# edshkim98/LocalDiffusion-Hallucination

Measured on AMD Instinct MI355X. Metric: local patches/sec (256^2, T=1000), higher is better.
Workload: dtype bf16; 1 GPU; cfg3: 8 local patches (vertical band masks) of one 3x256x256 image per GPU, 4-stage dim-32 conditional UNet (12.1M params), DDPM T=1000, pred_x0, sigmoid schedule; patches_per_gpu=8, parallelism=patch-sharded x1, one all-gather per sample, step_graph_replay=True, whole_batch_graph_flag=False, concurrent_sub_batches=2, weight_split_levels=0

## Files before the change

include/localdiff_hip.h:

```cpp
#ifndef LOCALDIFF_HIP_H
#define LOCALDIFF_HIP_H

#include <stddef.h>
#include <stdint.h>

#ifdef __cplusplus
extern "C" {
#endif

#define LD_OK 0
#define LD_EINVAL (-1)
#define LD_EHIP (-2)
#define LD_ETIMEOUT (-3)

#define LD_F32 0
#define LD_BF16 1
#define LD_F16 2

#define LD_STAT_STRIPES 16

#define LD_ACT_NONE 0
#define LD_ACT_SILU 1
#define LD_ACT_RELU 2

// ... 20 lines not shown
int ld_tuning_count(void);
const char* ld_tuning_name(int index);
#define LD_COUNTER_CONV3X3_C32 0
#define LD_COUNTER_CONV3X3_GENERIC 1
#define LD_COUNTER_CONV3X3_S32 2
#define LD_COUNTER_MAX 8
long long ld_counter(int which);
int ld_range_push(const char* name );
int ld_range_pop(void);

typedef struct ld_src {
  const void* data;
  int32_t C;
  int32_t pix_stride;
  int32_t upsample;
  const double* gn_stats;
  const float* gn_gamma;
  const float* gn_beta;
  int32_t gn_groups;
  int32_t act;
  const float* film;
  int32_t film_tstride;
  int32_t film_bstride;
} ld_src;

typedef struct ld_conv3x3_args {
  ld_src src[2];
  int32_t nsrc;
  const void* weight;
  const float* bias;
  void* out;
  double* out_stats;
  int32_t out_groups;
  int32_t B, H, W, Cout;
  const int32_t* t_ptr;
  int32_t dtype;
  const void* addend;
  int32_t weight_terms;
  const void* side_weight;
  const float* side_bias;
  void* side_out;
} ld_conv3x3_args;
int ld_conv3x3(const ld_conv3x3_args* args, void* stream);

#define LD_EPI_PLAIN 0
#define LD_EPI_QKV_LINEAR 1
#define LD_EPI_QKV_FULL 2
#define LD_EPI_RMS_RES 3
#define LD_EPI_RES 4
#define LD_EPI_GN_TAIL 5
typedef struct ld_conv1x1_args {
  ld_src src[2];
  int32_t nsrc;
  int32_t unshuffle;
  int32_t rms_in;
  const void* weight;
  int64_t weight_bstride;
  const float* bias;
  int32_t epilogue;
  int32_t hidden;
  float q_scale;
  const float* g2;
  const void* residual;
  ld_src gn_tail;
  void* out;
  uint32_t* kmax_out;
  int32_t B, H, W, Cout;
  int32_t dtype;
  int32_t weight_terms;
} ld_conv1x1_args;
int ld_conv1x1(const ld_conv1x1_args* args, void* stream);

int ld_pack_conv_weight(const float* w_oihw, const float* scale_in, void* out, int cout, int cin,
                        int ksize, int unshuffle, int dtype, void* stream);
int ld_pack_conv_weight_terms(const float* w_oihw, const float* scale_in, void* out, int cout, int cin,
                              int ksize, int unshuffle, int dtype, int terms, void* stream);

int ld_conv_image(const float* x_nchw, const float* w_oihw, const float* bias, void* out,
                  double* out_stats, int out_groups, int B, int Cin, int H, int W, int ksize,
                  int dtype, void* stream);

size_t ld_stem_packed_bytes(void);
int ld_pack_stem_weight(const float* w_oihw , void* out_packed, int Cin, void* stream);
int ld_conv_stem(const float* x, const void* w_packed, const float* bias, void* out, int B, int Cin, int H, int W,
                 int dtype , void* stream);
typedef struct ld_step_begin_args {
  void* zero_a; size_t bytes_a; void* zero_b; size_t bytes_b;
  int32_t* t_ptr; int delta; int32_t* idx_ptr; const int32_t* t_table;
  const float* film_rows; int row_floats; float* film_cur;
} ld_step_begin_args;
int ld_conv_stem_begin(const float* x, const void* w_packed, const float* bias, void* out, int B, int Cin, int H, int W,
                       int dtype, const ld_step_begin_args* begin, void* stream);


typedef struct ld_gn_apply_args {
  ld_src a;
  ld_src b;
  int32_t final_act;
  int32_t pool;
  void* out;
  int32_t B, H, W;
  const int32_t* t_ptr;
  int32_t dtype;
} ld_gn_apply_args;
int ld_gn_apply(const ld_gn_apply_args* args, void* stream);

int ld_linattn_kmax(const void* qkv, uint32_t* kmax_enc, int B, int n, int heads, int dim_head,
                    int dtype, void* stream);
int ld_linattn_ctx(const void* qkv, const uint32_t* kmax_enc, float* ctx_part,
                   int B, int n, int heads, int dim_head, int nchunks, int dtype, void* stream);
int ld_linattn_ctx_reduce(const float* ctx_part, int nchunks, float* ctxn, int B, int heads,
                          int dim_head, void* stream);
int ld_linattn_fold(const float* ctxn, const float* w_out ,
                    void* w_packed , int B, int C, int heads, int dim_head,
                    int perm, int dtype, void* stream);
int ld_linattn_ctxfold(const float* ctx_part, int nchunks, const float* w_out ,
                       void* w_packed , int B, int C, int heads, int dim_head,
                       int perm, int dtype, void* stream);
int ld_linattn_kvctx(const void* x, const void* wkv_packed, const float* kshift, float* ctx_part, int B,
                     int n, int C, int heads, int dim_head, int nchunks, int dtype, void* stream);
int ld_linattn_out(const void* x, const void* wq_packed, const float* qshift, const void* mfold,
                   const float* bias, const float* g2, void* out, int B, int n, int C, float q_scale,
                   int dtype, void* stream);
int ld_linattn_kvctx_terms(const void* x, const void* wkv_packed, const float* kshift, float* ctx_part, int B, int n, int C,
                           int heads, int dim_head, int nchunks, int dtype, int weight_terms, void* stream);
int ld_linattn_out_terms(const void* x, const void* wq_packed, const float* qshift, const void* mfold, const float* bias,
                         const float* g2, void* out, int B, int n, int C, float q_scale, int dtype, int weight_terms,
                         void* stream);
size_t ld_linattn_ctx_part_floats(int B, int heads, int dim_head, int nchunks);

int ld_attention(const void* qkv, void* out, int B, int n, int heads, int dim_head, int dtype,
                 void* stream);

int ld_time_mlp(const int32_t* times, int n, const float* freqs, int dim, const float* w1,
                const float* b1, const float* w2, const float* b2, int time_dim, float* temb,
                void* stream);
int ld_time_mlp_fourier(const int32_t* times, int n, const float* weights, int learned_dim, const float* w1,
                        const float* b1, const float* w2, const float* b2, int time_dim, float* temb, void* stream);
int ld_film(const float* temb, int n, int time_dim, const float* w, const float* b, int two_c,
            float* film, void* stream);

int ld_final_conv(const void* x, const float* w , const float* b, float* out_nchw,
                  int B, int H, int W, int Cin, int Cout, int dtype, void* stream);

int ld_final_step(const void* x, const float* w, const float* b, float* model_out, float* x_t, float* x0_out,
                  const float* sched, const int32_t* t_ptr, float lo, float hi, int objective, uint64_t seed,
                  int64_t noise_stream, int B, int H, int W, int Cin, int Cout, int dtype, void* stream);


int ld_final_step_at(const void* x, const float* w, const float* b, float* model_out, float* x_t, float* x0_out,
                     const float* sched, const int32_t* t_ptr, float lo, float hi, int objective, uint64_t seed,
                     int64_t noise_base, int64_t noise_tmul, int64_t noise_first, const float* keep_mask,
                     int B, int H, int W, int Cin, int Cout, int dtype, void* stream);

#define LD_OBJ_X0 0
#define LD_OBJ_NOISE 1
#define LD_OBJ_V 2
#define LD_SCHED_COLS 8
#define LD_SCHED_COEF1 0
#define LD_SCHED_COEF2 1
#define LD_SCHED_SIGMA 2
#define LD_SCHED_SQRT_RECIP 3
#define LD_SCHED_SQRT_RECIPM1 4
#define LD_SCHED_SQRT_AB 5
#define LD_SCHED_SQRT_1MAB 6
#define LD_SCHED_ABAR 7

int ld_randn(float* out, int64_t n, uint64_t seed, int64_t stream_base, int64_t stream_tmul,
             const int32_t* t_ptr, void* stream);
int ld_randn_at(float* out, int64_t n, int64_t first, uint64_t seed, int64_t stream_base, int64_t stream_tmul,
                const int32_t* t_ptr, void* stream);
int ld_step_add(int32_t* t_ptr, int delta, void* stream);
int ld_step_begin(void* zero_a, size_t bytes_a, void* zero_b, size_t bytes_b, int32_t* t_ptr, int delta,
                  int32_t* idx_ptr, const int32_t* t_table, void* stream);
int ld_step_begin_film(void* zero_a, size_t bytes_a, void* zero_b, size_t bytes_b, int32_t* t_ptr, int delta,
                       int32_t* idx_ptr, const int32_t* t_table, const float* film_rows, int row_floats,
                       float* film_cur, void* stream);

int ld_ddpm_step(const float* x_t, const float* model_out, const float* noise, float* x_prev,
                 float* x0_out, const float* sched, const int32_t* t_ptr, float lo, float hi,
                 int objective, int64_t n, void* stream);
int ld_ddim_step(const float* x_t, const float* model_out, const float* noise, float* x_next,
                 float sqrt_recip, float sqrt_recipm1, float sqrt_ab, float sqrt_1mab,
                 float sqrt_abar_next, float c, float sigma, float lo, float hi, int objective,
                 int last, int64_t n, void* stream);
int ld_ddim_step_at(const float* x_t, const float* model_out, const float* noise, float* x_next,
                    const float* pair_table, const int32_t* idx_ptr, float lo, float hi, int objective, int64_t n,
                    void* stream);
int ld_branch_conditions(const float* cond, const float* mask, float* cond_out, float* cond_in,
                         float lo_clip, int B, int C, int HW, void* stream);
int ld_mask_out(float* model_out, const float* mask, float min_val, int B, int C, int HW,
                void* stream);
int ld_fuse_ddpm(const float* x_out, const float* x_in, const float* x0_out, const float* x0_in,
                 const float* mask, float* x, float* x0, float lo, float hi, int B, int C, int HW,
                 void* stream);
int ld_branch_conditions_k(const float* cond, const float* masks, float* cond_k, float lo_clip, int B, int C, int K,
                           int HW, void* stream);
int ld_fuse_ddpm_k(const float* x_first, const float* x_rest, const float* x0_first, const float* x0_rest,
                   const float* masks, float* x, float* x0, float lo, float hi, int B, int C, int K, int HW,
                   void* stream);
int ld_posterior_step(const float* x_t, const float* x0, const float* noise, float* x_prev,
                      const float* sched, const int32_t* t_ptr, int64_t n, void* stream);
int ld_fuse_ddim(const float* x_out, const float* x_in, const float* x0_out, const float* x0_in,
                 const float* mask, const float* noise, float* x_next, float sqrt_recip,
                 float sqrt_recipm1, float sqrt_abar_next, float c, float sigma, float lo,
                 float hi, int B, int C, int HW, void* stream);
int ld_fuse_ddim_k(const float* x_first, const float* x_rest, const float* x0_first, const float* x0_rest,
                   const float* masks, const float* noise, float* x_next, float sqrt_recip, float sqrt_recipm1,
                   float sqrt_abar_next, float c, float sigma, float lo, float hi, int B, int C, int K, int HW,
                   void* stream);
int ld_q_sample(const float* x0, const float* noise, float* out, float sqrt_ab, float sqrt_1mab,
                int64_t n, void* stream);
int ld_q_sample_t(const float* x0, const float* noise, float* out, const int* t, const float* sqrt_ab,
                  const float* sqrt_1mab, int B, int64_t elems_per_sample, void* stream);
int ld_p_losses(const float* model_out, const float* x_start, const float* noise, const int* t, const float* sqrt_ab,
                const float* sqrt_1mab, const float* loss_weight, float* loss_out, int B, int64_t elems_per_sample,
                int objective, void* stream);
int ld_recompose(const float* patches , const float* masks , float* out,
                 int B, int K, int C, int HW, void* stream);

#define LD_SEG_SRC_PLAIN 0
#define LD_SEG_SRC_POOL 1
#define LD_SEG_SRC_CAT_D2S 2
typedef struct ld_seg_conv_args {
  const void* src0;
  const void* src1;
  int32_t C0, C1;
  int32_t mode;
  int32_t ksize;
  const float* weight;
  const float* scale;
  const float* shift;
  int32_t relu;
  void* out;
  int32_t B, H, W, Cout;
  int32_t dtype;
} ld_seg_conv_args;
int ld_seg_conv(const ld_seg_conv_args* args, void* stream);
int ld_seg_conv_image(const float* x_nchw, const float* w_oihw, const float* scale, const float* shift, void* out,
                      int B, int Cin, int H, int W, int dtype, void* stream);
int ld_seg_head(const void* x, const float* w, const float* bias, float* logits, float* prob, float* mask,
                int B, int H, int W, int C, int dtype, void* stream);
int ld_seg_pack_weight(const float* w_oihw, float* out, int cout, int cin, int ksize, void* stream);
int ld_seg_pack_convt(const float* w, const float* bias, float* w_out, float* bias_out, int cin, int cout, void* stream);

#define LD_SEG_RED_WORK_BYTES (2048 * 2 * 64 * 8)
int ld_seg_wgrad_splits(int B, int H, int W, int Cin, int Cout, int ksize);
int ld_seg_wgrad(const float* dy, const float* a, float* work, float* dw, int B, int H, int W, int Cin, int Cout,
                 int ksize, int splits, void* stream);
int ld_seg_bn_train(const float* y, const float* gamma, const float* beta, double* work, float* stat, float* running_mean,
                    float* running_var, float momentum, float eps, float* out, int64_t M, int C, void* stream);
int ld_seg_bn_backward(const float* da, const float* act, const float* y, const float* gamma, const float* stat, double* work,
                       float* dgamma, float* dbeta, float* dy, int64_t M, int C, void* stream);
int ld_seg_colsum(const float* x, double* work, float* out, int64_t M, int C, int fold, void* stream);
int ld_seg_pool(const float* x, float* out, int B, int H, int W, int C, void* stream);
int ld_seg_pool_backward(const float* x, const float* dpool, const float* dskip, float* dx, int B, int H, int W, int C,
                         void* stream);
int ld_seg_cat_d2s(const float* skip, const float* low, float* out, int B, int H, int W, int C0, int C1, void* stream);
int ld_seg_cat_d2s_backward(const float* dcat, float* dskip, float* dlow, int B, int H, int W, int C0, int C1, void* stream);
int ld_seg_loss(const float* logits, const float* target, double* work, float* out, float* dz, int64_t M, float pos_weight,
                float dice_eps, void* stream);
int ld_seg_head_backward(const float* dz, const float* x, const float* w, double* work, float* dw, float* db, float* dx,
                         int64_t M, int C, void* stream);
int ld_seg_adam(float* param, const float* grad, float* m, float* v, int d0, int d1, int d2, int64_t s0, int64_t s1,
                int64_t s2, double beta1, double beta2, double eps, double step_size, double bc2_sqrt, void* stream);
int ld_seg_permute3(const float* in, float* out, int d0, int d1, int d2, int64_t off, int64_t s0, int64_t s1, int64_t s2,
                    void* stream);

typedef struct ld_pc_conv_args {
  const float* src;
  const float* weight;
  const float* scale;
  const float* shift;
  const float* residual;
  float* out;
  int32_t B, Hi, Wi, Cin, Ho, Wo, Cout;
  int32_t ksize;
  int32_t stride;
  int32_t relu;
} ld_pc_conv_args;
int ld_pc_conv(const ld_pc_conv_args* args, void* stream);
int ld_pc_stem(const float* x_nchw, const float* w_oihw, const float* scale, const float* shift, float* out,
               int B, int H, int W, void* stream);
int ld_pc_maxpool(const float* x, float* out, int B, int H, int W, int C, void* stream);
int ld_pc_embed(const float* l2, const float* l3, float* rows, float* norms, int B, int h2, int w2, int C2, int h3,
                int w3, int C3, void* stream);
int ld_pc_row_norms(const float* x, float* norms, int64_t n, int d, void* stream);
int ld_pc_knn(const float* q, const float* qn, int N, const float* bank, const float* bn, int64_t M, int D,
              unsigned long long* work, float* dist, int32_t* idx, void* stream);
int ld_pc_knn_topk(const float* q, const float* qn, int N, const float* bank, const float* bn, int64_t M, int D, int k,
                   float* d2, float* dist, int32_t* idx, void* stream);
int ld_pc_score_prepare(const float* patch_scores, const int32_t* loc, const float* bank, const float* bn, int B, int P,
                        int D, float* q, float* qn, int32_t* argmax, void* stream);
int ld_pc_score(const float* rows, const float* row_norms, const float* patch_scores, const int32_t* argmax,
                const float* bank, const float* bn, const int32_t* support, int B, int P, int D, int k, float* pred_score,
                void* stream);
int ld_pc_anomaly_map(const float* scores, const float* g, int ks, float* tmp, float* out, int B, int h, int w, int H,
                      int W, void* stream);

int ld_pc_project(const float* e, int64_t N, int D, const int32_t* rowptr, const int32_t* cols, const float* vals, int k,
                  float* out, int64_t ld, void* stream);
int ld_pc_coreset(const float* ft, int64_t ld, int64_t N, int k, int64_t n, int64_t start, float* min_d,
                  unsigned long long* keys, int64_t* idx, void* stream);

int ld_clf_max(const float* x, int groups, int64_t n, uint32_t* words, void* stream);
enum { LD_CLF_PLAIN = 0, LD_CLF_HALVE = 1, LD_CLF_AFFINE = 2 };
// ... 61 lines not shown
```

localdiffusion-hallucination_amd/_cabi.py:

```python
import ctypes as C
import os

from .tuning import lib_override_path

_HERE = os.path.dirname(os.path.abspath(__file__))

LIB_PATH = lib_override_path() or os.path.join(_HERE, "csrc", "liblocaldiff_hip.so")

LD_F32, LD_BF16, LD_F16 = 0, 1, 2
ACT_NONE, ACT_SILU, ACT_RELU = 0, 1, 2
EPI_PLAIN, EPI_QKV_LINEAR, EPI_QKV_FULL, EPI_RMS_RES, EPI_RES, EPI_GN_TAIL = 0, 1, 2, 3, 4, 5
OBJ = {"pred_x0": 0, "pred_noise": 1, "pred_v": 2}
SCHED_COLS = 8
STAT_STRIPES = 16
COUNTER_CONV3X3_C32, COUNTER_CONV3X3_GENERIC, COUNTER_CONV3X3_S32 = 0, 1, 2
SEG_SRC_PLAIN, SEG_SRC_POOL, SEG_SRC_CAT_D2S = 0, 1, 2
CLF_PLAIN, CLF_HALVE, CLF_AFFINE = 0, 1, 2

vp, i32, i64, u64, f32 = C.c_void_p, C.c_int32, C.c_int64, C.c_uint64, C.c_float


class Src(C.Structure):
    _fields_ = [("data", vp), ("C", i32), ("pix_stride", i32), ("upsample", i32), ("gn_stats", vp),
                ("gn_gamma", vp), ("gn_beta", vp), ("gn_groups", i32), ("act", i32), ("film", vp),
                ("film_tstride", i32), ("film_bstride", i32)]


class Conv3x3Args(C.Structure):
    _fields_ = [("src", Src * 2), ("nsrc", i32), ("weight", vp), ("bias", vp), ("out", vp),
                ("out_stats", vp), ("out_groups", i32), ("B", i32), ("H", i32), ("W", i32),
                ("Cout", i32), ("t_ptr", vp), ("dtype", i32), ("addend", vp), ("weight_terms", i32),
                ("side_weight", vp), ("side_bias", vp), ("side_out", vp)]


class Conv1x1Args(C.Structure):
    _fields_ = [("src", Src * 2), ("nsrc", i32), ("unshuffle", i32), ("rms_in", i32), ("weight", vp),
                ("weight_bstride", i64), ("bias", vp), ("epilogue", i32), ("hidden", i32),
                ("q_scale", f32), ("g2", vp), ("residual", vp), ("gn_tail", Src), ("out", vp), ("kmax_out", vp), ("B", i32), ("H", i32),
                ("W", i32), ("Cout", i32), ("dtype", i32), ("weight_terms", i32)]


class GnApplyArgs(C.Structure):
    _fields_ = [("a", Src), ("b", Src), ("final_act", i32), ("pool", i32), ("out", vp), ("B", i32),
                ("H", i32), ("W", i32), ("t_ptr", vp), ("dtype", i32)]


class StepBeginArgs(C.Structure):
    _fields_ = [("zero_a", vp), ("bytes_a", C.c_size_t), ("zero_b", vp), ("bytes_b", C.c_size_t), ("t_ptr", vp), ("delta", i32),
                ("idx_ptr", vp), ("t_table", vp), ("film_rows", vp), ("row_floats", i32), ("film_cur", vp)]


class SegConvArgs(C.Structure):
    _fields_ = [("src0", vp), ("src1", vp), ("C0", i32), ("C1", i32), ("mode", i32), ("ksize", i32), ("weight", vp),
                ("scale", vp), ("shift", vp), ("relu", i32), ("out", vp), ("B", i32), ("H", i32), ("W", i32),
                ("Cout", i32), ("dtype", i32)]


class PcConvArgs(C.Structure):
    _fields_ = [("src", vp), ("weight", vp), ("scale", vp), ("shift", vp), ("residual", vp), ("out", vp), ("B", i32),
                ("Hi", i32), ("Wi", i32), ("Cin", i32), ("Ho", i32), ("Wo", i32), ("Cout", i32), ("ksize", i32),
                ("stride", i32), ("relu", i32)]


class ClfResizeArgs(C.Structure):
    _fields_ = [("x", vp), ("out", vp), ("B", i32), ("Cin", i32), ("Cout", i32), ("Hi", i32), ("Wi", i32), ("Ho", i32),
                ("Wo", i32), ("mode", i32), ("max_words", vp), ("per_sample", i32), ("zero_words", vp), ("n_zero", i32),
                ("sub", f32), ("mul", f32), ("add", f32), ("div", f32), ("normalize", i32), ("mean", f32 * 3),
                ("std", f32 * 3), ("pred", vp), ("threshold", f32), ("decision", vp), ("n_decision", i32)]


class McAdamTensor(C.Structure):
    _fields_ = [("param", vp), ("grad", vp), ("m", vp), ("v", vp), ("d0", i32), ("d1", i32), ("d2", i32), ("gs0", i64),
                ("gs1", i64), ("gs2", i64), ("mirror0", vp), ("m0_off", i64), ("m0_s0", i64), ("m0_s1", i64), ("m0_s2", i64),
                ("mirror1", vp), ("m1_off", i64), ("m1_s0", i64), ("m1_s1", i64), ("m1_s2", i64)]


_SIGS = {
    "ld_last_error": (C.c_char_p, []),
    "ld_version": (C.c_int, []),
    "ld_device_info": (C.c_int, [C.c_char_p, C.c_int, C.POINTER(C.c_int), C.POINTER(i64)]),
    "ld_graph_begin": (C.c_int, [vp]),
    "ld_graph_end": (C.c_int, [vp, C.POINTER(vp)]),
    "ld_graph_launch": (C.c_int, [vp, vp]),
    "ld_graph_destroy": (C.c_int, [vp]),
    "ld_memset_zero": (C.c_int, [vp, C.c_size_t, vp]),
    "ld_memset_bytes": (C.c_int, [vp, C.c_int, C.c_size_t, vp]),
    "ld_event_create": (C.c_int, [C.POINTER(vp)]),
    "ld_event_record": (C.c_int, [vp, vp]),
    "ld_event_elapsed_ms": (C.c_int, [vp, vp, C.POINTER(f32)]),
    "ld_event_destroy": (C.c_int, [vp]),
    "ld_stream_wait_event": (C.c_int, [vp, vp]),
    "ld_counter": (C.c_longlong, [C.c_int]),
    "ld_tuning_set": (C.c_int, [C.c_char_p, C.c_longlong]),
    "ld_tuning_get": (C.c_int, [C.c_char_p, C.POINTER(C.c_longlong)]),
    "ld_tuning_count": (C.c_int, []),
    "ld_tuning_name": (C.c_char_p, [C.c_int]),
    "ld_range_push": (C.c_int, [C.c_char_p]),
    "ld_range_pop": (C.c_int, []),
    "ld_conv3x3": (C.c_int, [C.POINTER(Conv3x3Args), vp]),
    "ld_conv1x1": (C.c_int, [C.POINTER(Conv1x1Args), vp]),
    "ld_pack_conv_weight": (C.c_int, [vp, vp, vp, C.c_int, C.c_int, C.c_int, C.c_int, C.c_int, vp]),
    "ld_pack_conv_weight_terms": (C.c_int, [vp, vp, vp, C.c_int, C.c_int, C.c_int, C.c_int, C.c_int, C.c_int, vp]),
    "ld_conv_image": (C.c_int, [vp, vp, vp, vp, vp, C.c_int, C.c_int, C.c_int, C.c_int, C.c_int,
                                C.c_int, C.c_int, vp]),
    "ld_stem_packed_bytes": (C.c_size_t, []),
    "ld_pack_stem_weight": (C.c_int, [vp, vp, C.c_int, vp]),
    "ld_conv_stem": (C.c_int, [vp, vp, vp, vp, C.c_int, C.c_int, C.c_int, C.c_int, C.c_int, vp]),
    "ld_conv_stem_begin": (C.c_int, [vp, vp, vp, vp, C.c_int, C.c_int, C.c_int, C.c_int, C.c_int, C.POINTER(StepBeginArgs), vp]),
    "ld_gn_apply": (C.c_int, [C.POINTER(GnApplyArgs), vp]),
    "ld_linattn_kmax": (C.c_int, [vp, vp, C.c_int, C.c_int, C.c_int, C.c_int, C.c_int, vp]),
    "ld_linattn_ctx": (C.c_int, [vp, vp, vp, C.c_int, C.c_int, C.c_int, C.c_int, C.c_int, C.c_int, vp]),
    "ld_linattn_ctx_reduce": (C.c_int, [vp, C.c_int, vp, C.c_int, C.c_int, C.c_int, vp]),
    "ld_linattn_fold": (C.c_int, [vp, vp, vp, C.c_int, C.c_int, C.c_int, C.c_int, C.c_int, C.c_int, vp]),
    "ld_linattn_ctxfold": (C.c_int, [vp, C.c_int, vp, vp, C.c_int, C.c_int, C.c_int, C.c_int, C.c_int, C.c_int, vp]),
    "ld_linattn_kvctx": (C.c_int, [vp, vp, vp, vp, C.c_int, C.c_int, C.c_int, C.c_int, C.c_int, C.c_int, C.c_int, vp]),
    "ld_linattn_out": (C.c_int, [vp, vp, vp, vp, vp, vp, vp, C.c_int, C.c_int, C.c_int, f32, C.c_int, vp]),
    "ld_linattn_kvctx_terms": (C.c_int, [vp, vp, vp, vp, C.c_int, C.c_int, C.c_int, C.c_int, C.c_int, C.c_int, C.c_int, C.c_int, vp]),
    "ld_linattn_out_terms": (C.c_int, [vp, vp, vp, vp, vp, vp, vp, C.c_int, C.c_int, C.c_int, f32, C.c_int, C.c_int, vp]),
    "ld_linattn_ctx_part_floats": (C.c_size_t, [C.c_int, C.c_int, C.c_int, C.c_int]),
    "ld_attention": (C.c_int, [vp, vp, C.c_int, C.c_int, C.c_int, C.c_int, C.c_int, vp]),
    "ld_time_mlp": (C.c_int, [vp, C.c_int, vp, C.c_int, vp, vp, vp, vp, C.c_int, vp, vp]),
    "ld_time_mlp_fourier": (C.c_int, [vp, C.c_int, vp, C.c_int, vp, vp, vp, vp, C.c_int, vp, vp]),
    "ld_film": (C.c_int, [vp, C.c_int, C.c_int, vp, vp, C.c_int, vp, vp]),
    "ld_final_conv": (C.c_int, [vp, vp, vp, vp, C.c_int, C.c_int, C.c_int, C.c_int, C.c_int, C.c_int, vp]),
    "ld_final_step": (C.c_int, [vp, vp, vp, vp, vp, vp, vp, vp, f32, f32, C.c_int, u64, i64, C.c_int, C.c_int, C.c_int,
                                C.c_int, C.c_int, C.c_int, vp]),
    "ld_final_step_at": (C.c_int, [vp, vp, vp, vp, vp, vp, vp, vp, f32, f32, C.c_int, u64, i64, i64, i64, vp, C.c_int,
                                   C.c_int, C.c_int, C.c_int, C.c_int, C.c_int, vp]),
    "ld_timing_begin": (C.c_int, [C.c_int]),
    "ld_timing_count": (C.c_int, []),
    "ld_timing_end": (C.c_int, [vp, C.c_int, vp]),
    "ld_timing_end_abs": (C.c_int, [vp, vp, C.c_int, vp]),
    "ld_randn": (C.c_int, [vp, i64, u64, i64, i64, vp, vp]),
    "ld_randn_at": (C.c_int, [vp, i64, i64, u64, i64, i64, vp, vp]),
    "ld_step_add": (C.c_int, [vp, C.c_int, vp]),
    "ld_step_begin": (C.c_int, [vp, C.c_size_t, vp, C.c_size_t, vp, C.c_int, vp, vp, vp]),
    "ld_step_begin_film": (C.c_int, [vp, C.c_size_t, vp, C.c_size_t, vp, C.c_int, vp, vp, vp, C.c_int, vp, vp]),
    "ld_ddim_step_at": (C.c_int, [vp, vp, vp, vp, vp, vp, f32, f32, C.c_int, i64, vp]),
    "ld_ddpm_step": (C.c_int, [vp, vp, vp, vp, vp, vp, vp, f32, f32, C.c_int, i64, vp]),
    "ld_posterior_step": (C.c_int, [vp, vp, vp, vp, vp, vp, i64, vp]),
    "ld_ddim_step": (C.c_int, [vp, vp, vp, vp, f32, f32, f32, f32, f32, f32, f32, f32, f32, C.c_int,
                               C.c_int, i64, vp]),
    "ld_branch_conditions": (C.c_int, [vp, vp, vp, vp, f32, C.c_int, C.c_int, C.c_int, vp]),
    "ld_mask_out": (C.c_int, [vp, vp, f32, C.c_int, C.c_int, C.c_int, vp]),
    "ld_fuse_ddpm": (C.c_int, [vp, vp, vp, vp, vp, vp, vp, f32, f32, C.c_int, C.c_int, C.c_int, vp]),
    "ld_branch_conditions_k": (C.c_int, [vp, vp, vp, f32, C.c_int, C.c_int, C.c_int, C.c_int, vp]),
    "ld_fuse_ddpm_k": (C.c_int, [vp, vp, vp, vp, vp, vp, vp, f32, f32, C.c_int, C.c_int, C.c_int, C.c_int, vp]),
    "ld_fuse_ddim": (C.c_int, [vp, vp, vp, vp, vp, vp, vp, f32, f32, f32, f32, f32, f32, f32, C.c_int,
                               C.c_int, C.c_int, vp]),
    "ld_fuse_ddim_k": (C.c_int, [vp, vp, vp, vp, vp, vp, vp, f32, f32, f32, f32, f32, f32, f32, C.c_int, C.c_int,
                                 C.c_int, C.c_int, vp]),
    "ld_q_sample": (C.c_int, [vp, vp, vp, f32, f32, i64, vp]),
    "ld_q_sample_t": (C.c_int, [vp, vp, vp, vp, vp, vp, C.c_int, i64, vp]),
    "ld_p_losses": (C.c_int, [vp, vp, vp, vp, vp, vp, vp, vp, C.c_int, i64, C.c_int, vp]),
    "ld_recompose": (C.c_int, [vp, vp, vp, C.c_int, C.c_int, C.c_int, C.c_int, vp]),
    "ld_seg_conv": (C.c_int, [C.POINTER(SegConvArgs), vp]),
    "ld_seg_conv_image": (C.c_int, [vp, vp, vp, vp, vp, C.c_int, C.c_int, C.c_int, C.c_int, C.c_int, vp]),
    "ld_seg_head": (C.c_int, [vp, vp, vp, vp, vp, vp, C.c_int, C.c_int, C.c_int, C.c_int, C.c_int, vp]),
    "ld_seg_pack_weight": (C.c_int, [vp, vp, C.c_int, C.c_int, C.c_int, vp]),
    "ld_seg_pack_convt": (C.c_int, [vp, vp, vp, vp, C.c_int, C.c_int, vp]),
    "ld_seg_wgrad_splits": (C.c_int, [C.c_int, C.c_int, C.c_int, C.c_int, C.c_int, C.c_int]),
    "ld_seg_wgrad": (C.c_int, [vp, vp, vp, vp, C.c_int, C.c_int, C.c_int, C.c_int, C.c_int, C.c_int, C.c_int, vp]),
    "ld_seg_bn_train": (C.c_int, [vp, vp, vp, vp, vp, vp, vp, f32, f32, vp, i64, C.c_int, vp]),
    "ld_seg_bn_backward": (C.c_int, [vp, vp, vp, vp, vp, vp, vp, vp, vp, i64, C.c_int, vp]),
    "ld_seg_colsum": (C.c_int, [vp, vp, vp, i64, C.c_int, C.c_int, vp]),
    "ld_seg_pool": (C.c_int, [vp, vp, C.c_int, C.c_int, C.c_int, C.c_int, vp]),
    "ld_seg_pool_backward": (C.c_int, [vp, vp, vp, vp, C.c_int, C.c_int, C.c_int, C.c_int, vp]),
    "ld_seg_cat_d2s": (C.c_int, [vp, vp, vp, C.c_int, C.c_int, C.c_int, C.c_int, C.c_int, vp]),
    "ld_seg_cat_d2s_backward": (C.c_int, [vp, vp, vp, C.c_int, C.c_int, C.c_int, C.c_int, C.c_int, vp]),
    "ld_seg_loss": (C.c_int, [vp, vp, vp, vp, vp, i64, f32, f32, vp]),
    "ld_seg_head_backward": (C.c_int, [vp, vp, vp, vp, vp, vp, vp, i64, C.c_int, vp]),
    "ld_seg_adam": (C.c_int, [vp, vp, vp, vp, C.c_int, C.c_int, C.c_int, i64, i64, i64, C.c_double, C.c_double, C.c_double,
                    C.c_double, C.c_double, vp]),
    "ld_seg_permute3": (C.c_int, [vp, vp, C.c_int, C.c_int, C.c_int, i64, i64, i64, i64, vp]),
    "ld_pc_conv": (C.c_int, [C.POINTER(PcConvArgs), vp]),
    "ld_pc_stem": (C.c_int, [vp, vp, vp, vp, vp, C.c_int, C.c_int, C.c_int, vp]),
    "ld_pc_maxpool": (C.c_int, [vp, vp, C.c_int, C.c_int, C.c_int, C.c_int, vp]),
    "ld_pc_embed": (C.c_int, [vp, vp, vp, vp, C.c_int, C.c_int, C.c_int, C.c_int, C.c_int, C.c_int, C.c_int, vp]),
    "ld_pc_row_norms": (C.c_int, [vp, vp, i64, C.c_int, vp]),
    "ld_pc_knn": (C.c_int, [vp, vp, C.c_int, vp, vp, i64, C.c_int, vp, vp, vp, vp]),
    "ld_pc_knn_topk": (C.c_int, [vp, vp, C.c_int, vp, vp, i64, C.c_int, C.c_int, vp, vp, vp, vp]),
    "ld_pc_score_prepare": (C.c_int, [vp, vp, vp, vp, C.c_int, C.c_int, C.c_int, vp, vp, vp, vp]),
    "ld_pc_score": (C.c_int, [vp, vp, vp, vp, vp, vp, vp, C.c_int, C.c_int, C.c_int, C.c_int, vp, vp]),
    "ld_pc_anomaly_map": (C.c_int, [vp, vp, C.c_int, vp, vp, C.c_int, C.c_int, C.c_int, C.c_int, C.c_int, vp]),
    "ld_pc_project": (C.c_int, [vp, i64, C.c_int, vp, vp, vp, C.c_int, vp, i64, vp]),
    "ld_pc_coreset": (C.c_int, [vp, i64, i64, C.c_int, i64, i64, vp, vp, vp, vp]),
    "ld_clf_max": (C.c_int, [vp, C.c_int, i64, vp, vp]),
    "ld_clf_resize": (C.c_int, [C.POINTER(ClfResizeArgs), vp]),
    "ld_clf_decide": (C.c_int, [vp, f32, vp, C.c_int, vp]),
    "ld_mc_conv1": (C.c_int, [vp, vp, vp, vp, vp, C.c_int, vp]),
    "ld_mc_pool": (C.c_int, [vp, vp, vp, C.c_int, C.c_int, C.c_int, C.c_int, vp]),
    "ld_mc_pool_backward": (C.c_int, [vp, vp, vp, vp, C.c_int, C.c_int, C.c_int, C.c_int, vp]),
    "ld_mc_gemm": (C.c_int, [vp, vp, vp, C.c_int, C.c_int, C.c_int, i64, i64, i64, i64, i64, C.c_int, vp]),
    "ld_mc_fc1_finish": (C.c_int, [vp, vp, vp, C.c_int, C.c_int, C.c_int, vp]),
    "ld_mc_head": (C.c_int, [vp, vp, vp, vp, vp, vp, vp, vp, vp, vp, C.c_int, vp]),
    "ld_mc_small_grads": (C.c_int, [vp, vp, vp, vp, vp, vp, vp, vp, C.c_int, vp]),
    "ld_mc_conv1_wgrad_work_floats": (i64, [C.c_int]),
    "ld_mc_conv1_wgrad": (C.c_int, [vp, vp, vp, vp, vp, vp, vp, C.c_int, vp]),
    "ld_mc_adam": (C.c_int, [C.POINTER(McAdamTensor), C.c_int, C.c_double, C.c_double, C.c_double, C.c_double, C.c_double, vp]),
    "ld_comm_unique_id": (C.c_int, [vp]),
    "ld_comm_init": (C.c_int, [C.POINTER(vp), vp, C.c_int, C.c_int]),
    "ld_comm_init_timeout": (C.c_int, [C.POINTER(vp), vp, C.c_int, C.c_int, C.c_double]),
    "ld_allgather": (C.c_int, [vp, vp, C.c_size_t, vp, vp]),
    "ld_comm_destroy": (C.c_int, [vp]),
}

EXPORTS = tuple(_SIGS)
_lib = None


def lib():
    global _lib
    if _lib is not None:
        return _lib
    if not os.path.exists(LIB_PATH):
        raise RuntimeError(
            f"{LIB_PATH} is missing: build it with `python -c 'import __graft_entry__ as g; g.build()'` "
            "(or csrc/build.sh).  There is no CPU fallback for the HIP hot path.")
    try:
        l = C.CDLL(LIB_PATH)
    except OSError as e:
        raise RuntimeError(f"cannot load {LIB_PATH}: {e}") from e
    for name, (res, args) in _SIGS.items():
        try:
            fn = getattr(l, name)
        except AttributeError as e:
            raise RuntimeError(f"{LIB_PATH} does not export {name}") from e
        fn.restype, fn.argtypes = res, args
    _lib = l
    return l


LD_ETIMEOUT = -3


def check(rc, what=""):
    if rc != 0:
        msg = lib().ld_last_error().decode("utf-8", "replace")
        if rc == LD_ETIMEOUT:
            raise TimeoutError(f"localdiff_hip {what} timed out: {msg}")
        raise RuntimeError(f"localdiff_hip {what} failed (rc={rc}): {msg}")


class prof_range:

    def __init__(self, name):
        self.name = name.encode()

    def __enter__(self):
        lib().ld_range_push(self.name)

    def __exit__(self, *exc):
        lib().ld_range_pop()


def ptr(t):
    return None if t is None else t.data_ptr()


def dtype_code(name):
    return {"fp32": LD_F32, "float32": LD_F32, "bf16": LD_BF16, "bfloat16": LD_BF16, "fp16": LD_F16, "float16": LD_F16,
            "half": LD_F16}[name]
```

localdiffusion-hallucination_amd/csrc/conv1x1.hip:

```cpp
#include "common.hip.h"
#include <stdlib.h>

namespace {

constexpr int EPI_GN_TAIL_RES = 6;

struct Conv1Dev {
  SrcDev s[2];
  const void* w;
  long w_bstride;
  const void* res;
  void* out;
  int nsrc, unshuffle, rms_in;
  int B, H, W, Cout;
  int wsplit;
  int group;
  int epi, hidden;
  float q_scale;
  const float* bias;
  const float* g2;
  unsigned* kmax;
  SrcDev tail;
};

constexpr int KG = 4;
typedef const Conv1Dev __attribute__((address_space(4)))* Conv1KernargPtr;
template <typename T, int MT, int NW, int EPI, int G, bool TLEAD, bool KLEAD = false>
__device__ __forceinline__ void conv1x1_body(const Conv1Dev& head, Conv1KernargPtr rest) {
  constexpr int E = DT<T>::E, CK = DT<T>::CK;
  constexpr int NPT = 64 * NW, PLANE = NPT * 16;
  constexpr int XCH = 4 * PLANE, WCHB = MT * 1024;
  static_assert(!TLEAD || EPI == LD_EPI_GN_TAIL || EPI == EPI_GN_TAIL_RES, "tail-lead variant: GroupNorm-tail epilogues only");
  Conv1Dev a = head;
  if constexpr (KLEAD) {
    a.out = rest->out; a.bias = rest->bias; a.g2 = rest->g2; a.kmax = rest->kmax; a.hidden = rest->hidden; a.q_scale = rest->q_scale;
  }
  if constexpr (!TLEAD && !KLEAD) {
    asm volatile("" ::"s"(a.H), "s"(a.W), "s"(a.Cout), "s"(a.nsrc), "s"(a.unshuffle), "s"(a.rms_in), "s"(a.wsplit), "s"(a.s[0].C),
                 "s"(a.s[0].ld), "s"(a.s[0].data), "s"(a.s[1].C), "s"(a.s[1].ld), "s"(a.s[1].data), "s"(a.w), "s"(a.w_bstride),
                 "s"(a.res), "s"(a.out));
    if constexpr (EPI == LD_EPI_GN_TAIL || EPI == EPI_GN_TAIL_RES)
      asm volatile("" ::"s"(a.tail.data), "s"(a.tail.stats), "s"(a.tail.gamma), "s"(a.tail.beta), "s"(a.tail.film), "s"(a.tail.C),
                   "s"(a.tail.groups), "s"(a.tail.act), "s"(a.tail.film_bstride));
  }

  extern __shared__ __attribute__((aligned(16))) char smem[];
  char* s_x = smem;
  char* s_w = smem + G * XCH;
  float* s_rinv = reinterpret_cast<float*>(s_w + G * WCHB);
  float* s_tcoef = s_rinv + NPT;

  const int tid = threadIdx.x, lane = tid & 63, wv = tid >> 6, px = lane & 15, kq = lane >> 4;
  const int b = blockIdx.z, m0 = blockIdx.y * MT;
  const int HW = a.H * a.W, p0 = blockIdx.x * NPT;
  const int mt_total = a.Cout / 16;

  f32x4 acc[MT][NW];
#pragma unroll
  for (int m = 0; m < MT; ++m)
#pragma unroll
    for (int j = 0; j < NW; ++j) acc[m][j] = f32x4{0.f, 0.f, 0.f, 0.f};
  float rs[NW];
#pragma unroll
  for (int i = 0; i < NW; ++i) rs[i] = 0.f;

  constexpr bool TAIL = EPI == LD_EPI_GN_TAIL || EPI == EPI_GN_TAIL_RES;
  constexpr bool HAS_OP2 = EPI == LD_EPI_RMS_RES || EPI == LD_EPI_RES || TAIL;
  typedef typename Raw4<T>::type R4;
  constexpr bool W2 = sizeof(T) == 2;
  constexpr int MP = W2 ? MT / 2 : MT;
  typedef typename std::conditional<W2, uint4, R4>::type RP;
  RP op2[HAS_OP2 ? MP : 1][HAS_OP2 ? NW : 1];
  auto load_op = [&](const T* src, RP (&dst)[MP][NW]) {
#pragma unroll
    for (int j = 0; j < NW; ++j) {
      const int p = min(p0 + (wv * NW + j) * 16 + px, HW - 1);
      const T* pix = src + ((size_t)b * HW + p) * a.Cout + m0 * 16;
#pragma unroll
      for (int m = 0; m < MP; ++m) {
        if constexpr (W2) dst[m][j] = *reinterpret_cast<const uint4*>(reinterpret_cast<const char*>(pix + m * 32) + pair_frag16_off(kq));
        else dst[m][j] = load4_raw<T>(pix + m * 16 + kq * 4);
      }
    }
  };
  auto pin_op = [&](const RP& r) {
    if constexpr (W2) asm volatile("" ::"v"(r.x), "v"(r.y), "v"(r.z), "v"(r.w));
    else pin_raw4(r);
  };
  auto frag_op = [&](const RP (&src)[MP][NW], int m, int j, float* v) {
    if constexpr (W2) {
      uint2 f0, f1;
      unpair_frag16(src[m >> 1][j], f0, f1);
      unpack4<T>((m & 1) ? f1 : f0, v);
    } else {
      unpack4<T>(src[m][j], v);
    }
  };
  if constexpr (HAS_OP2) load_op(reinterpret_cast<const T*>(TAIL ? a.tail.data : a.res), op2);
  if constexpr (TAIL) {
    double* red = reinterpret_cast<double*>(s_tcoef + 2 * a.Cout);
    if constexpr (TLEAD) {
      build_gn_coef<DT<T>::precise>(a.tail, b, 0, (long)HW, s_tcoef, red, tid, 256, [&]() {
        Conv1KernargPtr pr = rest;
        asm volatile("" : "+s"(pr));
        a.s[0].data = pr->s[0].data; a.s[0].C = pr->s[0].C; a.s[0].ld = pr->s[0].ld;
        a.s[1].data = pr->s[1].data; a.s[1].C = pr->s[1].C; a.s[1].ld = pr->s[1].ld;
        a.w = pr->w; a.w_bstride = pr->w_bstride; a.res = pr->res; a.out = pr->out;
        a.nsrc = pr->nsrc; a.unshuffle = pr->unshuffle; a.rms_in = pr->rms_in; a.H = pr->H; a.W = pr->W;
        a.wsplit = pr->wsplit; a.hidden = pr->hidden; a.q_scale = pr->q_scale; a.bias = pr->bias; a.g2 = pr->g2; a.kmax = pr->kmax;
        a.tail.act = pr->tail.act;
      });
    } else {
      build_gn_coef<DT<T>::precise>(a.tail, b, 0, (long)HW, s_tcoef, red, tid, 256);
    }
  }
  const int nc0 = a.s[0].C / CK;
  const int ws = a.wsplit;
  const int nch = (a.unshuffle ? 4 * nc0 : nc0 + (a.nsrc > 1 ? a.s[1].C / CK : 0)) << ws;
  const uint4* wg = reinterpret_cast<const uint4*>(reinterpret_cast<const char*>(a.w) + (size_t)b * a.w_bstride);

  auto frag_ptr = [&](int chv, int it) -> const uint4* {
    const int ch = chv >> ws;
    int si = 0, c0, p1 = 0, p2 = 0;
    if (a.unshuffle) {
      const int pp = ch / nc0;
      c0 = (ch - pp * nc0) * CK;
      p1 = pp >> 1; p2 = pp & 1;
    } else {
      si = ch >= nc0 ? 1 : 0;
      c0 = (ch - si * nc0) * CK;
    }
    const T* sdata = reinterpret_cast<const T*>(si ? a.s[1].data : a.s[0].data);
    const int Cs = si ? a.s[1].ld : a.s[0].ld;
    const int p = p0 + (it * 4 + wv) * 16 + px;
    if (p >= HW) return nullptr;
    size_t pix;
    if (a.unshuffle) {
      const int y = p / a.W, x = p - y * a.W;
      pix = ((size_t)b * (2 * a.H) + 2 * y + p1) * (2 * a.W) + 2 * x + p2;
    } else {
      pix = (size_t)b * HW + p;
    }
    return reinterpret_cast<const uint4*>(sdata + pix * Cs + c0 + kq * E);
  };
  auto stage = [&](const uint4& raw, int it, char* xdst) {
    if (a.rms_in) {
      float v[E];
      unpack16<T>(raw, v);
#pragma unroll
      for (int e = 0; e < E; ++e) rs[it] = fmaf(v[e], v[e], rs[it]);
    }
    *reinterpret_cast<uint4*>(xdst + kq * PLANE + ((it * 4 + wv) * 16 + px) * 16) = raw;
  };
  auto mfma_chunk = [&](const char* xsrc, const char* wsrc) {
    uint4 A[MT];
#pragma unroll
    for (int m = 0; m < MT; ++m) A[m] = *reinterpret_cast<const uint4*>(wsrc + m * 1024 + lane * 16);
#pragma unroll
    for (int j = 0; j < NW; ++j) {
      const uint4 Bf = *reinterpret_cast<const uint4*>(xsrc + kq * PLANE + ((wv * NW + j) * 16 + px) * 16);
#pragma unroll
      for (int m = 0; m < MT; ++m) mma16<T>(acc[m][j], A[m], Bf);
    }
  };
  constexpr int WPT = (MT * 64 + 255) / 256;
  if constexpr (G > 1) {
    for (int c0 = 0; c0 < nch; c0 += G) {
      uint4 raw[G][NW], wr[G][WPT];
#pragma unroll
      for (int g = 0; g < G; ++g) {
        if (c0 + g < nch) {
#pragma unroll
          for (int it = 0; it < NW; ++it) {
            const uint4* gp = frag_ptr(c0 + g, it);
            raw[g][it] = gp ? *gp : make_uint4(0u, 0u, 0u, 0u);
          }
#pragma unroll
          for (int k = 0; k < WPT; ++k) {
            const int u = k * 256 + tid;
            wr[g][k] = u < MT * 64 ? wg[((size_t)(c0 + g) * mt_total + m0) * 64 + u] : make_uint4(0u, 0u, 0u, 0u);
          }
        }
      }
      __syncthreads();
#pragma unroll
      for (int g = 0; g < G; ++g) {
        if (c0 + g < nch) {
#pragma unroll
          for (int it = 0; it < NW; ++it) stage(raw[g][it], it, s_x + (size_t)g * XCH);
#pragma unroll
          for (int k = 0; k < WPT; ++k) {
            const int u = k * 256 + tid;
            if (u < MT * 64) *reinterpret_cast<uint4*>(s_w + (size_t)g * WCHB + u * 16) = wr[g][k];
          }
        }
      }
      __syncthreads();
#pragma unroll
      for (int g = 0; g < G; ++g)
        if (c0 + g < nch) mfma_chunk(s_x + (size_t)g * XCH, s_w + (size_t)g * WCHB);
    }
  } else {
    for (int ch = 0; ch < nch; ++ch) {
      __syncthreads();
#pragma unroll
      for (int it = 0; it < NW; ++it) {
        const uint4* gp = frag_ptr(ch, it);
        stage(gp ? *gp : make_uint4(0u, 0u, 0u, 0u), it, s_x);
      }
#pragma unroll
      for (int k = 0; k < WPT; ++k) {
        const int u = k * 256 + tid;
        if (u < MT * 64) *reinterpret_cast<uint4*>(s_w + u * 16) = wg[((size_t)ch * mt_total + m0) * 64 + u];
      }
      __syncthreads();
      mfma_chunk(s_x, s_w);
    }
  }

  if (a.rms_in) {
#pragma unroll
    for (int it = 0; it < NW; ++it) {
      float r = rs[it];
      r = kq4_sum(r);
      if (kq == 0) s_rinv[(it * 4 + wv) * 16 + px] = rms_rinv<DT<T>::precise>(r);
    }
    __syncthreads();
  }

  float bv[MT][4], g2v[EPI == LD_EPI_RMS_RES ? MT : 1][4];
#pragma unroll
  for (int m = 0; m < MT; ++m) {
    const int co = (m0 + m) * 16 + kq * 4;
    const float4 t = a.bias ? *reinterpret_cast<const float4*>(a.bias + co) : make_float4(0.f, 0.f, 0.f, 0.f);
    bv[m][0] = t.x; bv[m][1] = t.y; bv[m][2] = t.z; bv[m][3] = t.w;
    if constexpr (EPI == LD_EPI_RMS_RES) {
      const float4 g = *reinterpret_cast<const float4*>(a.g2 + co);
      g2v[m][0] = g.x; g2v[m][1] = g.y; g2v[m][2] = g.z; g2v[m][3] = g.w;
    }
  }
  constexpr bool HAS_OP3 = EPI == EPI_GN_TAIL_RES;
  RP op3[HAS_OP3 ? MP : 1][HAS_OP3 ? NW : 1];
  if constexpr (HAS_OP3) load_op(reinterpret_cast<const T*>(a.res), op3);

  T* out = reinterpret_cast<T*>(a.out);
  const bool q_part = (m0 * 16) < a.hidden;
  const bool k_part = a.kmax != nullptr && (m0 * 16) >= a.hidden && (m0 * 16) < 2 * a.hidden;
  float cmax[MT][4];
#pragma unroll
  for (int m = 0; m < MT; ++m)
#pragma unroll
    for (int r = 0; r < 4; ++r) cmax[m][r] = -INFINITY;
#pragma unroll
  for (int m = 0; m < MT; ++m) {
    asm volatile("" ::"v"(bv[m][0]), "v"(bv[m][1]), "v"(bv[m][2]), "v"(bv[m][3]));
    if constexpr (EPI == LD_EPI_RMS_RES) asm volatile("" ::"v"(g2v[m][0]), "v"(g2v[m][1]), "v"(g2v[m][2]), "v"(g2v[m][3]));
  }
#pragma unroll
  for (int m = 0; m < MP; ++m) {
    if constexpr (HAS_OP2) {
#pragma unroll
      for (int j = 0; j < NW; ++j) pin_op(op2[m][j]);
    }
    if constexpr (HAS_OP3) {
#pragma unroll
      for (int j = 0; j < NW; ++j) pin_op(op3[m][j]);
    }
  }
#pragma unroll
  for (int j = 0; j < NW; ++j) {
    const int qq = (wv * NW + j) * 16 + px;
    const int p = p0 + qq;
    const bool valid = p < HW;
    const float rinv = a.rms_in ? s_rinv[qq] : 1.0f;
    float v[MT][4];
#pragma unroll
    for (int m = 0; m < MT; ++m) {
#pragma unroll
      for (int r = 0; r < 4; ++r) v[m][r] = acc[m][j][r] * rinv + bv[m][r];
    }
    if (EPI == LD_EPI_QKV_LINEAR && q_part) {
#pragma unroll
      for (int m = 0; m < MT; m += 2) {
        float mx = v[m][0];
#pragma unroll
        for (int r = 0; r < 4; ++r) { mx = fmaxf(mx, v[m][r]); mx = fmaxf(mx, v[m + 1][r]); }
        mx = kq4_max(mx);
        float sum = 0.f;
#pragma unroll
        for (int r = 0; r < 4; ++r) {
          v[m][r] = DT<T>::precise ? expf(v[m][r] - mx) : __expf(v[m][r] - mx);
          v[m + 1][r] = DT<T>::precise ? expf(v[m + 1][r] - mx) : __expf(v[m + 1][r] - mx);
          sum += v[m][r] + v[m + 1][r];
        }
        sum = kq4_sum(sum);
        const float sc = DT<T>::precise ? a.q_scale / sum : a.q_scale * __builtin_amdgcn_rcpf(sum);
#pragma unroll
        for (int r = 0; r < 4; ++r) { v[m][r] *= sc; v[m + 1][r] *= sc; }
      }
    } else if (EPI == LD_EPI_QKV_FULL && q_part) {
#pragma unroll
      for (int m = 0; m < MT; ++m)
#pragma unroll
        for (int r = 0; r < 4; ++r) v[m][r] *= a.q_scale;
    } else if (EPI == LD_EPI_RMS_RES) {
      float ss = 0.f;
#pragma unroll
      for (int m = 0; m < MT; ++m)
#pragma unroll
        for (int r = 0; r < 4; ++r) ss = fmaf(v[m][r], v[m][r], ss);
      ss = kq4_sum(ss);
      const float inv = rms_rinv<DT<T>::precise>(ss);
#pragma unroll
      for (int m = 0; m < MT; ++m) {
#pragma unroll
        for (int r = 0; r < 4; ++r) v[m][r] = v[m][r] * inv * g2v[m][r];
      }
    }
    if (k_part && valid) {
#pragma unroll
      for (int m = 0; m < MT; ++m)
#pragma unroll
        for (int r = 0; r < 4; ++r) cmax[m][r] = fmaxf(cmax[m][r], v[m][r]);
    }
#pragma unroll
    for (int m = 0; m < MT; ++m) {
      const int co = (m0 + m) * 16 + kq * 4;
      if constexpr (EPI == LD_EPI_RMS_RES || EPI == LD_EPI_RES) {
        float o2[4];
        frag_op(op2, m, j, o2);
#pragma unroll
        for (int r = 0; r < 4; ++r) v[m][r] += o2[r];
      } else if constexpr (TAIL) {
        float rv[4];
        frag_op(op2, m, j, rv);
        affine_act_n<DT<T>::precise, 4>(rv, s_tcoef + co, s_tcoef + a.Cout + co, a.tail.act);
#pragma unroll
        for (int r = 0; r < 4; ++r) v[m][r] += rv[r];
        if constexpr (HAS_OP3) {
          float o3[4];
          frag_op(op3, m, j, o3);
#pragma unroll
          for (int r = 0; r < 4; ++r) v[m][r] += o3[r];
        }
      }
    }
    T* opix = out + ((size_t)b * HW + (valid ? p : 0)) * a.Cout + m0 * 16;
    if constexpr (sizeof(T) == 2) {
      static_assert(MT % 2 == 0, "m-tiles are stored in pairs");
#pragma unroll
      for (int m = 0; m < MT; m += 2) {
        const uint4 w16 = pair_frag16<T>(v[m], v[m + 1]);
        if (valid) store16_out(reinterpret_cast<char*>(opix + m * 16) + pair_frag16_off(kq), w16);
      }
    } else if (valid) {
#pragma unroll
      for (int m = 0; m < MT; ++m) store4<T>(opix + m * 16 + kq * 4, v[m]);
    }
  }
  if (k_part) {
    float* s_cm = reinterpret_cast<float*>(s_x);
    __syncthreads();
#pragma unroll
    for (int m = 0; m < MT; ++m)
#pragma unroll
      for (int r = 0; r < 4; ++r) {
        const float cm = wave16_max(cmax[m][r]);
        if (px == 0) s_cm[wv * 16 * MT + m * 16 + kq * 4 + r] = cm;
      }
    __syncthreads();
    if (tid < 16 * MT) {
      const float cm = fmaxf(fmaxf(s_cm[tid], s_cm[16 * MT + tid]), fmaxf(s_cm[32 * MT + tid], s_cm[48 * MT + tid]));
      const int stripe = blockIdx.x % LD_STAT_STRIPES;
      if (cm > -INFINITY)
        atomicMax(a.kmax + ((size_t)b * LD_STAT_STRIPES + stripe) * a.hidden + m0 * 16 + tid - a.hidden, enc_max(cm));
    }
  }
}

template <typename T, int MT, int NW, int EPI, int G = 1>
__global__ __launch_bounds__(256) void conv1x1_kernel(Conv1Dev a) {
  conv1x1_body<T, MT, NW, EPI, G, false>(a, nullptr);
}
template <typename T, int MT, int NW, int EPI, int G>
__global__ __launch_bounds__(256) void conv1x1_taillead_kernel(const void* t_data, const double* t_stats, const float* t_gamma, const float* t_beta,
                                                               const float* t_film, int cout_groups, int hw, Conv1Dev rest) {
  Conv1Dev a{};
  a.tail.data = t_data; a.tail.stats = t_stats; a.tail.gamma = t_gamma; a.tail.beta = t_beta; a.tail.film = t_film;
  a.Cout = cout_groups & 0xffff; a.tail.C = a.Cout; a.tail.ld = a.Cout; a.tail.groups = (int)((unsigned)cout_groups >> 16);
  a.H = hw; a.W = 1;
  constexpr unsigned REST_OFF = ld_kernarg_offset<const void*, const double*, const float*, const float*, const float*, int, int>(alignof(Conv1Dev));
  static_assert(REST_OFF == 48, "conv1x1_taillead_kernel: leading arguments changed");
  typedef const char __attribute__((address_space(4)))* KChar;
  conv1x1_body<T, MT, NW, EPI, G, true>(a, (Conv1KernargPtr)((KChar)__builtin_amdgcn_kernarg_segment_ptr() + REST_OFF));
}

template <typename T, int MT, int NW, int EPI, int G>
__global__ __launch_bounds__(256) void conv1x1_klead_kernel(const void* data0, const void* w, const void* data1, const void* res, int H, int W,
                                                            int Cout, int c0_flags, int ld0, int c1_ld1, Conv1Dev rest) {
  Conv1Dev a{};
  a.s[0].data = data0; a.s[0].C = c0_flags & 0xffff; a.s[0].ld = ld0;
  a.s[1].data = data1; a.s[1].C = c1_ld1 & 0xffff; a.s[1].ld = (int)((unsigned)c1_ld1 >> 16);
  a.w = w; a.res = res; a.H = H; a.W = W; a.Cout = Cout;
  a.nsrc = (c0_flags >> 16) & 3; a.unshuffle = (c0_flags >> 18) & 1; a.rms_in = (c0_flags >> 19) & 1; a.wsplit = (c0_flags >> 20) & 1;
  constexpr unsigned REST_OFF = ld_kernarg_offset<const void*, const void*, const void*, const void*, int, int, int, int, int, int>(alignof(Conv1Dev));
  static_assert(REST_OFF == 56, "conv1x1_klead_kernel: leading arguments changed");
  typedef const char __attribute__((address_space(4)))* KChar;
  conv1x1_body<T, MT, NW, EPI, G, false, true>(a, (Conv1KernargPtr)((KChar)__builtin_amdgcn_kernarg_segment_ptr() + REST_OFF));
}

template <typename T, int MT, int NW, int EPI>
int launch_epi(const Conv1Dev& a, hipStream_t st) {
  constexpr int NPT = 64 * NW;
  const size_t tail = NPT * sizeof(float) + (EPI == LD_EPI_GN_TAIL || EPI == EPI_GN_TAIL_RES ? 2 * a.Cout * sizeof(float) + 64 * sizeof(double) : 0);
  const size_t chunk = 4 * NPT * 16 + MT * 1024;
  const int HW = a.H * a.W;
  dim3 grid((HW + NPT - 1) / NPT, a.Cout / (16 * MT), a.B);
  constexpr bool CAN_TLEAD = EPI == LD_EPI_GN_TAIL || EPI == EPI_GN_TAIL_RES;
  const bool tlead = CAN_TLEAD && ld_tuning().lead_args && a.tail.film_bstride == 0 && a.tail.film_tstride == 0 && a.Cout < 65536 && a.tail.groups < 32768 &&
                     a.tail.C == a.Cout && a.tail.ld == a.Cout && (long)HW < (1L << 31);
#define LD_C1_TLEAD_ARGS a.tail.data, a.tail.stats, a.tail.gamma, a.tail.beta, a.tail.film, a.Cout | (a.tail.groups << 16), HW, a
  if constexpr (CAN_TLEAD) {
    if (tlead && (a.group == KG || a.group == 2)) {
      const size_t lds = (size_t)a.group * chunk + tail;
      if (a.group == KG) {
        if (lds > 65536) LD_HIP(ld_allow_lds((conv1x1_taillead_kernel<T, MT, NW, EPI, KG>), lds));
        LD_LAUNCH((conv1x1_taillead_kernel<T, MT, NW, EPI, KG>), grid, dim3(256), lds, st, LD_C1_TLEAD_ARGS);
      } else {
        if (lds > 65536) LD_HIP(ld_allow_lds((conv1x1_taillead_kernel<T, MT, NW, EPI, 2>), lds));
        LD_LAUNCH((conv1x1_taillead_kernel<T, MT, NW, EPI, 2>), grid, dim3(256), lds, st, LD_C1_TLEAD_ARGS);
      }
      LD_LAUNCH_CHECK("conv1x1(GroupNorm tail, lead)");
      return LD_OK;
    }
  }
#undef LD_C1_TLEAD_ARGS
  if constexpr (!CAN_TLEAD) {
    const bool klead = ld_tuning().lead_args && (a.group == KG || a.group == 2) && a.w_bstride == 0 && a.s[0].C < 65536 && a.s[1].C < 65536 && a.s[1].ld < 65536;
    if (klead) {
      const int c0f = a.s[0].C | (a.nsrc << 16) | (a.unshuffle ? 1 << 18 : 0) | (a.rms_in ? 1 << 19 : 0) | (a.wsplit ? 1 << 20 : 0);
      const int c1l = (a.nsrc > 1 ? a.s[1].C : 0) | ((a.nsrc > 1 ? a.s[1].ld : 0) << 16);
      const size_t lds = (size_t)a.group * chunk + tail;
#define LD_C1_KLEAD_ARGS a.s[0].data, a.w, a.s[1].data, a.res, a.H, a.W, a.Cout, c0f, a.s[0].ld, c1l, a
      if (a.group == KG) {
        if (lds > 65536) LD_HIP(ld_allow_lds((conv1x1_klead_kernel<T, MT, NW, EPI, KG>), lds));
        LD_LAUNCH((conv1x1_klead_kernel<T, MT, NW, EPI, KG>), grid, dim3(256), lds, st, LD_C1_KLEAD_ARGS);
      } else {
        if (lds > 65536) LD_HIP(ld_allow_lds((conv1x1_klead_kernel<T, MT, NW, EPI, 2>), lds));
        LD_LAUNCH((conv1x1_klead_kernel<T, MT, NW, EPI, 2>), grid, dim3(256), lds, st, LD_C1_KLEAD_ARGS);
      }
#undef LD_C1_KLEAD_ARGS
      LD_LAUNCH_CHECK("conv1x1(grouped K, lead)");
      return LD_OK;
    }
  }
  if (a.group == KG) {
    const size_t lds = KG * chunk + tail;
    if (lds > 65536) LD_HIP(ld_allow_lds((conv1x1_kernel<T, MT, NW, EPI, KG>), lds));
    LD_LAUNCH((conv1x1_kernel<T, MT, NW, EPI, KG>), grid, dim3(256), lds, st, a);
    LD_LAUNCH_CHECK("conv1x1(grouped K)");
    return LD_OK;
  }
  if (a.group == 2) {
    const size_t lds = 2 * chunk + tail;
    if (lds > 65536) LD_HIP(ld_allow_lds((conv1x1_kernel<T, MT, NW, EPI, 2>), lds));
    LD_LAUNCH((conv1x1_kernel<T, MT, NW, EPI, 2>), grid, dim3(256), lds, st, a);
    LD_LAUNCH_CHECK("conv1x1(grouped K, pairs)");
    return LD_OK;
  }
  LD_LAUNCH((conv1x1_kernel<T, MT, NW, EPI>), grid, dim3(256), chunk + tail, st, a);
  LD_LAUNCH_CHECK("conv1x1");
  return LD_OK;
}

template <typename T, int MT, int NW>
int launch(const Conv1Dev& a, hipStream_t st) {
  switch (a.epi) {
    case LD_EPI_PLAIN: return launch_epi<T, MT, NW, LD_EPI_PLAIN>(a, st);
    case LD_EPI_QKV_LINEAR: return launch_epi<T, MT, NW, LD_EPI_QKV_LINEAR>(a, st);
    case LD_EPI_QKV_FULL: return launch_epi<T, MT, NW, LD_EPI_QKV_FULL>(a, st);
    case LD_EPI_RMS_RES: return launch_epi<T, MT, NW, LD_EPI_RMS_RES>(a, st);
    case LD_EPI_RES: return launch_epi<T, MT, NW, LD_EPI_RES>(a, st);
    default: return a.res ? launch_epi<T, MT, NW, EPI_GN_TAIL_RES>(a, st) : launch_epi<T, MT, NW, LD_EPI_GN_TAIL>(a, st);
  }
}

template <typename T>
int dispatch(const Conv1Dev& a0, hipStream_t st) {
  Conv1Dev a = a0;
  const int HW = a.H * a.W;
  {
    const LdTuning& tn = ld_tuning();
    const long group_max_px = tn.c1_group_max_px;
    const int group_on = (int)tn.c1_group;
    const int ck = DT<T>::CK;
    const int nc0 = a.s[0].C / ck;
    const int nch = (a.unshuffle ? 4 * nc0 : nc0 + (a.nsrc > 1 ? a.s[1].C / ck : 0)) << a.wsplit;
    const int group_min_ch = (int)tn.c1_group_min_ch;
    a.group = (group_on && (long)HW * a.B <= group_max_px && nch >= group_min_ch) ? KG : 0;
    const long pair_max_px = tn.c1_pair_max_px;
    if (group_on && !a.group && (long)HW * a.B <= pair_max_px && nch >= 2) a.group = 2;
  }
  if (a.epi == LD_EPI_RMS_RES) {
    switch (a.Cout) {
      case 32: return launch<T, 2, 2>(a, st);
      case 64: return launch<T, 4, 2>(a, st);
      case 128: return launch<T, 8, 2>(a, st);
      default: return ld_fail(LD_EINVAL, "ld_conv1x1: RMS_RES epilogue supports Cout 32/64/128 (got %d)", a.Cout);
    }
  }
  bool mt4 = (a.Cout % 64) == 0;
  const long small_min = ld_tuning().c1_small_min;
  if (mt4 && (long)((HW + 127) / 128) * (a.Cout / 64) * a.B < small_min) mt4 = false;
  const long blocks4 = (long)((HW + 255) / 256) * (a.Cout / (mt4 ? 64 : 32)) * a.B;
  const bool big = blocks4 >= 512;
  if (mt4) return big ? launch<T, 4, 4>(a, st) : launch<T, 4, 2>(a, st);
  return big ? launch<T, 2, 4>(a, st) : launch<T, 2, 2>(a, st);
}

}

extern "C" int ld_conv1x1(const ld_conv1x1_args* p, void* stream) {
  LD_REQUIRE(p != nullptr, "ld_conv1x1: null args");
  LD_REQUIRE(p->nsrc == 1 || p->nsrc == 2, "ld_conv1x1: nsrc must be 1 or 2");
  LD_REQUIRE(ld_dtype_ok(p->dtype), "ld_conv1x1: bad dtype %d", p->dtype);
  LD_REQUIRE(p->Cout > 0 && p->Cout % 32 == 0, "ld_conv1x1: Cout %d must be a multiple of 32", p->Cout);
  LD_REQUIRE(p->B > 0 && p->H > 0 && p->W > 0 && p->weight && p->out, "ld_conv1x1: bad shape/null");
  LD_REQUIRE(!(p->unshuffle && p->nsrc != 1), "ld_conv1x1: unshuffle takes one source");
  LD_REQUIRE(p->epilogue >= LD_EPI_PLAIN && p->epilogue <= LD_EPI_GN_TAIL, "ld_conv1x1: bad epilogue");
  if (p->epilogue == LD_EPI_QKV_LINEAR || p->epilogue == LD_EPI_QKV_FULL)
    LD_REQUIRE(p->hidden > 0 && p->hidden % 64 == 0 && p->Cout == 3 * p->hidden,
               "ld_conv1x1: QKV epilogue needs Cout == 3*hidden, hidden %% 64 == 0");
  if (p->epilogue == LD_EPI_RMS_RES) LD_REQUIRE(p->g2 && p->residual, "ld_conv1x1: RMS_RES needs g2/residual");
  LD_REQUIRE((reinterpret_cast<uintptr_t>(p->bias) & 15) == 0 && (reinterpret_cast<uintptr_t>(p->g2) & 15) == 0,
             "ld_conv1x1: bias / g2 must be 16-byte aligned (read as float4)");
  if (p->epilogue == LD_EPI_RES) LD_REQUIRE(p->residual, "ld_conv1x1: RES needs residual");
  Conv1Dev a;
  for (int s = 0; s < p->nsrc; ++s) {
    LD_REQUIRE(p->src[s].data && p->src[s].C > 0 && p->src[s].C % 32 == 0,
               "ld_conv1x1: src[%d] null or C %% 32 != 0", s);
    LD_REQUIRE(p->src[s].gn_stats == nullptr && !p->src[s].upsample,
               "ld_conv1x1: GroupNorm/upsample prologues are 3x3-only");
    a.s[s] = to_dev(p->src[s]);
  }
  if (p->nsrc == 1) a.s[1] = a.s[0];
  a.nsrc = p->nsrc; a.unshuffle = p->unshuffle; a.rms_in = p->rms_in;
  a.w = p->weight; a.w_bstride = p->weight_bstride; a.bias = p->bias;
  a.epi = p->epilogue;
  a.hidden = (p->epilogue == LD_EPI_QKV_LINEAR || p->epilogue == LD_EPI_QKV_FULL) ? p->hidden : 0;
  a.q_scale = p->q_scale; a.g2 = p->g2; a.res = p->residual; a.out = p->out;
  a.kmax = (p->epilogue == LD_EPI_QKV_LINEAR) ? p->kmax_out : nullptr;
  if (p->epilogue == LD_EPI_GN_TAIL) {
    const ld_src& t = p->gn_tail;
    LD_REQUIRE(t.gn_groups <= 16, "ld_conv1x1: gn_tail groups %d > 16 (the stripe reduction uses 16 lanes per group)", t.gn_groups);
    LD_REQUIRE(t.data && t.gn_stats && t.gn_gamma && t.gn_beta && t.gn_groups > 0 && t.C == p->Cout &&
               t.C % t.gn_groups == 0 && (t.pix_stride == 0 || t.pix_stride == t.C) && !t.film,
               "ld_conv1x1: GN_TAIL operand incomplete");
    a.tail = to_dev(t);
  } else {
    a.tail = a.s[0];
  }
  a.B = p->B; a.H = p->H; a.W = p->W; a.Cout = p->Cout;
  a.group = 0;
  LD_REQUIRE(p->weight_terms >= 0 && p->weight_terms <= 2 && !(p->weight_terms == 2 && (!ld_dtype_16(p->dtype) || p->rms_in || p->weight_bstride)),
             "ld_conv1x1: weight_terms %d (2 needs 16-bit storage, no rms_in, no per-batch weights)", p->weight_terms);
  a.wsplit = p->weight_terms == 2 ? 1 : 0;
  hipStream_t st = reinterpret_cast<hipStream_t>(stream);
  return LD_DISPATCH(p->dtype, dispatch<T>(a, st));
}
```

localdiffusion-hallucination_amd/csrc/pointwise.hip:

```cpp
#include "common.hip.h"

namespace {
constexpr int BS = 256;
inline unsigned nblocks(long n, int per = 1) {
  long b = (n + (long)BS * per - 1) / ((long)BS * per);
  if (b > 4096) b = 4096;
  if (b < 1) b = 1;
  return (unsigned)b;
}
#define GRID_STRIDE(i, n) for (long i = (long)blockIdx.x * BS + threadIdx.x; i < (n); i += (long)gridDim.x * BS)

__device__ __forceinline__ float clampf(float v, float lo, float hi) { return fminf(fmaxf(v, lo), hi); }

__device__ __forceinline__ float to_x0(float x, float mo, const float* row, int obj) {
  if (obj == LD_OBJ_X0) return mo;
  if (obj == LD_OBJ_NOISE) return row[LD_SCHED_SQRT_RECIP] * x - row[LD_SCHED_SQRT_RECIPM1] * mo;
  return row[LD_SCHED_SQRT_AB] * x - row[LD_SCHED_SQRT_1MAB] * mo;
}

__device__ __forceinline__ unsigned long long mix64(unsigned long long z) {
  z = (z ^ (z >> 30)) * 0xBF58476D1CE4E5B9ull;
  z = (z ^ (z >> 27)) * 0x94D049BB133111EBull;
  return z ^ (z >> 31);
}
__global__ void randn_kernel(float* out, long n, long first, unsigned long long seed, long stream_base, long stream_tmul,
                             const int* t_ptr) {
  const long stream = stream_base + (t_ptr ? stream_tmul * (long)(*t_ptr) : 0);
  const unsigned long long base = mix64(seed ^ ((unsigned long long)stream * 0xD1B54A32D192ED03ull));
  GRID_STRIDE(i, n) {
    const unsigned long long h = mix64(base + (unsigned long long)(first + i + 1) * 0x9E3779B97F4A7C15ull);
    const float u1 = ((float)(unsigned)(h >> 40) + 1.0f) * 5.9604644775390625e-8f;
    const float u2 = (float)(unsigned)((h >> 16) & 0xFFFFFFu) * 5.9604644775390625e-8f;
    out[i] = sqrtf(-2.0f * logf(u1)) * cosf(6.283185307179586f * u2);
  }
}
__global__ void step_add_kernel(int* t, int delta) { if (threadIdx.x == 0 && blockIdx.x == 0) *t += delta; }
__global__ void step_begin_kernel(StepBeginDev sb) {
  __shared__ int s_t;
  step_begin_work(sb, blockIdx.x, gridDim.x, &s_t);
}

__global__ void ddpm_step_kernel(const float* x, const float* mo, const float* z, float* xp, float* x0o,
                                 const float* sched, const int* t_ptr, float lo, float hi, int obj, long n) {
  const int t = t_ptr ? *t_ptr : 0;
  const float* row = sched + (size_t)t * LD_SCHED_COLS;
  const float c1 = row[LD_SCHED_COEF1], c2 = row[LD_SCHED_COEF2], sg = row[LD_SCHED_SIGMA];
  const bool draw = (t_ptr ? t > 0 : true) && z != nullptr;
  GRID_STRIDE(i, n) {
    const float xi = x[i];
    const float x0 = clampf(to_x0(xi, mo[i], row, obj), lo, hi);
    const float mean = c1 * x0 + c2 * xi;
    xp[i] = draw ? mean + sg * z[i] : mean;
    if (x0o) x0o[i] = x0;
  }
}
__global__ void posterior_step_kernel(const float* x, const float* x0, const float* z, float* xp,
                                      const float* sched, const int* t_ptr, long n) {
  const int t = t_ptr ? *t_ptr : 0;
  const float* row = sched + (size_t)t * LD_SCHED_COLS;
  const float c1 = row[LD_SCHED_COEF1], c2 = row[LD_SCHED_COEF2], sg = row[LD_SCHED_SIGMA];
  const bool draw = (t_ptr ? t > 0 : true) && z != nullptr;
  GRID_STRIDE(i, n) {
    const float mean = c1 * x0[i] + c2 * x[i];
    xp[i] = draw ? mean + sg * z[i] : mean;
  }
}
struct DdimK { float sr, srm1, sab, s1mab, san, c, sigma, lo, hi; int obj, last; };
__global__ void ddim_step_kernel(const float* x, const float* mo, const float* z, float* xn, DdimK k, long n) {
  GRID_STRIDE(i, n) {
    const float xi = x[i], m = mo[i];
    float x0;
    if (k.obj == LD_OBJ_X0) x0 = m;
    else if (k.obj == LD_OBJ_NOISE) x0 = k.sr * xi - k.srm1 * m;
    else x0 = k.sab * xi - k.s1mab * m;
    x0 = clampf(x0, k.lo, k.hi);
    if (k.last) { xn[i] = x0; continue; }
    const float eps = (k.sr * xi - x0) / k.srm1;
    xn[i] = x0 * k.san + k.c * eps + k.sigma * (z ? z[i] : 0.f);
  }
}

__global__ void ddim_step_at_kernel(const float* x, const float* mo, const float* z, float* xn, const float* table,
                                    const int* idx, float lo, float hi, int obj, long n) {
  const float* r = table + 8 * (size_t)(*idx);
  const float sr = r[0], srm1 = r[1], sab = r[2], s1mab = r[3], san = r[4], c = r[5], sigma = r[6];
  const bool last = r[7] != 0.0f;
  GRID_STRIDE(i, n) {
    const float xi = x[i], m = mo[i];
    float x0;
    if (obj == LD_OBJ_X0) x0 = m;
    else if (obj == LD_OBJ_NOISE) x0 = sr * xi - srm1 * m;
    else x0 = sab * xi - s1mab * m;
    x0 = clampf(x0, lo, hi);
    if (last) { xn[i] = x0; continue; }
    const float eps = (sr * xi - x0) / srm1;
    xn[i] = x0 * san + c * eps + sigma * (z ? z[i] : 0.f);
  }
}

__global__ void branch_cond_kernel(const float* cond, const float* mask, float* co, float* ci, float lo_clip,
                                   int C, int HW, long n) {
  GRID_STRIDE(i, n) {
    const long bc = i / HW, p = i - bc * HW, b = bc / C;
    const float bin = mask[b * HW + p] >= 1.0f ? 1.0f : 0.0f;
    const float c = cond[i];
    co[i] = c * bin;
    ci[i] = c * clampf(1.0f - bin, lo_clip, 1.0f);
  }
}
__global__ void mask_out_kernel(float* mo, const float* mask, float min_val, int C, int HW, long n) {
  GRID_STRIDE(i, n) {
    const long bc = i / HW, p = i - bc * HW, b = bc / C;
    const float bin = mask[b * HW + p] >= 1.0f ? 1.0f : 0.0f;
    mo[i] = (bin == 0.0f) ? min_val : mo[i] * bin;
  }
}
__global__ void fuse_ddpm_kernel(const float* xo, const float* xi, const float* x0o, const float* x0i,
                                 const float* mask, float* x, float* x0, float lo, float hi, int C, int HW, long n) {
  GRID_STRIDE(i, n) {
    const long bc = i / HW, p = i - bc * HW, b = bc / C;
    const float m = mask[b * HW + p] >= 1.0f ? 1.0f : 0.0f;
    x0[i] = clampf(clampf(x0i[i], lo, hi) * (1.0f - m) + clampf(x0o[i], lo, hi), lo, hi);
    const float a = xo[i] * m, c = xi[i] * (1.0f - m);
    x[i] = (a == 0.0f) ? c : a;
  }
}
__global__ void branch_cond_k_kernel(const float* cond, const float* masks, float* out, float lo_clip, int B, int C,
                                     int K, int HW, long n) {
  GRID_STRIDE(i, n) {
    const long bc = i / HW, p = i - bc * HW, b = bc / C;
    const float c = cond[i];
    for (int k = 0; k < K; ++k) {
      const float bin = masks[((size_t)b * K + k) * HW + p] >= 1.0f ? 1.0f : 0.0f;
      out[(size_t)k * n + i] = c * (k == 0 ? bin : clampf(bin, lo_clip, 1.0f));
    }
  }
}
__global__ void fuse_ddpm_k_kernel(const float* x_first, const float* x_rest, const float* x0_first, const float* x0_rest,
                                   const float* masks, float* x, float* x0, float lo, float hi, int C, int K, int HW, long n) {
  GRID_STRIDE(i, n) {
    const long bc = i / HW, p = i - bc * HW, b = bc / C;
    const float* mrow = masks + (size_t)b * K * HW + p;
    float m = mrow[HW] >= 1.0f ? 1.0f : 0.0f;
    float acc = clampf(x0_rest[i], lo, hi) * m;
    const float a0 = x_first[i] * (mrow[0] >= 1.0f ? 1.0f : 0.0f);
    float xv = (a0 == 0.0f) ? x_rest[i] * m : a0;
    for (int k = 2; k < K; ++k) {
      m = mrow[(size_t)k * HW] >= 1.0f ? 1.0f : 0.0f;
      acc += clampf(x0_rest[(size_t)(k - 1) * n + i], lo, hi) * m;
      if (xv == 0.0f) xv = x_rest[(size_t)(k - 1) * n + i] * m;
    }
    x0[i] = clampf(acc + clampf(x0_first[i], lo, hi), lo, hi);
    x[i] = xv;
  }
}
struct FuseDdimK { float sr, srm1, san, c, sigma, lo, hi; };
__global__ void fuse_ddim_kernel(const float* xo, const float* xi, const float* x0o, const float* x0i,
                                 const float* mask, const float* z, float* xn, FuseDdimK k, int C, int HW, long n) {
  GRID_STRIDE(i, n) {
    const long bc = i / HW, p = i - bc * HW, b = bc / C;
    const float m = mask[b * HW + p] >= 1.0f ? 1.0f : 0.0f;
    const float a0 = clampf(x0o[i], k.lo, k.hi), b0 = clampf(x0i[i], k.lo, k.hi);
    const float eo = (k.sr * xo[i] - a0) / k.srm1, ei = (k.sr * xi[i] - b0) / k.srm1;
    const float x0 = clampf((a0 == 0.0f) ? b0 : a0, k.lo, k.hi);
    const float po = eo * m, pi = ei * (1.0f - m);
    const float eps = (po == 0.0f) ? pi : po;
    xn[i] = x0 * k.san + k.c * eps + k.sigma * (z ? z[i] : 0.f);
  }
}
__global__ void fuse_ddim_k_kernel(const float* x_first, const float* x_rest, const float* x0_first, const float* x0_rest,
                                   const float* masks, const float* z, float* xn, FuseDdimK k, int C, int K, int HW, long n) {
  GRID_STRIDE(i, n) {
    const long bc = i / HW, p = i - bc * HW, b = bc / C;
    const float* mrow = masks + (size_t)b * K * HW + p;
    const float a0 = clampf(x0_first[i], k.lo, k.hi);
    const float e0 = (k.sr * x_first[i] - a0) / k.srm1;
    float eps = e0 * (mrow[0] >= 1.0f ? 1.0f : 0.0f);
    float alt = 0.f;
    bool have = false;
    for (int kk = 1; kk < K; ++kk) {
      const float m = mrow[(size_t)kk * HW] >= 1.0f ? 1.0f : 0.0f;
      const float ak = clampf(x0_rest[(size_t)(kk - 1) * n + i], k.lo, k.hi);
      const float ek = (k.sr * x_rest[(size_t)(kk - 1) * n + i] - ak) / k.srm1;
      if (!have && (m == 1.0f || kk == K - 1)) { alt = ak; have = true; }
      if (eps == 0.0f) eps = ek * m;
    }
    const float x0 = clampf((a0 == 0.0f) ? alt : a0, k.lo, k.hi);
    xn[i] = x0 * k.san + k.c * eps + k.sigma * (z ? z[i] : 0.f);
  }
}
__global__ void q_sample_kernel(const float* x0, const float* z, float* out, float sab, float s1mab, long n) {
  GRID_STRIDE(i, n) out[i] = sab * x0[i] + s1mab * z[i];
}
__global__ void q_sample_t_kernel(const float* x0, const float* z, float* out, const int* t, const float* sab, const float* s1mab,
                                  long per) {
  const int b = blockIdx.y;
  const float a = sab[t[b]], c = s1mab[t[b]];
  const long base = (long)b * per;
  for (long i = (long)blockIdx.x * blockDim.x + threadIdx.x; i < per; i += (long)gridDim.x * blockDim.x)
    out[base + i] = a * x0[base + i] + c * z[base + i];
}
__global__ __launch_bounds__(256) void p_losses_kernel(const float* mo, const float* x0, const float* z, const int* t,
                                                       const float* sab, const float* s1mab, const float* lw, float* loss,
                                                       long per, int objective) {
  __shared__ double s_part[256];
  const int b = blockIdx.x, tid = threadIdx.x;
  const int tb = t[b];
  const float a = sab[tb], c = s1mab[tb];
  const long base = (long)b * per;
  double acc = 0.0;
  for (long i = tid; i < per; i += 256) {
    const float xs = x0[base + i], nz = z[base + i];
    const float target = objective == LD_OBJ_NOISE ? nz : (objective == LD_OBJ_X0 ? xs : a * nz - c * xs);
    const float d = mo[base + i] - target;
    acc += (double)(d * d);
  }
  s_part[tid] = acc;
  __syncthreads();
  for (int s = 128; s > 0; s >>= 1) {
    if (tid < s) s_part[tid] += s_part[tid + s];
    __syncthreads();
  }
  if (tid == 0) loss[b] = (float)(s_part[0] / (double)per) * lw[tb];
}
__global__ void recompose_kernel(const float* patches, const float* masks, float* out, int K, int C, int HW, long n) {
  GRID_STRIDE(i, n) {
    const long bc = i / HW, p = i - bc * HW, b = bc / C, c = bc - b * C;
    float acc = 0.f;
    for (int k = 0; k < K; ++k) {
      const float m = masks[(size_t)k * HW + p] >= 1.0f ? 1.0f : 0.0f;
      acc += patches[(((size_t)b * K + k) * C + c) * HW + p] * m;
    }
    out[i] = acc;
  }
}

template <typename T>
__device__ __forceinline__ void final_conv_pixel(const T* xp, const float* s_w, int Cin, int Cout, float* acc) {
  constexpr int E = 16 / sizeof(T);
  acc[0] = acc[1] = acc[2] = acc[3] = 0.f;
  for (int c0 = 0; c0 < Cin; c0 += 4 * E) {
    uint4 raw[4];
#pragma unroll
    for (int q = 0; q < 4; ++q)
      raw[q] = (c0 + q * E < Cin) ? *reinterpret_cast<const uint4*>(xp + c0 + q * E) : make_uint4(0u, 0u, 0u, 0u);
#pragma unroll
    for (int q = 0; q < 4; ++q) {
      if (c0 + q * E >= Cin) break;
      float v[E];
      unpack16<T>(raw[q], v);
#pragma unroll
      for (int g = 0; g < E; g += 4) {
        const int c = c0 + q * E + g;
        for (int o = 0; o < Cout; ++o) {
          const float* wr = s_w + o * Cin + c;
          acc[o] = fmaf(v[g], wr[0], fmaf(v[g + 1], wr[1], fmaf(v[g + 2], wr[2], fmaf(v[g + 3], wr[3], acc[o]))));
        }
      }
    }
  }
}

template <typename T>
__global__ void final_conv_kernel(const T* __restrict__ x, const float* __restrict__ w, const float* __restrict__ bias,
                                  float* __restrict__ out, int HW, int Cin, int Cout, long npix) {
  extern __shared__ float s_fw[];
  for (int i = threadIdx.x; i < Cin * Cout; i += BS) s_fw[i] = w[i];
  __syncthreads();
  GRID_STRIDE(i, npix) {
    const long b = i / HW, p = i - b * HW;
    float acc[4];
    final_conv_pixel<T>(x + (size_t)i * Cin, s_fw, Cin, Cout, acc);
    for (int o = 0; o < Cout; ++o) out[((size_t)b * Cout + o) * HW + p] = acc[o] + bias[o];
  }
}

template <typename T>
__global__ void final_step_kernel(const T* __restrict__ x, const float* __restrict__ w, const float* __restrict__ bias,
                                  float* __restrict__ model_out, float* __restrict__ x_t, float* __restrict__ x0o,
                                  const float* __restrict__ sched, const int* __restrict__ t_ptr, float lo, float hi,
                                  int obj, unsigned long long seed, long stream_base, long stream_tmul, long first,
                                  const float* __restrict__ keep_mask, int HW, int Cin, int Cout, long npix) {
  extern __shared__ float s_fw[];
  for (int i = threadIdx.x; i < Cin * Cout; i += BS) s_fw[i] = w[i];
  const int t = t_ptr ? *t_ptr : 0;
  const long stream = stream_base + stream_tmul * (long)t;
  const float* row = sched + (size_t)t * LD_SCHED_COLS;
  const float c1 = row[LD_SCHED_COEF1], c2 = row[LD_SCHED_COEF2], sg = row[LD_SCHED_SIGMA];
  const unsigned long long base = mix64(seed ^ ((unsigned long long)stream * 0xD1B54A32D192ED03ull));
  __syncthreads();
  GRID_STRIDE(i, npix) {
    const long b = i / HW, p = i - b * HW;
    float acc[4];
    final_conv_pixel<T>(x + (size_t)i * Cin, s_fw, Cin, Cout, acc);
    const bool keep = keep_mask ? keep_mask[i] >= 1.0f : true;
    for (int o = 0; o < Cout; ++o) {
      const size_t idx = ((size_t)b * Cout + o) * HW + p;
      const float mo = keep ? acc[o] + bias[o] : lo;
      store_f32_out(&model_out[idx], mo);
      const float xi = x_t[idx];
      const float x0 = clampf(to_x0(xi, mo, row, obj), lo, hi);
      const float mean = c1 * x0 + c2 * xi;
      float r = mean;
      if (t > 0) {
        const unsigned long long h = mix64(base + (unsigned long long)(first + idx + 1) * 0x9E3779B97F4A7C15ull);
        const float u1 = ((float)(unsigned)(h >> 40) + 1.0f) * 5.9604644775390625e-8f;
        const float u2 = (float)(unsigned)((h >> 16) & 0xFFFFFFu) * 5.9604644775390625e-8f;
        r = mean + sg * (sqrtf(-2.0f * logf(u1)) * cosf(6.283185307179586f * u2));
      }
      store_f32_out(&x_t[idx], r);
      if (x0o) store_f32_out(&x0o[idx], x0);
    }
  }
}
}

#define ST(s) reinterpret_cast<hipStream_t>(s)

extern "C" int ld_randn_at(float* out, int64_t n, int64_t first, uint64_t seed, int64_t stream_base,
                           int64_t stream_tmul, const int32_t* t_ptr, void* stream) {
  LD_REQUIRE(out && n > 0 && first >= 0, "ld_randn: bad args");
  LD_LAUNCH(randn_kernel, dim3(nblocks(n)), dim3(BS), 0, ST(stream), out, (long)n, (long)first,
                     (unsigned long long)seed, (long)stream_base, (long)stream_tmul, t_ptr);
  LD_LAUNCH_CHECK("randn");
  return LD_OK;
}
extern "C" int ld_randn(float* out, int64_t n, uint64_t seed, int64_t stream_base, int64_t stream_tmul,
                        const int32_t* t_ptr, void* stream) {
  return ld_randn_at(out, n, 0, seed, stream_base, stream_tmul, t_ptr, stream);
}
extern "C" int ld_step_add(int32_t* t_ptr, int delta, void* stream) {
  LD_REQUIRE(t_ptr, "ld_step_add: null");
  LD_LAUNCH(step_add_kernel, dim3(1), dim3(64), 0, ST(stream), t_ptr, delta);
  LD_LAUNCH_CHECK("step_add");
  return LD_OK;
}
int ld_step_begin_check(const void* zero_a, size_t bytes_a, const void* zero_b, size_t bytes_b, const void* t_ptr, const void* idx_ptr,
                        const void* t_table, const void* film_rows, int row_floats, const void* film_cur) {
  LD_REQUIRE((idx_ptr == nullptr) == (t_table == nullptr), "ld_step_begin: idx_ptr and t_table go together");
  LD_REQUIRE((film_rows == nullptr) == (film_cur == nullptr), "ld_step_begin_film: film_rows and film_cur go together");
  LD_REQUIRE(!film_rows || (t_ptr && row_floats > 0 && row_floats % 4 == 0 && ((size_t)film_rows % 16) == 0 && ((size_t)film_cur % 16) == 0),
             "ld_step_begin_film: needs the step counter, row_floats %% 4 == 0 and 16-byte aligned rows");
  LD_REQUIRE((zero_a || bytes_a == 0) && (zero_b || bytes_b == 0), "ld_step_begin: null arena");
  LD_REQUIRE(bytes_a % 16 == 0 && bytes_b % 16 == 0 && ((size_t)zero_a % 16) == 0 && ((size_t)zero_b % 16) == 0,
             "ld_step_begin: arenas must be 16-byte aligned and sized");
  return LD_OK;
}
extern "C" int ld_step_begin(void* zero_a, size_t bytes_a, void* zero_b, size_t bytes_b, int32_t* t_ptr, int delta,
                             int32_t* idx_ptr, const int32_t* t_table, void* stream) {
  return ld_step_begin_film(zero_a, bytes_a, zero_b, bytes_b, t_ptr, delta, idx_ptr, t_table, nullptr, 0, nullptr, stream);
}
extern "C" int ld_step_begin_film(void* zero_a, size_t bytes_a, void* zero_b, size_t bytes_b, int32_t* t_ptr, int delta,
                                  int32_t* idx_ptr, const int32_t* t_table, const float* film_rows, int row_floats,
                                  float* film_cur, void* stream) {
  if (int rc = ld_step_begin_check(zero_a, bytes_a, zero_b, bytes_b, t_ptr, idx_ptr, t_table, film_rows, row_floats, film_cur)) return rc;
  const long na = (long)(bytes_a / 16), nb = (long)(bytes_b / 16);
  const StepBeginDev sb{(uint4*)zero_a, na, (uint4*)zero_b, nb, t_ptr, delta, idx_ptr, t_table, film_rows, row_floats, film_cur};
  LD_LAUNCH(step_begin_kernel, dim3(nblocks(na + nb + 1)), dim3(BS), 0, ST(stream), sb);
  LD_LAUNCH_CHECK("step_begin");
  return LD_OK;
}
extern "C" int ld_ddpm_step(const float* x_t, const float* model_out, const float* noise, float* x_prev,
                            float* x0_out, const float* sched, const int32_t* t_ptr, float lo, float hi,
                            int objective, int64_t n, void* stream) {
  LD_REQUIRE(x_t && model_out && x_prev && sched && n > 0, "ld_ddpm_step: null pointer");
  LD_REQUIRE(objective >= 0 && objective <= 2, "ld_ddpm_step: objective %d", objective);
  LD_LAUNCH(ddpm_step_kernel, dim3(nblocks(n)), dim3(BS), 0, ST(stream), x_t, model_out, noise, x_prev,
                     x0_out, sched, t_ptr, lo, hi, objective, (long)n);
  LD_LAUNCH_CHECK("ddpm_step");
  return LD_OK;
}
extern "C" int ld_posterior_step(const float* x_t, const float* x0, const float* noise, float* x_prev,
                                 const float* sched, const int32_t* t_ptr, int64_t n, void* stream) {
  LD_REQUIRE(x_t && x0 && x_prev && sched && n > 0, "ld_posterior_step: null pointer");
  LD_LAUNCH(posterior_step_kernel, dim3(nblocks(n)), dim3(BS), 0, ST(stream), x_t, x0, noise, x_prev,
                     sched, t_ptr, (long)n);
  LD_LAUNCH_CHECK("posterior_step");
  return LD_OK;
}
extern "C" int ld_ddim_step(const float* x_t, const float* model_out, const float* noise, float* x_next,
                            float sqrt_recip, float sqrt_recipm1, float sqrt_ab, float sqrt_1mab,
                            float sqrt_abar_next, float c, float sigma, float lo, float hi, int objective,
                            int last, int64_t n, void* stream) {
  LD_REQUIRE(x_t && model_out && x_next && n > 0, "ld_ddim_step: null pointer");
  DdimK k{sqrt_recip, sqrt_recipm1, sqrt_ab, sqrt_1mab, sqrt_abar_next, c, sigma, lo, hi, objective, last};
  LD_LAUNCH(ddim_step_kernel, dim3(nblocks(n)), dim3(BS), 0, ST(stream), x_t, model_out, noise, x_next, k, (long)n);
  LD_LAUNCH_CHECK("ddim_step");
  return LD_OK;
}
extern "C" int ld_ddim_step_at(const float* x_t, const float* model_out, const float* noise, float* x_next,
                               const float* pair_table, const int32_t* idx_ptr, float lo, float hi, int objective,
                               int64_t n, void* stream) {
  LD_REQUIRE(x_t && model_out && x_next && pair_table && idx_ptr && n > 0, "ld_ddim_step_at: null pointer");
  LD_REQUIRE(objective >= 0 && objective <= 2, "ld_ddim_step_at: objective %d", objective);
  LD_LAUNCH(ddim_step_at_kernel, dim3(nblocks(n)), dim3(BS), 0, ST(stream), x_t, model_out, noise, x_next, pair_table, idx_ptr,
            lo, hi, objective, (long)n);
  LD_LAUNCH_CHECK("ddim_step_at");
  return LD_OK;
}
extern "C" int ld_branch_conditions(const float* cond, const float* mask, float* cond_out, float* cond_in,
                                    float lo_clip, int B, int C, int HW, void* stream) {
  LD_REQUIRE(cond && mask && cond_out && cond_in, "ld_branch_conditions: null pointer");
  const long n = (long)B * C * HW;
  LD_LAUNCH(branch_cond_kernel, dim3(nblocks(n)), dim3(BS), 0, ST(stream), cond, mask, cond_out, cond_in, lo_clip, C, HW, n);
  LD_LAUNCH_CHECK("branch_conditions");
  return LD_OK;
}
extern "C" int ld_mask_out(float* model_out, const float* mask, float min_val, int B, int C, int HW, void* stream) {
  LD_REQUIRE(model_out && mask, "ld_mask_out: null pointer");
  const long n = (long)B * C * HW;
  LD_LAUNCH(mask_out_kernel, dim3(nblocks(n)), dim3(BS), 0, ST(stream), model_out, mask, min_val, C, HW, n);
  LD_LAUNCH_CHECK("mask_out");
  return LD_OK;
}
extern "C" int ld_fuse_ddpm(const float* x_out, const float* x_in, const float* x0_out, const float* x0_in,
                            const float* mask, float* x, float* x0, float lo, float hi, int B, int C, int HW,
                            void* stream) {
  LD_REQUIRE(x_out && x_in && x0_out && x0_in && mask && x && x0, "ld_fuse_ddpm: null pointer");
  const long n = (long)B * C * HW;
  LD_LAUNCH(fuse_ddpm_kernel, dim3(nblocks(n)), dim3(BS), 0, ST(stream), x_out, x_in, x0_out, x0_in, mask, x, x0, lo, hi, C, HW, n);
  LD_LAUNCH_CHECK("fuse_ddpm");
  return LD_OK;
}
extern "C" int ld_branch_conditions_k(const float* cond, const float* masks, float* cond_k, float lo_clip, int B, int C,
                                      int K, int HW, void* stream) {
  LD_REQUIRE(cond && masks && cond_k && K >= 2, "ld_branch_conditions_k: bad args (K >= 2)");
  const long n = (long)B * C * HW;
  LD_LAUNCH(branch_cond_k_kernel, dim3(nblocks(n)), dim3(BS), 0, ST(stream), cond, masks, cond_k, lo_clip, B, C, K, HW, n);
  LD_LAUNCH_CHECK("branch_conditions_k");
  return LD_OK;
}
extern "C" int ld_fuse_ddpm_k(const float* x_first, const float* x_rest, const float* x0_first, const float* x0_rest,
                              const float* masks, float* x, float* x0, float lo, float hi, int B, int C, int K, int HW,
                              void* stream) {
  LD_REQUIRE(x_first && x_rest && x0_first && x0_rest && masks && x && x0 && K >= 2, "ld_fuse_ddpm_k: bad args (K >= 2)");
  const long n = (long)B * C * HW;
  LD_LAUNCH(fuse_ddpm_k_kernel, dim3(nblocks(n)), dim3(BS), 0, ST(stream), x_first, x_rest, x0_first, x0_rest, masks, x, x0,
            lo, hi, C, K, HW, n);
  LD_LAUNCH_CHECK("fuse_ddpm_k");
  return LD_OK;
}
extern "C" int ld_fuse_ddim(const float* x_out, const float* x_in, const float* x0_out, const float* x0_in,
                            const float* mask, const float* noise, float* x_next, float sqrt_recip,
                            float sqrt_recipm1, float sqrt_abar_next, float c, float sigma, float lo, float hi,
                            int B, int C, int HW, void* stream) {
  LD_REQUIRE(x_out && x_in && x0_out && x0_in && mask && x_next, "ld_fuse_ddim: null pointer");
  const long n = (long)B * C * HW;
  FuseDdimK k{sqrt_recip, sqrt_recipm1, sqrt_abar_next, c, sigma, lo, hi};
  LD_LAUNCH(fuse_ddim_kernel, dim3(nblocks(n)), dim3(BS), 0, ST(stream), x_out, x_in, x0_out, x0_in, mask, noise, x_next, k, C, HW, n);
  LD_LAUNCH_CHECK("fuse_ddim");
  return LD_OK;
}
extern "C" int ld_fuse_ddim_k(const float* x_first, const float* x_rest, const float* x0_first, const float* x0_rest,
                              const float* masks, const float* noise, float* x_next, float sqrt_recip, float sqrt_recipm1,
                              float sqrt_abar_next, float c, float sigma, float lo, float hi, int B, int C, int K, int HW,
                              void* stream) {
  LD_REQUIRE(x_first && x_rest && x0_first && x0_rest && masks && x_next && K >= 2, "ld_fuse_ddim_k: bad args (K >= 2)");
  const long n = (long)B * C * HW;
  FuseDdimK k{sqrt_recip, sqrt_recipm1, sqrt_abar_next, c, sigma, lo, hi};
  LD_LAUNCH(fuse_ddim_k_kernel, dim3(nblocks(n)), dim3(BS), 0, ST(stream), x_first, x_rest, x0_first, x0_rest, masks, noise,
            x_next, k, C, K, HW, n);
  LD_LAUNCH_CHECK("fuse_ddim_k");
  return LD_OK;
}
// ... 78 lines not shown
```

localdiffusion-hallucination_amd/diffusion.py:

```python
import time

import torch
from torch import nn

from . import _cabi as cabi
from . import rng, schedule
from .tuning import Tuning, runtime_configured

_REPLACE_OUT = ("mnist", "mvtec", "oct", "imagenet")


class _Pace:

    def __init__(self, streams, ahead):
        self.streams, self.pending, self.ahead = streams, [], int(ahead)

    def step_enqueued(self):
        if self.ahead <= 0:
            return
        evs = [torch.cuda.Event() for _ in self.streams]
        for e, gs in zip(evs, self.streams):
            e.record(gs)
        self.pending.append(evs)
        if len(self.pending) > self.ahead:
            for e in self.pending.pop(0):
                e.synchronize()


def _align_streams(streams):
    evs = [torch.cuda.Event() for _ in streams]
    for ev, gs in zip(evs, streams):
        ev.record(gs)
    for i, gs in enumerate(streams):
        for j, ev in enumerate(evs):
            if j != i:
                gs.wait_event(ev)


_SIDE_STREAMS = {}


def _masked_stream(i, kind):
    if not kind:
        return None
    import ctypes as C
    hip = C.CDLL("libamdhip64.so")
    n, i = 256, i % 2
    pick = {"lo": lambda b: b // 128 == i, "xcd": lambda b: (b % 8) // 4 == i, "even": lambda b: b % 2 == i}[kind]
    words = (C.c_uint32 * (n // 32))()
    for b in range(n):
        if pick(b):
            words[b // 32] |= 1 << (b % 32)
    st = C.c_void_p()
    rc = hip.hipExtStreamCreateWithCUMask(C.byref(st), C.c_uint32(n // 32), words)
    if rc != 0:
        raise RuntimeError(f"hipExtStreamCreateWithCUMask failed: {rc}")
    return torch.cuda.ExternalStream(st.value)


def _low_priority_stream():
    import ctypes as C
    hip = C.CDLL("libamdhip64.so")
    least, greatest = C.c_int(), C.c_int()
    rc = hip.hipDeviceGetStreamPriorityRange(C.byref(least), C.byref(greatest))
    st = C.c_void_p()
    if rc == 0:
        rc = hip.hipStreamCreateWithPriority(C.byref(st), C.c_uint(1), least)
    if rc != 0:
        raise RuntimeError(f"hipStreamCreateWithPriority failed: {rc}")
    return torch.cuda.ExternalStream(st.value)


class _SubBatches:

    def __init__(self, gd, jp, S, shared_noise=False, masked=(), instance_base=0):
        self.gd, self.jp, self.S = gd, jp, S
        if not runtime_configured() and not getattr(_SubBatches, "_warned", False):
            _SubBatches._warned = True
            import warnings
            warnings.warn("graph-replay sampling without localdiffusion_hallucination_amd.configure_runtime(): the HIP "
                          "runtime's captured AQL packets make replayed steps 1-5 % slower (call it before the first "
                          "GPU call of the process; INTEGRATION.md)", RuntimeWarning, stacklevel=3)
        B, _, H, W = jp.x_in.shape
        self.b = B // S
        self.plans = [gd.model.plan(self.b, H, W, table_T=gd.num_timesteps_ori, instance=instance_base + i + 1)
                      for i in range(S)]
        self.streams = gd._sub_streams(S)
        self.shared_noise = shared_noise
        self.masks = {i: torch.ones(self.b, H * W, dtype=torch.float32, device=jp.x_in.device) for i in masked}
        self.graphs = {}
        self.cond_seen = None

    def set_mask(self, mask):
        for m in self.masks.values():
            m.copy_(mask.reshape(m.shape))

    def _step(self, i, st, lo, hi, base):
        gd, sp = self.gd, self.plans[i]
        lib = cabi.lib()
        xa, wf, bf = sp.final
        B_, C_, H_, W_ = sp.model_out.shape
        sp.run_main(st, skip_final=True, step_delta=-1)
        cabi.check(lib.ld_final_step_at(xa.data_ptr(), wf.data_ptr(), bf.data_ptr(), sp.model_out.data_ptr(),
                                        sp.x_in.data_ptr(), None, gd._sched_table().data_ptr(), sp.t_dev.data_ptr(),
                                        lo, hi, cabi.OBJ[gd.objective], gd.noise_seed, base, -1,
                                        gd.noise_offset + (0 if self.shared_noise else i * sp.x_in.numel()),
                                        cabi.ptr(self.masks.get(i)),
                                        B_, H_, W_, wf.shape[1], C_, sp.dt, st), "final_step")

    def _ensure_graph(self, i, gs, lo, hi, base):
        import ctypes as C
        lib, st = cabi.lib(), gs.cuda_stream
        key = (i, float(lo), float(hi), base, self.gd.noise_seed, self.gd.noise_offset)
        if key in self.graphs:
            return 0
        ran = 0
        if not getattr(self, "_warm", False) and not any(k[0] == i for k in self.graphs):
            self._step(i, st, lo, hi, base)
            ran = 1
        gs.synchronize()
        cabi.check(lib.ld_graph_begin(st), "graph_begin")
        try:
            self._step(i, st, lo, hi, base)
        finally:
            g = C.c_void_p()
            rc = lib.ld_graph_end(st, C.byref(g))
        cabi.check(rc, "graph_end")
        self.graphs[key] = g
        return ran

    def _ensure_joint_graph(self, lo, hi, base):
        import ctypes as C
        lib = cabi.lib()
        key = ("joint", float(lo), float(hi), base, self.gd.noise_seed, self.gd.noise_offset)
        if key in self.graphs:
            return self.graphs[key]
        s0 = self.streams[0]
        for gs in self.streams:
            gs.synchronize()
        fork = torch.cuda.Event()
        joins = [torch.cuda.Event() for _ in self.streams[1:]]
        cabi.check(lib.ld_graph_begin(s0.cuda_stream), "graph_begin")
        try:
            fork.record(s0)
            for gs in self.streams[1:]:
                gs.wait_event(fork)
            for i, gs in enumerate(self.streams):
                with torch.cuda.stream(gs):
                    self._step(i, gs.cuda_stream, lo, hi, base)
            for ev, gs in zip(joins, self.streams[1:]):
                ev.record(gs)
                s0.wait_event(ev)
        finally:
            g = C.c_void_p()
            rc = lib.ld_graph_end(s0.cuda_stream, C.byref(g))
        cabi.check(rc, "graph_end")
        self.graphs[key] = g
        return g

    def _trim(self, lo, hi, base):
        if (0, float(lo), float(hi), base, self.gd.noise_seed, self.gd.noise_offset) in self.graphs or len(self.graphs) < 8 * self.S:
            return
        torch.cuda.synchronize()
        for g in self.graphs.values():
            cabi.lib().ld_graph_destroy(g)
        self.graphs.clear()
        self._warm = True

    def run(self, t_start, n_steps, lo, hi, draw):
        lib, jp, b = cabi.lib(), self.jp, self.b
        cur = torch.cuda.current_stream()
        base = draw + t_start
        self._trim(lo, hi, base)
        recond = self.cond_seen != getattr(jp, "cond_version", 0)
        self.cond_seen = getattr(jp, "cond_version", 0)
        todo, ex = [n_steps] * self.S, [None] * self.S
        for i, (sp, gs) in enumerate(zip(self.plans, self.streams)):
            gs.wait_stream(cur)
            st = gs.cuda_stream
            with torch.cuda.stream(gs):
                sp.x_in.copy_(jp.x_in[i * b:(i + 1) * b])
                if recond:
                    sp.cond_in.copy_(jp.cond_in[i * b:(i + 1) * b])
                    sp.run_cond_replayed(gs)
                sp.set_step(t_start + 1)
                todo[i] -= self._ensure_graph(i, gs, lo, hi, base)
                ex[i] = self.graphs[(i, float(lo), float(hi), base, self.gd.noise_seed, self.gd.noise_offset)]
        h0 = time.perf_counter()
        tn = self.gd.tuning
        if tn.sub_joint_graph and self.S > 1 and min(todo) == max(todo):
            gj = self._ensure_joint_graph(lo, hi, base)
            s0 = self.streams[0]
            for gs in self.streams[1:]:
                s0.wait_stream(gs)
            pace = _Pace(self.streams[:1], tn.sub_ahead)
            lib.ld_range_push(b"steps (one forked graph per step, %d sub-batches)" % self.S)
            for k in range(todo[0]):
                cabi.check(lib.ld_graph_launch(gj, s0.cuda_stream), "graph_launch")
                pace.step_enqueued()
            lib.ld_range_pop()
            for gs in self.streams[1:]:
                gs.wait_stream(s0)
            todo = [0] * self.S
        pace = _Pace(self.streams, tn.sub_ahead)
        lib.ld_range_push(b"steps (graph replay, %d sub-batches)" % self.S)
        for k in range(max(todo)):
            if self.S > 1 and tn.sub_resync > 0 and (k % tn.sub_resync == 0 or k <= tn.sub_resync_early) and k < min(todo):
                _align_streams(self.streams)
            for i, gs in enumerate(self.streams):
                if k < todo[i]:
                    cabi.check(lib.ld_graph_launch(ex[i], gs.cuda_stream), "graph_launch")
            pace.step_enqueued()
        lib.ld_range_pop()
        self.host_launch_s = getattr(self, "host_launch_s", 0.0) + time.perf_counter() - h0
        self.host_launch_n = getattr(self, "host_launch_n", 0) + sum(todo)
        for i, (sp, gs) in enumerate(zip(self.plans, self.streams)):
            with torch.cuda.stream(gs):
                jp.x_in[i * b:(i + 1) * b].copy_(sp.x_in)
            cur.wait_stream(gs)
        return draw + min(n_steps, t_start)

    def run_timed(self, t_start, n_steps, lo, hi, draw, acc):
        lib, jp, b, gd = cabi.lib(), self.jp, self.b, self.gd
        cur = torch.cuda.current_stream()
        base = draw + t_start
        self._trim(lo, hi, base)
        sched, obj = gd._sched_table(), cabi.OBJ[gd.objective]
        for i, (sp, gs) in enumerate(zip(self.plans, self.streams)):
            gs.wait_stream(cur)
            with torch.cuda.stream(gs):
                sp.x_in.copy_(jp.x_in[i * b:(i + 1) * b])
                sp.set_step(t_start + (1 if i > 0 else 0))
        for i in range(1, self.S):
            with torch.cuda.stream(self.streams[i]):
                self._ensure_graph(i, self.streams[i], lo, hi, base)
            g = self.graphs[(i, float(lo), float(hi), base, self.gd.noise_seed, self.gd.noise_offset)]
            for _ in range(n_steps + 2):
                cabi.check(lib.ld_graph_launch(g, self.streams[i].cuda_stream), "graph_launch")
        sp, gs = self.plans[0], self.streams[0]
        z = torch.empty_like(sp.x_in)
        with torch.cuda.stream(gs):
            st = gs.cuda_stream
            for k in range(n_steps):
                sp.set_step(t_start - k)
                sp.run_main_timed(st, acc)
                cabi.check(lib.ld_randn_at(z.data_ptr(), z.numel(), gd.noise_offset, gd.noise_seed, base, -1, sp.t_dev.data_ptr(), st), "randn")
                if 0 in self.masks:
                    cabi.check(lib.ld_mask_out(sp.model_out.data_ptr(), self.masks[0].data_ptr(), lo, sp.x_in.shape[0],
                                               sp.x_in.shape[1], z.shape[2] * z.shape[3], st), "mask_out")
                cabi.check(lib.ld_ddpm_step(sp.x_in.data_ptr(), sp.model_out.data_ptr(), z.data_ptr(), sp.x_in.data_ptr(),
                                            None, sched.data_ptr(), sp.t_dev.data_ptr(), lo, hi, obj, z.numel(), st), "ddpm_step")
        for gs in self.streams:
            cur.wait_stream(gs)
        torch.cuda.synchronize()
        return draw + min(n_steps, t_start)


class _DdimBranches:

    def __init__(self, gd, B, H, W, mask_x, times, pair_rows, shared=True):
        self.gd, self.B, self.mask_x, self.shared = gd, B, mask_x and shared, shared
        dev = gd.device
        self.plans = [gd.model.plan(B, H, W, table_T=gd.num_timesteps_ori, instance=200 + i) for i in range(2)]
        self.streams = gd._sub_streams(2)
        self.idx = [torch.zeros(1, dtype=torch.int32, device=dev) for _ in range(2)]
        self.times = torch.tensor(times, dtype=torch.int32, device=dev)
        self.table = torch.tensor(pair_rows, dtype=torch.float32, device=dev).contiguous()
        self.mask = torch.ones(B, H * W, dtype=torch.float32, device=dev)
        self.z = [torch.zeros(B, gd.channels, H, W, dtype=torch.float32, device=dev) for _ in range(2)]
        self.with_noise = any(r[6] != 0.0 for r in pair_rows)
        self.graphs = {}

    def _step(self, i, st, lo, hi):
        gd, sp, lib = self.gd, self.plans[i], cabi.lib()
        B, C, H, W = sp.model_out.shape
        n = sp.x_in.numel()
        sp.run_main(st, idx_ptr=self.idx[i].data_ptr(), t_table=self.times.data_ptr())
        if i == 0 and self.mask_x:
            cabi.check(lib.ld_mask_out(sp.model_out.data_ptr(), self.mask.data_ptr(), lo, B, C, H * W, st), "mask_out")
        zp = None
        if self.with_noise:
            first = gd.noise_offset + (0 if self.shared else i * n)
            cabi.check(lib.ld_randn_at(self.z[i].data_ptr(), n, first, gd.noise_seed, 1, 1, self.idx[i].data_ptr(), st), "randn")
            zp = self.z[i].data_ptr()
        cabi.check(lib.ld_ddim_step_at(sp.x_in.data_ptr(), sp.model_out.data_ptr(), zp, sp.x_in.data_ptr(), self.table.data_ptr(),
                                       self.idx[i].data_ptr(), lo, hi, cabi.OBJ[gd.objective], n, st), "ddim_step_at")

    @torch.inference_mode()
    def run_timed(self, n_steps, acc, lo, hi, alone=False):
        lib = cabi.lib()
        cur = torch.cuda.current_stream()
        g1 = next((g for k, g in self.graphs.items() if k[0] == 1), None)
        for gs in self.streams:
            gs.wait_stream(cur)
        if g1 is not None and not alone:
            self.idx[1].fill_(0)
            for _ in range(n_steps + 2):
                cabi.check(lib.ld_graph_launch(g1, self.streams[1].cuda_stream), "graph_launch")
        sp, gs = self.plans[0], self.streams[0]
        with torch.cuda.stream(gs):
            for k in range(n_steps):
                sp.set_step(int(self.times[min(k, len(self.times) - 1)]))
                sp.run_main_timed(gs.cuda_stream, acc)
        for gs in self.streams:
            cur.wait_stream(gs)
        torch.cuda.synchronize()

    def run(self, x_out, x_in, cond_out, cond_in, mask, first_pair, n_steps, lo, hi):
        import ctypes as C
        lib = cabi.lib()
        cur = torch.cuda.current_stream()
        if mask is not None:
            self.mask.copy_(mask.reshape(self.mask.shape))
        todo, ex = [n_steps, n_steps], [None, None]
        for i, (sp, gs, xv, cv) in enumerate(zip(self.plans, self.streams, (x_out, x_in), (cond_out, cond_in))):
            gs.wait_stream(cur)
            st = gs.cuda_stream
            with torch.cuda.stream(gs):
                sp.x_in.copy_(xv)
                sp.cond_in.copy_(cv)
                sp.run_cond_replayed(gs)
                self.idx[i].fill_(first_pair - 1)
                key = (i, float(lo), float(hi), gd_key(self.gd), self.shared)
                if key not in self.graphs:
                    self._step(i, st, lo, hi)
                    todo[i] -= 1
                    gs.synchronize()
                    cabi.check(lib.ld_graph_begin(st), "graph_begin")
                    try:
                        self._step(i, st, lo, hi)
                    finally:
                        g = C.c_void_p()
                        rc = lib.ld_graph_end(st, C.byref(g))
                    cabi.check(rc, "graph_end")
                    self.graphs[key] = g
                ex[i] = self.graphs[key]
        pace = _Pace(self.streams, self.gd.tuning.sub_ahead)
        for k in range(max(todo)):
            for i, gs in enumerate(self.streams):
                if k < todo[i]:
                    cabi.check(lib.ld_graph_launch(ex[i], gs.cuda_stream), "graph_launch")
            pace.step_enqueued()
        for sp, gs, xv in zip(self.plans, self.streams, (x_out, x_in)):
            with torch.cuda.stream(gs):
                xv.copy_(sp.x_in)
            cur.wait_stream(gs)


def gd_key(gd):
    return (gd.noise_seed, gd.noise_offset, gd.objective)


class GaussianDiffusion(nn.Module):
    def __init__(self, config, model, *, image_size, timesteps=1000, sampling_timesteps=None,
                 objective="pred_v", beta_schedule="sigmoid", schedule_fn_kwargs=dict(),
                 ddim_sampling_eta=0.0, auto_normalize=False, offset_noise_strength=0.0,
                 min_snr_loss_weight=False, min_snr_gamma=5):
        super().__init__()
        assert not (type(self) == GaussianDiffusion and model.channels != model.out_dim)
        assert not model.random_or_learned_sinusoidal_cond
        assert objective in {"pred_noise", "pred_x0", "pred_v"}
        self.auto_normalize = bool(auto_normalize)
        self.config = config
        self.branch_out = bool(config["branch_out"])
        self.start_intermediate = bool(config["start_intermediate"])
        self.model = model
        self.channels = model.channels
        self.self_condition = model.self_condition
        self.image_size = image_size
        self.objective = objective
        bufs = schedule.make_buffers(timesteps, beta_schedule, objective, min_snr_loss_weight,
                                     min_snr_gamma, **schedule_fn_kwargs)
        for k, v in bufs.items():
            self.register_buffer(k, v)
        self.num_timesteps = int(timesteps)
        self.num_timesteps_ori = int(timesteps)
        self.sampling_timesteps = timesteps if sampling_timesteps is None else sampling_timesteps
        assert self.sampling_timesteps <= timesteps
        self.is_ddim_sampling = self.sampling_timesteps < timesteps
        self.ddim_sampling_eta = ddim_sampling_eta
        self.offset_noise_strength = offset_noise_strength
        self.cnt = -1
        self.instance = 0
        self.classifier = None
        self.classifier_flag = 0
        self.pred_cls = 0.0
        self.classifier_calls = 0
        self.first_call_semantics = False
        self._mask_x_carried = None
        self._mask_x_cfg_seen = None
        self._all_ones_forced = None
        self.tuning = getattr(model, "tuning", None) or Tuning.from_env()
        self.noise_source = "device"
        self.fuse_final_step = bool(self.tuning.fused_final_step)
        self.noise_seed = 10
        self.noise_offset = 0
        self.use_graph = False
        self.sub_batches = int(self.tuning.sub_batches)
        self.min_sub_batch = int(self.tuning.min_sub_batch)
        self.sub_cu_mask = None
        self._sched = None
        self._graphs = {}
        self._subs = {}

    def call_classifier(self):
        if self.config.get("classifier", False) and self.classifier is None:
            raise RuntimeError("config['classifier'] is on: assign a callable x0 -> (score, _, _) to "
                               ".classifier before sampling (the reference's PatchCore weights are not shipped)")

    @property
    def device(self):
        return self.betas.device

    def _st(self):
        return torch.cuda.current_stream().cuda_stream

    def _sched_table(self):
        if self._sched is None or self._sched.device != self.device:
            cols = [self.posterior_mean_coef1, self.posterior_mean_coef2,
                    (0.5 * self.posterior_log_variance_clipped).exp(),
                    self.sqrt_recip_alphas_cumprod, self.sqrt_recipm1_alphas_cumprod,
                    self.sqrt_alphas_cumprod, self.sqrt_one_minus_alphas_cumprod, self.alphas_cumprod]
            self._sched = torch.stack([c.to(torch.float32) for c in cols], dim=1).contiguous()
        return self._sched

    def _noise(self, buf, k, t_dev=None):
        src = self.noise_source
        if callable(src):
            buf.copy_(src(tuple(buf.shape), k).to(buf.device, torch.float32))
        elif src == "host":
            buf.copy_(torch.from_numpy(rng.randn(tuple(buf.shape), self.noise_seed, k, self.noise_offset)))
        elif src == "device":
            cabi.check(cabi.lib().ld_randn_at(buf.data_ptr(), buf.numel(), self.noise_offset, self.noise_seed, k, 0,
                                              None, self._st()), "randn")
        else:
            raise ValueError(f"noise_source {src!r}")

    def _mask_x_get(self):
        cfgv = bool(self.config.get("mask_x", False))
        if self.first_call_semantics or self._mask_x_carried is None or cfgv != self._mask_x_cfg_seen:
            self._mask_x_carried = None
            return cfgv
        return self._mask_x_carried

    def _mask_x_set(self, v):
        if not self.first_call_semantics:
            self._mask_x_carried = bool(v)
            self._mask_x_cfg_seen = bool(self.config.get("mask_x", False))

    def reset_call_state(self):
        self._mask_x_carried, self._mask_x_cfg_seen = None, None
        self.classifier_flag = 0

    def advance_call_state(self, mask):
        c = self.config
        self.cnt += 1
        if bool(c.get("ood_AD", False)) or bool(c.get("ood_confidence", False)):
            self._mask_x_set(True)
        branch_cfg = bool(c["branch_out"]) or self.branch_out
        fuse_cfg = bool(c["start_intermediate"]) or self.start_intermediate
        if branch_cfg and self._all_ones(mask):
            self._mask_x_set(False)
        elif branch_cfg and fuse_cfg and mask is not None:
            self._mask_x_set(False)

    def _all_ones(self, mask):
        if self._all_ones_forced is not None:
            return self._all_ones_forced
        if mask is None or mask.shape[1] != 1:
            return False
        u = torch.unique(mask)
        return len(u) == 1 and float(u[0]) == 1.0

    def _flags(self, mask):
        c = self.config
        branch = bool(c["branch_out"]) or self.branch_out
        fuse = bool(c["start_intermediate"]) or self.start_intermediate
        mask_x = self._mask_x_get() or bool(c.get("ood_AD", False)) or bool(c.get("ood_confidence", False))
        if branch and self._all_ones(mask):
            branch, fuse, mask_x = False, False, False
        return branch, fuse, mask_x

    def result_layout(self, mask):
        branch, fuse, _ = self._flags(mask)
        if self.is_ddim_sampling:
            return "list" if (branch and not fuse) else "plain"
        start_int = bool(self.config["start_intermediate"]) or self.start_intermediate
        return "stacked" if ((not start_int) and self.branch_out) else "plain"

    def _replaced_out(self, mask_x):
        d = self.config["data"]
        return mask_x and any(k in d for k in _REPLACE_OUT) and "mri" not in d

    @torch.inference_mode()
    def sample(self, cond_img, gt, batch_size=16, return_all_timesteps=False, return_all_outputs=False,
               mask=None, ood_confidence_ad=False, min_max_val=None, instance=0):
        self.instance = instance
        self.cnt += 1
        self.min_max_val = min_max_val
        self.hr = gt
        c = self.config
        if bool(c.get("ood_AD", False)) or bool(c.get("ood_confidence", False)):
            self._mask_x_set(True)
        branch_cfg = bool(c["branch_out"]) or self.branch_out
        decided_here = branch_cfg and self._all_ones_forced is None
        if decided_here:
            self._all_ones_forced = self._all_ones(mask)
        try:
            if branch_cfg and self._all_ones_forced:
                self._mask_x_set(False)
            shape = (batch_size, self.channels, self.image_size, self.image_size)
            if self.is_ddim_sampling:
                return self.unnormalize(self.ddim_sample(cond_img, mask, min_max_val, shape, return_all_timesteps=return_all_timesteps))
            out = self.p_sample_loop(cond_img, mask, min_max_val, shape, return_all_timesteps=return_all_timesteps,
                                     return_all_outputs=return_all_outputs)
            if return_all_outputs:
                return (self.unnormalize(out[0]),) + tuple(out[1:])
            return self.unnormalize(out)
        finally:
            if decided_here:
                self._all_ones_forced = None

    @torch.inference_mode()
    def p_sample(self, x, mask, min_max_val, cond_img, t: int, x_self_cond=None, draw=None):
        lib, st = cabi.lib(), self._st()
        B, C, H, W = x.shape
        model_out = self.model(x, cond_img, torch.full((B,), t, device=x.device, dtype=torch.long))
        z = torch.empty_like(x)
        if t > 0:
            if draw is None:
                draw = self._p_sample_draw = getattr(self, "_p_sample_draw", 0) + 1
            self._noise(z, int(draw))
        x_prev, x0 = torch.empty_like(x), torch.empty_like(x)
        row = self._sched_table()[t:t + 1].contiguous()
        cabi.check(lib.ld_ddpm_step(x.data_ptr(), model_out.data_ptr(), z.data_ptr() if t > 0 else None, x_prev.data_ptr(),
                                    x0.data_ptr(), row.data_ptr(), None, float(min_max_val[0]),
                                    float(min_max_val[1]), cabi.OBJ[self.objective], x.numel(), st), "ddpm_step")
        return x_prev, x0

    def normalize(self, x):
        return x * 2 - 1 if self.auto_normalize else x

    def unnormalize(self, x):
        if not self.auto_normalize:
            return x
        if isinstance(x, (list, tuple)):
            raise TypeError("can only concatenate list (not \"int\") to list")
        return (x + 1) * 0.5

    @torch.inference_mode()
    def q_sample(self, x_start, t, noise=None):
        x0 = x_start.to(self.device, torch.float32).contiguous()
        if noise is None:
            noise = torch.empty_like(x0)
            self._train_draw = getattr(self, "_train_draw", -1) + 1
            self._noise(noise, self._train_draw)
        noise = noise.to(self.device, torch.float32).contiguous()
        t32 = t.to(self.device, torch.int32).contiguous()
        out = torch.empty_like(x0)
        cabi.check(cabi.lib().ld_q_sample_t(x0.data_ptr(), noise.data_ptr(), out.data_ptr(), t32.data_ptr(),
                                            self.sqrt_alphas_cumprod.data_ptr(), self.sqrt_one_minus_alphas_cumprod.data_ptr(),
                                            x0.shape[0], x0[0].numel(), self._st()), "q_sample_t")
        return out

    @torch.inference_mode()
    def p_losses(self, x_start, cond_img, t, noise=None, offset_noise_strength=None, per_sample=False):
        assert not self.self_condition
        lib, st, dev = cabi.lib(), self._st(), self.device
        x0 = x_start.to(dev, torch.float32).contiguous()
        B = x0.shape[0]
        if noise is None:
            noise = torch.empty_like(x0)
            self._train_draw = getattr(self, "_train_draw", -1) + 1
            self._noise(noise, self._train_draw)
        noise = noise.to(dev, torch.float32).contiguous()
        strength = self.offset_noise_strength if offset_noise_strength is None else offset_noise_strength
        if strength > 0.0:
            off = torch.empty(B, x0.shape[1], dtype=torch.float32, device=dev)
            self._train_draw = getattr(self, "_train_draw", -1) + 1
            self._noise(off, self._train_draw)
            noise = (noise + strength * off[:, :, None, None]).contiguous()
        x = self.q_sample(x0, t, noise)
        model_out = self.model(x, cond_img.to(dev, torch.float32), t.to(dev, torch.long)).contiguous()
        t32 = t.to(dev, torch.int32).contiguous()
        loss = torch.empty(B, dtype=torch.float32, device=dev)
        cabi.check(lib.ld_p_losses(model_out.data_ptr(), x0.data_ptr(), noise.data_ptr(), t32.data_ptr(),
                                   self.sqrt_alphas_cumprod.data_ptr(), self.sqrt_one_minus_alphas_cumprod.data_ptr(),
                                   self.loss_weight.data_ptr(), loss.data_ptr(), B, x0[0].numel(), cabi.OBJ[self.objective], st),
                   "p_losses")
        total = loss.mean()
        return (total, loss) if per_sample else total

    def forward(self, img, cond_img, train, *args, **kwargs):
        b, c, h, w = img.shape
        assert h == self.image_size and w == self.image_size, f"height and width of image must be {self.image_size}"
        if not train:
            torch.random.manual_seed(42)
        t = torch.randint(0, self.num_timesteps, (b,)).long()
        return self.p_losses(self.normalize(img), cond_img, t, *args, **kwargs)

    def _sync_model(self):
        v = getattr(self.model, "_version", 0)
        if v == getattr(self, "_model_version", None):
            return
        self._model_version = v
        if self._graphs or self._subs:
            torch.cuda.synchronize()
        for g in self._graphs.values():
            cabi.lib().ld_graph_destroy(g)
        self._graphs = {}
        for sub in self._subs.values():
            for g in sub.graphs.values():
                cabi.lib().ld_graph_destroy(g)
            sub.graphs = {}
        self._subs = {}

    def _sub_ok(self, b, H, W):
        return b * H * W >= self.min_sub_batch * 256 * 256 or b >= 2 * self.min_sub_batch

    def _sub_streams(self, S):
        key = (torch.cuda.current_device(), self.sub_cu_mask)
        pool = _SIDE_STREAMS.setdefault(key, [])
        while len(pool) < S:
            pool.append(_masked_stream(len(pool), self.sub_cu_mask) or _low_priority_stream())
        return pool[:S]

    def timed_plan(self, jp):
        sub = self._subs.get((id(jp), self.sub_batches))
        return sub.plans[0] if sub is not None else jp

    def _will_sub_batch(self, jp, n_steps, x0_buf=None, after=None, timers=None):
        S, B_ = self.sub_batches, jp.x_in.shape[0]
        return (S > 1 and B_ % S == 0 and (B_ // S >= self.min_sub_batch or self._sub_ok(B_ // S, *jp.x_in.shape[2:]))
                and self.noise_source == "device" and x0_buf is None and after is None and timers is None and n_steps >= 4
                and not self.use_graph and jp.x_in.shape[1] == jp.model_out.shape[1])

    def encode_cond(self, jp, n_steps, x0_buf=None, after=None):
        if self._will_sub_batch(jp, n_steps, x0_buf, after):
            jp.cond_version = getattr(jp, "cond_version", 0) + 1
        else:
            jp.run_cond(self._st())

    def run_joint_steps(self, jp, t_start, n_steps, lo, hi, z, draw, x0_buf=None, after=None, timers=None):
        self._sync_model()
        lib, st = cabi.lib(), self._st()
        sched = self._sched_table()
        obj = cabi.OBJ[self.objective]
        n = jp.x_in.numel()
        B_ = jp.x_in.shape[0]
        S = self.sub_batches
        if self._will_sub_batch(jp, n_steps, x0_buf, after, timers):
            key = (id(jp), S)
            if key not in self._subs:
                self._subs[key] = _SubBatches(self, jp, S)
            return self._subs[key].run(t_start, n_steps, lo, hi, draw)
        if timers is not None and (id(jp), S) in self._subs and x0_buf is None and after is None:
            return self._subs[(id(jp), S)].run_timed(t_start, n_steps, lo, hi, draw, timers)
        if (self.use_graph and self.noise_source == "device" and x0_buf is None and after is None
                and timers is None and n_steps > 1):
            return self._run_joint_steps_graph(jp, t_start, n_steps, lo, hi, z, draw)
        t = t_start
        fused = (self.noise_source == "device" and timers is None and self.fuse_final_step
                 and jp.x_in.shape[1] == jp.model_out.shape[1])
        if fused:
            xa, wf, bf = jp.final
            B_, C_, H_, W_ = jp.model_out.shape
            for _ in range(n_steps):
                jp.set_step(t)
                jp.run_main(st, skip_final=True)
                k = draw if t > 0 else 0
                cabi.check(lib.ld_final_step_at(xa.data_ptr(), wf.data_ptr(), bf.data_ptr(), jp.model_out.data_ptr(),
                                                jp.x_in.data_ptr(), cabi.ptr(x0_buf), sched.data_ptr(), jp.t_dev.data_ptr(),
                                                lo, hi, obj, self.noise_seed, k, 0, self.noise_offset, None,
                                                B_, H_, W_, wf.shape[1], C_, jp.dt, st), "final_step")
                if t > 0:
                    draw += 1
                if after is not None:
                    after(t)
                t -= 1
            return draw
        for _ in range(n_steps):
            jp.set_step(t)
            if timers is None:
                jp.run_main(st)
            else:
                jp.run_main_timed(st, timers)
            if t > 0:
                self._noise(z, draw)
                draw += 1
            cabi.check(lib.ld_ddpm_step(jp.x_in.data_ptr(), jp.model_out.data_ptr(), z.data_ptr(),
                                        jp.x_in.data_ptr(), cabi.ptr(x0_buf), sched.data_ptr(),
                                        jp.t_dev.data_ptr(), lo, hi, obj, n, st), "ddpm_step")
            if after is not None:
                after(t)
            t -= 1
        return draw

    def _run_joint_steps_graph(self, jp, t_start, n_steps, lo, hi, z, draw):
        import ctypes as C
        lib = cabi.lib()
        sched = self._sched_table()
        obj = cabi.OBJ[self.objective]
        n = jp.x_in.numel()
        base = draw + t_start
        key = (id(jp), float(lo), float(hi), obj, base, z.data_ptr(), self.noise_seed, self.noise_offset)
        cur = torch.cuda.current_stream()
        if getattr(self, "_gstream", None) is None:
            self._gstream = torch.cuda.Stream()
        gs = self._gstream
        gs.wait_stream(cur)
        st = gs.cuda_stream
        first = key not in self._graphs
        t = t_start
        with torch.cuda.stream(gs):
            if first:
                jp.set_step(t)
                jp.run_main(st)
                cabi.check(lib.ld_randn_at(z.data_ptr(), n, self.noise_offset, self.noise_seed, base, -1, jp.t_dev.data_ptr(), st), "randn")
                cabi.check(lib.ld_ddpm_step(jp.x_in.data_ptr(), jp.model_out.data_ptr(), z.data_ptr(), jp.x_in.data_ptr(),
                                            None, sched.data_ptr(), jp.t_dev.data_ptr(), lo, hi, obj, n, st), "ddpm_step")
                t -= 1
                n_steps -= 1
                gs.synchronize()
                cabi.check(lib.ld_graph_begin(st), "graph_begin")
                try:
                    jp.run_main(st)
                    cabi.check(lib.ld_randn_at(z.data_ptr(), n, self.noise_offset, self.noise_seed, base, -1, jp.t_dev.data_ptr(), st), "randn")
                    cabi.check(lib.ld_ddpm_step(jp.x_in.data_ptr(), jp.model_out.data_ptr(), z.data_ptr(),
                                                jp.x_in.data_ptr(), None, sched.data_ptr(), jp.t_dev.data_ptr(),
                                                lo, hi, obj, n, st), "ddpm_step")
                    cabi.check(lib.ld_step_add(jp.t_dev.data_ptr(), -1, st), "step_add")
                finally:
                    ex = C.c_void_p()
                    rc = lib.ld_graph_end(st, C.byref(ex))
                cabi.check(rc, "graph_end")
                self._graphs[key] = ex
            ex = self._graphs[key]
            if n_steps > 0:
                jp.set_step(t)
                for _ in range(n_steps):
                    cabi.check(lib.ld_graph_launch(ex, st), "graph_launch")
        cur.wait_stream(gs)
        return draw + (t_start - t) + n_steps

    @torch.inference_mode()
    def p_sample_loop(self, cond_img, mask, min_max_val, shape, return_all_timesteps=False,
                      return_all_outputs=False):
        self._sync_model()
        lib, st, dev = cabi.lib(), self._st(), self.device
        B, C, H, W = shape
        HW, n = H * W, B * C * H * W
        lo, hi = float(min_max_val[0]), float(min_max_val[1])
        T = self.num_timesteps
        branch, fuse, mask_x = self._flags(mask)
        obj = cabi.OBJ[self.objective]
        sched = self._sched_table()
        cond = cond_img.to(dev, torch.float32).contiguous()
        if mask is not None:
            mask = mask.to(dev, torch.float32).contiguous()
        start_t = T - 1
        x_T = torch.empty(shape, dtype=torch.float32, device=dev)
        self._noise(x_T, 0)
        if (bool(self.config["start_intermediate"]) or self.start_intermediate) and self.config.get("use_gt", False):
            t0 = int(self.config["use_gt_timestep"])
            hr = self.hr.to(dev, torch.float32).contiguous()
            cabi.check(lib.ld_q_sample(hr.data_ptr(), x_T.data_ptr(), x_T.data_ptr(),
                                       float(self.sqrt_alphas_cumprod[t0]),
                                       float(self.sqrt_one_minus_alphas_cumprod[t0]), n, st), "q_sample")
            start_t = t0 - 1
        z = torch.empty(shape, dtype=torch.float32, device=dev)
        if branch and mask is not None and mask.shape[1] > 1:
            if return_all_timesteps:
                raise TypeError("return_all_timesteps is only defined for the single-branch reverse process "
                                "(the reference's torch.stack(imgs) fails on the per-branch lists, ddpm.py:865,963)")
            return self._p_sample_loop_kmask(cond, mask, lo, hi, shape, x_T, z, start_t, fuse, mask_x,
                                             return_all_outputs=return_all_outputs)
        x0_buf = torch.empty(shape, dtype=torch.float32, device=dev) if return_all_outputs else None
        if return_all_timesteps and branch:
            raise TypeError("return_all_timesteps is only defined for the single-branch reverse process "
                            "(the reference's torch.stack(imgs) fails on the per-branch lists, ddpm.py:865,963)")
        hist_x, hist_x0 = [x_T.clone()] if return_all_timesteps else None, []
        x0_pair = [torch.empty(shape, dtype=torch.float32, device=dev) for _ in range(2)] if (return_all_outputs and branch) else None
        draw = 1
        t = start_t
        xs = None
        gate = bool(self.config.get("classifier", False)) and branch and fuse
        if gate:
            self.call_classifier()
        x_branchout = None
        if branch:
            assert self.objective == "pred_x0", "branch mode exists only for pred_x0 (ddpm.py:739-749)"
            assert mask is not None
            if mask_x:
                assert len(torch.unique((mask >= 1.0).float())) == 2, "mask should be binary"
            lo_clip = 0.5 if self.config["data"] == "mnist" else 0.95
            cond_out, cond_in = torch.empty_like(cond), torch.empty_like(cond)
            cabi.check(lib.ld_branch_conditions(cond.data_ptr(), mask.data_ptr(), cond_out.data_ptr(),
                                                cond_in.data_ptr(), lo_clip, B, cond.shape[1], HW, st), "branch_conditions")
            replaced = self._replaced_out(mask_x)
            nb = B if replaced else 2 * B
            plan = self.model.plan(nb, H, W, table_T=self.num_timesteps_ori)
            if replaced:
                plan.cond_in.copy_(cond_in)
            else:
                plan.cond_in[:B].copy_(cond_out)
                plan.cond_in[B:].copy_(cond_in)
            plan.run_cond(st)
            x_in_view = plan.x_in if replaced else plan.x_in[B:]
            x_out_view = torch.empty(shape, dtype=torch.float32, device=dev) if replaced else plan.x_in[:B]
            x_out_view.copy_(x_T)
            x_in_view.copy_(x_T)
            mo_in = plan.model_out if replaced else plan.model_out[B:]
            mo_out = cond_out if replaced else plan.model_out[:B]
            n_plain = (t - int(self.config["start_timestep"])) if fuse else t + 1
            if (not replaced and self.sub_batches > 1 and (B >= self.min_sub_batch or self._sub_ok(B, H, W))
                    and self.noise_source == "device"
                    and not return_all_timesteps and not return_all_outputs and n_plain >= 4
                    and C == plan.model_out.shape[1] and not self.use_graph):
                key = (id(plan), "branch", bool(mask_x))
                if key not in self._subs:
                    self._subs[key] = _SubBatches(self, plan, 2, shared_noise=True, masked=(0,) if mask_x else (),
                                                  instance_base=100)
                if mask_x:
                    self._subs[key].set_mask(mask)
                draw = self._subs[key].run(t, n_plain, lo, hi, draw)
                t -= n_plain
            while t >= 0:
# ... 696 lines not shown
```

localdiffusion-hallucination_amd/unet.py:

```python
import ctypes as C
import math

import numpy as np
import torch
from torch import nn

from . import _cabi as cabi
from .pool import check_declared, intervals_from_declared, peak_live, place_intervals
from .tuning import Tuning
from .weights import UnetConfig, unet_param_shapes

_TORCH_DT = {"fp32": torch.float32, "bf16": torch.bfloat16, "fp16": torch.float16}
_LOWP = ("bf16", "fp16")


def _register(root: nn.Module, dotted: str, tensor: torch.Tensor):
    parts = dotted.split(".")
    mod = root
    for name in parts[:-1]:
        if name not in mod._modules:
            mod.add_module(name, nn.Module())
        mod = mod._modules[name]
    mod.register_parameter(parts[-1], nn.Parameter(tensor, requires_grad=False))

# ... 430 lines not shown
        def stale(v):
            return isinstance(v, int) and not isinstance(v, bool) and owner(v) is not None
        cur = [0]

        def still(obj, name, k, delta):
            raise RuntimeError(f"pool: launch {cur[0]} ({op_names[cur[0]]}) field {name} still points into the old allocation of {buf_names[k]}")
        for i, op in enumerate(self.ops_main):
            cur[0] = i
            for v in held(op):
                if hasattr(v, "_obj"):
                    scan_struct(v._obj, still)
                vals = list(v) if isinstance(v, (tuple, list)) else (list(v.values()) if isinstance(v, dict) else [v])
                for e in vals:
                    if stale(e):
                        raise RuntimeError(f"pool: launch {i} ({op_names[i]}) holds the old address of {buf_names[owner(e)]} as a plain integer")
                for t in tensors(v):
                    if t.is_cuda and owner(t.data_ptr()) is not None:
                        raise RuntimeError(f"pool: launch {i} ({op_names[i]}) holds a tensor that was not re-pointed at the pool")
        self.named = {k: v for k, v in self.named.items() if id(v) not in pooled}
        peak = peak_live(size, first, last)
        self.pool_stats = dict(buffers=len(bufs), bytes_unshared=sum(size), bytes_pool=top, bytes_peak_live=peak)
        self.pool_intervals = [(first[k], last[k], offset[k], size[k]) for k in range(len(bufs))]
        if self.tn.pool_verify:
            dying = {}
            for k in range(len(bufs)):
                if 0 <= last[k] < n_ops:
                    dying.setdefault(last[k], []).append((base + offset[k], size[k]))
            lib = self.lib
            for i, regions in dying.items():
                def poisoned(st, op=self.ops_main[i], regions=tuple(regions)):
                    op(st)
                    for ptr, nbytes in regions:
                        cabi.check(lib.ld_memset_bytes(ptr, 0xFF, nbytes, st), "pool verify")
                self.ops_main[i] = poisoned
            self.pool_stats["verify_poisoned_buffers"] = sum(len(r) for r in dying.values())

    def slot(self):
        s = self._slot_cursor
        self._slot_cursor += 1
        assert s < self.stats.shape[0]
        return self.stats[s]

    def t_ptr(self):
        return None

    def src(self, t, c, stride=0, ups=0, gn=None, act=cabi.ACT_NONE, film=None):
        s = cabi.Src()
        s.data, s.C, s.pix_stride, s.upsample = t.data_ptr(), c, stride, ups
        if gn is not None:
            stats, gamma, beta, groups = gn
            s.gn_stats, s.gn_gamma, s.gn_beta, s.gn_groups = stats.data_ptr(), gamma.data_ptr(), beta.data_ptr(), groups
        s.act = act
        if film is not None and self.table_T:
            s.film = self.film_cur.data_ptr() + 4 * self._film_off[id(film)]
            s.film_tstride = s.film_bstride = 0
        elif film is not None:
            s.film = film.data_ptr()
            s.film_tstride = 0
            s.film_bstride = 2 * c
        self.keep.append(t)
        s._tensor = t
        return s

    def _call(self, ops, fn, args, what, meta=None, reads=(), writes=()):
        self.keep.append(args)
        ref = C.byref(args)
        ops.append(lambda st, fn=fn, ref=ref, what=what: cabi.check(fn(ref, st), what))
        if ops is self.ops_main:
            self.meta[len(ops) - 1] = dict(what=what, **(meta or {}))
            self.decl[len(ops) - 1] = ([t for t in reads if t is not None], [t for t in writes if t is not None])

    def _raw(self, ops, fn, what, nbytes=0, flops=0, reads=(), writes=()):
        ops.append(fn)
        if ops is self.ops_main:
            self.meta[len(ops) - 1] = dict(what=what, family=what, bytes=nbytes, flops=flops)
            self.decl[len(ops) - 1] = ([t for t in reads if t is not None], [t for t in writes if t is not None])

    def conv3(self, ops, srcs, wname, cout, h, w, stats=None, groups=8, weight=None, bias=None, addend=None, side=None):
        a = cabi.Conv3x3Args()
        for i, s in enumerate(srcs):
            a.src[i] = s
        a.nsrc = len(srcs)
        weight = self.P["w"][wname + ".weight"] if weight is None else weight
        bias = self.f32[wname + ".bias"] if bias is None else bias
        a.weight, a.bias = weight.data_ptr(), bias.data_ptr()
        a.weight_terms = 2 if weight.data_ptr() in self.P["terms2"] else 1
        a.addend = cabi.ptr(addend)
        self.keep += [weight, bias, addend]
        out = self.buf(h, w, cout)
        a.out = out.data_ptr()
        side_out = None
        if side is not None:
            side_out = self.buf(h, w, cout)
            a.side_weight, a.side_bias, a.side_out = side[0].data_ptr(), side[1].data_ptr(), side_out.data_ptr()
            self.keep += [side[0], side[1]]
        if stats is not None:
            a.out_stats, a.out_groups = stats.data_ptr(), groups
        a.B, a.H, a.W, a.Cout = self.B, h, w, cout
        a.t_ptr = self.t_ptr()
        a.dtype = self.dt
        cin = sum(s.C for s in srcs)
        npx = self.B * h * w
        mt4 = cout % 64 == 0 and ((w + 15) // 16) * ((h + 7) // 8) * (cout // 64) * self.B >= 256
        blocks16 = ((w + 15) // 16) * ((h + 15) // 16) * (cout // (64 if mt4 else 32)) * self.B
        big = blocks16 >= 512 and h >= 16 and not mt4
        big = big or (mt4 and h >= 16 and blocks16 >= self._kt("conv_big4_min"))
        dname = {cabi.LD_F32: "f32", cabi.LD_BF16: "bf16", cabi.LD_F16: "f16"}[self.dt]
        if side is not None:
            big = False
        fam = f"conv3x3<{dname},{4 if mt4 else 2},{4 if big else 2}>"
        ck = 16 if self.dt == cabi.LD_F32 else 32
        if side is not None:
            pass
        elif (cout == 32 and len(srcs) == 1 and cin == ck and addend is None and h >= 32 and w >= 32 and h % 16 == 0
                and w % 16 == 0 and (w // 16) * (h // 16) * self.B >= self._kt("conv_c32_min_tiles")
                and self._kt("conv_c32") and a.weight_terms != 2):
            fam = f"conv3x3_c32<{dname}>"
        elif (self.dt != cabi.LD_F32 and cout == 32 and addend is None and a.weight_terms != 2 and h % 16 == 0 and w % 16 == 0
              and (w // 16) * (h // 16) * self.B >= self._kt("conv_s32_min_tiles") and not any(s.upsample for s in srcs)
              and cin in (32, 64) and (len(srcs) == 1 or all(s.C == 32 for s in srcs)) and groups in (1, 2, 4, 8)):
            pro = any(s.gn_stats for s in srcs)
            bit = 2 if pro else (1 if cin == 32 else 4)
            if (self._kt("conv_s32") & bit) and (not pro or (len(srcs) == 1 and srcs[0].C == 32 and srcs[0].gn_groups == 8)):
                fam = f"conv3x3_s32<{dname}>"
        in_el = sum(s.C * (npx // 4 if s.upsample else npx) for s in srcs)
        side_b = (in_el + npx * cout + cin * cout) * self.esize + 4 * cout if side is not None else 0
        self._call(ops, self.lib.ld_conv3x3, a, "conv3x3 " + wname + (" + res_conv" if side is not None else ""),
                   dict(family=fam, bytes=(in_el + npx * cout + 9 * cin * cout) * self.esize + 4 * cout + side_b,
                        flops=2 * (9 + (1 if side is not None else 0)) * cin * cout * npx, shape=f"{cin}->{cout}@{h}x{w}"),
                   reads=[s._tensor for s in srcs] + [addend], writes=[out, side_out])
        return out if side is None else (out, side_out)

    def conv1(self, ops, srcs, weight, cout, h, w, bias=None, epi=cabi.EPI_PLAIN, unshuffle=0, rms_in=0,
              bstride=0, g2=None, residual=None, what="conv1x1", out=None, kmax_out=None, gn_tail=None):
        a = cabi.Conv1x1Args()
        for i, s in enumerate(srcs):
            a.src[i] = s
        a.nsrc, a.unshuffle, a.rms_in = len(srcs), unshuffle, rms_in
        a.weight, a.weight_bstride = weight.data_ptr(), bstride
        a.weight_terms = 2 if weight.data_ptr() in self.P["terms2"] else 1
        a.bias = cabi.ptr(bias)
        a.epilogue, a.hidden, a.q_scale = epi, self.cfg.hidden, self.cfg.attn_dim_head ** -0.5
        a.g2, a.residual = cabi.ptr(g2), cabi.ptr(residual)
        a.kmax_out = cabi.ptr(kmax_out)
        if gn_tail is not None:
            a.gn_tail = gn_tail
        out = self.buf(h, w, cout) if out is None else out
        a.out = out.data_ptr()
        a.B, a.H, a.W, a.Cout, a.dtype = self.B, h, w, cout, self.dt
        self.keep += [weight, bias, g2, residual]
        cin = sum(s.C for s in srcs) * (4 if unshuffle else 1)
        npx = self.B * h * w
        el = npx * cin + npx * cout + cin * cout * (self.B if bstride else 1) + (npx * cout if (residual is not None or gn_tail is not None) else 0)
        self._call(ops, self.lib.ld_conv1x1, a, what,
                   dict(family="conv1x1", bytes=el * self.esize, flops=2 * cin * cout * npx, shape=f"{cin}->{cout}@{h}x{w}"),
                   reads=[s._tensor for s in srcs] + [residual, gn_tail._tensor if gn_tail is not None else None], writes=[out])
        return out

    def gn_apply(self, ops, a_src, b_src, h, w, c, final_act=cabi.ACT_NONE, pool=0):
        g = cabi.GnApplyArgs()
        g.a = a_src
        if b_src is not None:
            g.b = b_src
        g.final_act, g.pool = final_act, pool
        out = self.buf(h // 2 if pool else h, w // 2 if pool else w, c)
        g.out = out.data_ptr()
        g.B, g.H, g.W, g.t_ptr, g.dtype = self.B, h, w, self.t_ptr(), self.dt
        nel = self.B * h * w * c
        self._call(ops, self.lib.ld_gn_apply, g, "gn_apply",
                   dict(family="gn_apply", bytes=(nel * (2 if b_src is not None else 1) + nel // (4 if pool else 1)) * self.esize, flops=0),
                   reads=[a_src._tensor, b_src._tensor if b_src is not None else None], writes=[out])
        return out

    def _build_time(self):
        cfg, f, lib = self.cfg, self.f32, self.lib
        if self.table_T:
            times = torch.arange(self.table_T, dtype=torch.int32, device=self.dev)
        else:
            times = self.times
        self.keep.append(times)
        freqs = self.P["freqs"]
        n, td = self.rows, cfg.time_dim
        if cfg.learned_sinusoidal_dim:
            wts = f["time_mlp.0.weights"]
            self.ops_time.append(lambda st: cabi.check(lib.ld_time_mlp_fourier(
                times.data_ptr(), n, wts.data_ptr(), cfg.learned_sinusoidal_dim, f["time_mlp.1.weight"].data_ptr(),
                f["time_mlp.1.bias"].data_ptr(), f["time_mlp.3.weight"].data_ptr(), f["time_mlp.3.bias"].data_ptr(),
                td, self.temb.data_ptr(), st), "time_mlp (learned Fourier features)"))
        else:
            self.ops_time.append(lambda st: cabi.check(lib.ld_time_mlp(
                times.data_ptr(), n, freqs.data_ptr(), cfg.dim, f["time_mlp.1.weight"].data_ptr(),
                f["time_mlp.1.bias"].data_ptr(), f["time_mlp.3.weight"].data_ptr(), f["time_mlp.3.bias"].data_ptr(),
                td, self.temb.data_ptr(), st), "time_mlp"))
        for name in f:
            if name.endswith(".mlp.1.weight") and not name.startswith("conv_fusion"):
                p = name[:-len(".mlp.1.weight")]
                two_c = f[name].shape[0]
                film = torch.zeros(n, two_c, dtype=torch.float32, device=self.dev)
                self.films[p] = film
                self._film_off[id(film)] = self.film_row
                self.film_row += two_c
                w, b = f[name], f[p + ".mlp.1.bias"]
                self.ops_time.append(lambda st, w=w, b=b, film=film, two_c=two_c: cabi.check(lib.ld_film(
                    self.temb.data_ptr(), n, td, w.data_ptr(), b.data_ptr(), two_c, film.data_ptr(), st), "film"))

    def resnet_block(self, ops, p, srcs_fn, cin_total, cout, h, w, res_tensor=None):
        f, G = self.f32, self.cfg.resnet_block_groups
        s1, s2 = self.slot(), self.slot()
        wres = self.P["w"].get(p + ".res_conv.weight")
        side = None
        px_ok = (h * w in self.tn.side_res_conv_px) if self.tn.side_res_conv_px is not None else h * w <= self.tn.side_res_conv_max_px
        if (wres is not None and self.tn.side_res_conv and self.dt != cabi.LD_F32 and px_ok and self.net.weight_split_levels == 0
                and wres.data_ptr() not in self.P["terms2"] and self.P["w"][p + ".block1.proj.weight"].data_ptr() not in self.P["terms2"]):
            side = (wres, f[p + ".res_conv.bias"])
        rc = None
        if side is not None:
            raw1, rc = self.conv3(ops, srcs_fn(), p + ".block1.proj", cout, h, w, stats=s1, groups=G, side=side)
        else:
            raw1 = self.conv3(ops, srcs_fn(), p + ".block1.proj", cout, h, w, stats=s1, groups=G)
        film = self.films.get(p)
        n1 = self.src(raw1, cout, gn=(s1, f[p + ".block1.norm.weight"], f[p + ".block1.norm.bias"], G),
                      act=cabi.ACT_SILU, film=film)
        if self._separate_act(h * w, cout):
            act1 = self.gn_apply(ops, n1, None, h, w, cout)
            n1 = self.src(act1, cout)
        raw2 = self.conv3(ops, [n1], p + ".block2.proj", cout, h, w, stats=s2, groups=G)
        n2 = self.src(raw2, cout, gn=(s2, f[p + ".block2.norm.weight"], f[p + ".block2.norm.bias"], G),
                      act=cabi.ACT_SILU)
        if rc is not None:
            out = self.gn_apply(ops, n2, self.src(rc, cout), h, w, cout)
        elif (p + ".res_conv.weight") in f:
            out = self.conv1(ops, srcs_fn(), self.P["w"][p + ".res_conv.weight"], cout, h, w,
                             bias=f[p + ".res_conv.bias"], epi=cabi.EPI_GN_TAIL, gn_tail=n2, what="res_conv+tail " + p)
        else:
            assert res_tensor is not None and cin_total == cout
            out = self.gn_apply(ops, n2, self.src(res_tensor, cout), h, w, cout)
        self.named[p] = out
        return out

    def fusion_block_folded(self, ops, x, c, h, w):
        f, G, p = self.f32, self.cfg.resnet_block_groups, "conv_fusion"
        p1, p2, zero = self.fusion_const
        s1, s2 = self.slot(), self.slot()
        raw1 = self.conv3(ops, [self.src(x, c)], p + ".block1.proj", c, h, w, stats=s1, groups=G,
                          weight=self.P["w"][p + ".block1.proj.weight#x"], bias=zero, addend=p1)
        n1 = self.src(raw1, c, gn=(s1, f[p + ".block1.norm.weight"], f[p + ".block1.norm.bias"], G),
                      act=cabi.ACT_SILU, film=self.films.get(p))
        if self._separate_act(h * w, c):
            n1 = self.src(self.gn_apply(ops, n1, None, h, w, c), c)
        raw2 = self.conv3(ops, [n1], p + ".block2.proj", c, h, w, stats=s2, groups=G)
        n2 = self.src(raw2, c, gn=(s2, f[p + ".block2.norm.weight"], f[p + ".block2.norm.bias"], G), act=cabi.ACT_SILU)
        out = self.conv1(ops, [self.src(x, c)], self.P["w"][p + ".res_conv.weight#x"], c, h, w, bias=None,
                         epi=cabi.EPI_GN_TAIL, gn_tail=n2, residual=p2, what="res_conv+tail " + p)
        self.named[p] = out
        return out

    def linear_attention_fused(self, ops, p, x, c, h, w):
        f, cfg, lib = self.f32, self.cfg, self.lib
        n, hid, B, heads, dt, es = h * w, cfg.hidden, self.B, cfg.attn_heads, self.dt, self.esize
        rule = self.tn.chunk_rule(B)
        chunk_px = rule[0] if n >= 65536 else (rule[1] if n >= 16384 else rule[2])
        nchunks = max(1, min(128, n // chunk_px)) if heads == 4 else max(1, min(32, n // 256))
        if heads == 4 and self.tn.linattn_chunk_px is None:
            while B * nchunks < 512 and nchunks < 512 and n // (2 * nchunks) >= 256:
                nchunks *= 2
        ctx = self._tracked(torch.empty(int(lib.ld_linattn_ctx_part_floats(B, heads, 32, nchunks)), dtype=torch.float32, device=self.dev))
        wfold = self._tracked(torch.empty(B, c * hid, dtype=self.tdt, device=self.dev))
        wout = f[p + ".to_out.0.weight"].reshape(c, hid).contiguous()
        wq, wkv = self.P["wq"][p], self.P["wkv"][p]
        kshift = self.P["kshift"].get(p) if heads == 4 else None
        ksp = kshift.data_ptr() if kshift is not None else None
        qshift = self.P["qshift"].get(p) if heads == 4 else None
        qsp = qshift.data_ptr() if qshift is not None else None
        bias, g2 = f[p + ".to_out.0.bias"], self.P["g2"][p + ".to_out.1.g"]
        out = self.buf(h, w, c)
        self.keep += [ctx, wfold, wout, wq, wkv, kshift, qshift, bias, g2, out, x]
        npx = B * n
        terms = self.P.get("attn_terms", {}).get(p, 1)
        self._raw(ops, lambda st: cabi.check(lib.ld_linattn_kvctx_terms(x.data_ptr(), wkv.data_ptr(), ksp, ctx.data_ptr(), B, n, c,
                                                                        heads, 32, nchunks, dt, terms, st), "linattn_kvctx"),
                  "linattn_kvctx", nbytes=npx * c * es, flops=2 * npx * c * 2 * hid * (1 if kshift is not None else 2) + 2 * npx * hid * 32,
                  reads=[x], writes=[ctx])
        self._raw(ops, lambda st: cabi.check(lib.ld_linattn_ctxfold(ctx.data_ptr(), nchunks, wout.data_ptr(), wfold.data_ptr(), B, c,
                                                                    heads, 32, 1, dt, st), "linattn_ctxfold"),
                  "linattn_ctxfold", nbytes=B * c * hid * es, flops=2 * B * c * hid * 32, reads=[ctx], writes=[wfold])
        scale = cfg.attn_dim_head ** -0.5
        self._raw(ops, lambda st: cabi.check(lib.ld_linattn_out_terms(x.data_ptr(), wq.data_ptr(), qsp, wfold.data_ptr(), bias.data_ptr(),
                                                                      g2.data_ptr(), out.data_ptr(), B, n, c, scale, dt, terms, st),
                                             "linattn_out"),
                  "linattn_out", nbytes=2 * npx * c * es, flops=2 * npx * hid * c * 2, reads=[x, wfold], writes=[out])
        return out

    def linear_attention(self, ops, p, x, c, h, w):
        if self.dt != cabi.LD_F32 and c in (32, 64, 128) and p in self.P["wq"]:
            return self.linear_attention_fused(ops, p, x, c, h, w)
        f, cfg, lib = self.f32, self.cfg, self.lib
        n, hid, B = h * w, cfg.hidden, self.B
        kmax = self.kmax_arena[self._kmax_cursor]
        self._kmax_cursor += 1
        qkv = self.conv1(ops, [self.src(x, c)], self.P["w"][p + ".to_qkv.weight"], 3 * hid, h, w,
                         epi=cabi.EPI_QKV_LINEAR, rms_in=1, what="to_qkv " + p, kmax_out=kmax)
        nchunks = max(1, min(32, n // 256))
        ctx = torch.empty(int(lib.ld_linattn_ctx_part_floats(B, cfg.attn_heads, 32, nchunks)),
                          dtype=torch.float32, device=self.dev)
        wfold = torch.empty(B, c * hid, dtype=self.tdt, device=self.dev)
        wout = f[p + ".to_out.0.weight"].reshape(c, hid).contiguous()
# ... 2 lines not shown
        es = self.esize
        self._raw(ops, lambda st: cabi.check(lib.ld_linattn_ctx(qkv.data_ptr(), kmax.data_ptr(), ctx.data_ptr(),
                                                                B, n, heads, 32, nchunks, dt, st), "linattn_ctx"),
                  "linattn_ctx", nbytes=2 * B * n * hid * es, flops=2 * B * n * hid * 32, reads=[qkv], writes=[ctx])
        self._raw(ops, lambda st: cabi.check(lib.ld_linattn_ctxfold(ctx.data_ptr(), nchunks, wout.data_ptr(), wfold.data_ptr(),
                                                                    B, c, heads, 32, 0, dt, st), "linattn_ctxfold"),
                  "linattn_ctxfold", nbytes=B * c * hid * es, flops=2 * B * c * hid * 32, reads=[ctx], writes=[wfold])
        q = self.src(qkv, hid, stride=3 * hid)
        return self.conv1(ops, [q], wfold, c, h, w, bias=f[p + ".to_out.0.bias"], epi=cabi.EPI_RMS_RES,
                          bstride=c * hid * self.esize, g2=self.P["g2"][p + ".to_out.1.g"], residual=x,
                          what="lin to_out " + p)

    def full_attention(self, ops, p, x, c, h, w):
        f, cfg, lib = self.f32, self.cfg, self.lib
        n, hid, B = h * w, cfg.hidden, self.B
        qkv = self.conv1(ops, [self.src(x, c)], self.P["w"][p + ".to_qkv.weight"], 3 * hid, h, w,
                         epi=cabi.EPI_QKV_FULL, rms_in=1, what="to_qkv " + p)
        att = self.buf(h, w, hid)
        dt, heads = self.dt, cfg.attn_heads
        self.keep += [qkv, att]
        self._raw(ops, lambda st: cabi.check(lib.ld_attention(qkv.data_ptr(), att.data_ptr(), B, n, heads, 32, dt, st),
                                             "attention"),
                  "attention", nbytes=4 * B * n * hid * self.esize, flops=4 * B * n * n * hid, reads=[qkv], writes=[att])
        return self.conv1(ops, [self.src(att, hid)], self.P["w"][p + ".to_out.weight"], c, h, w,
                          bias=f[p + ".to_out.bias"], epi=cabi.EPI_RES, residual=x, what="full to_out " + p)

    def attention(self, ops, p, x, c, h, w, full):
        out = (self.full_attention if full else self.linear_attention)(ops, p, x, c, h, w)
        self.named[p] = out
        return out

    def _basic_block(self, ops, p, x, cin, cmid, cout, h, w, pool, image=False):
        f, lib, G = self.f32, self.lib, 16
        s1, s2, s3 = self.slot(), self.slot(), self.slot()

        def image_conv(wname, c_out, stats):
            out = self.buf(h, w, c_out)
            wt, bs = f[wname + ".weight"], f[wname + ".bias"]
            B, dt = self.B, self.dt
            self.keep += [out, wt, bs]
            ops.append(lambda st: cabi.check(lib.ld_conv_image(
                self.cond_in.data_ptr(), wt.data_ptr(), bs.data_ptr(), out.data_ptr(), stats.data_ptr(), G,
                B, cin, h, w, 3, dt, st), "conv_image " + wname))
            return out

        if image:
            a1 = image_conv(p + ".convblock.0", cmid, s1)
            idr = image_conv(p + ".identity.0", cout, s3)
        else:
            a1 = self.conv3(ops, [self.src(x, cin)], p + ".convblock.0", cmid, h, w, stats=s1, groups=G)
            idr = self.conv3(ops, [self.src(x, cin)], p + ".identity.0", cout, h, w, stats=s3, groups=G)
        n1 = self.src(a1, cmid, gn=(s1, f[p + ".convblock.1.weight"], f[p + ".convblock.1.bias"], G),
                      act=cabi.ACT_RELU)
        a2 = self.conv3(ops, [n1], p + ".convblock.3", cout, h, w, stats=s2, groups=G)
        na = self.src(a2, cout, gn=(s2, f[p + ".convblock.4.weight"], f[p + ".convblock.4.bias"], G))
        nb = self.src(idr, cout, gn=(s3, f[p + ".identity.1.weight"], f[p + ".identity.1.bias"], G))
        return self.gn_apply(ops, na, nb, h, w, cout, final_act=cabi.ACT_RELU, pool=1 if pool else 0)

    def _build_cond(self):
        cfg, ops, H, W = self.cfg, self.ops_cond, self.H, self.W
        x = self._basic_block(ops, "cond_model.residual_conv1.0", None, cfg.cond_in_channels, 32, 32, H, W,
                              pool=True, image=True)
        x = self._basic_block(ops, "cond_model.residual_conv2.0", x, 32, 32, 64, H // 2, W // 2, pool=True)
        early = cfg.cond_early_exit
        x = self._basic_block(ops, "cond_model.residual_conv3.0", x, 64, 64, 128, H // 4, W // 4, pool=not early)
        if early:
            return x
        return self._basic_block(ops, "cond_model.mid_conv.0", x, 128, 128, 256, H // 8, W // 8, pool=False)

    def _build_main(self):
        cfg, ops, f, lib, B = self.cfg, self.ops_main, self.f32, self.lib, self.B
        H, W = self.H, self.W
        r = self.buf(H, W, cfg.init_dim)
        wi, bi = f["init_conv.weight"], f["init_conv.bias"]
        if self.dt != cabi.LD_F32 and cfg.init_dim == 32:
            wstem = self.P["stem"]
            self.keep.append(wstem)

            def stem_begin(st, delta, idx_ptr, t_table):
                za, ba, zb, bb = self._begin_args
                rows, row_floats, cur = self._film_args
                g = cabi.StepBeginArgs(za, ba, zb, bb, self._t_dev_ptr, int(delta), idx_ptr, t_table, rows, row_floats, cur)
                cabi.check(lib.ld_conv_stem_begin(self.x_in.data_ptr(), wstem.data_ptr(), bi.data_ptr(), r.data_ptr(), B, cfg.channels,
                                                  H, W, self.dt, C.byref(g), st), "init_conv + step_begin")
            self._stem_begin = stem_begin
            self._raw(ops, lambda st: cabi.check(lib.ld_conv_stem(
                self.x_in.data_ptr(), wstem.data_ptr(), bi.data_ptr(), r.data_ptr(), B, cfg.channels, H, W, self.dt, st),
                "init_conv"), "conv_image7x7",
                nbytes=B * H * W * (4 * cfg.channels + self.esize * cfg.init_dim), flops=2 * 49 * cfg.channels * cfg.init_dim * B * H * W, writes=[r])
        else:
            self._raw(ops, lambda st: cabi.check(lib.ld_conv_image(
                self.x_in.data_ptr(), wi.data_ptr(), bi.data_ptr(), r.data_ptr(), None, 1, B, cfg.channels, H, W, 7,
                self.dt, st), "init_conv"), "conv_image7x7",
                nbytes=B * H * W * (4 * cfg.channels + self.esize * cfg.init_dim), flops=2 * 49 * cfg.channels * cfg.init_dim * B * H * W, writes=[r])
        self.named["init_conv"] = r
        x, c, h, w = r, cfg.init_dim, H, W
        skips = []
        io, n = cfg.in_out, len(cfg.in_out)
        for i, (cin, cout) in enumerate(io):
            p = f"downs.{i}"
            x = self.resnet_block(ops, p + ".0", lambda x=x, c=c: [self.src(x, c)], c, c, h, w, res_tensor=x)
            skips.append((x, c))
            x = self.resnet_block(ops, p + ".1", lambda x=x, c=c: [self.src(x, c)], c, c, h, w, res_tensor=x)
            x = self.attention(ops, p + ".2", x, c, h, w, cfg.full_attn[i])
            skips.append((x, c))
            if i < n - 1:
                h, w = h // 2, w // 2
                x = self.conv1(ops, [self.src(x, c)], self.P["w"][p + ".3.1.weight"], cout, h, w,
                               bias=f[p + ".3.1.bias"], unshuffle=1, what="downsample " + p)
            else:
                x = self.conv3(ops, [self.src(x, c)], p + ".3", cout, h, w)
            self.named[p + ".3"] = x
            c = cout
        x = self.resnet_block(ops, "mid_block1", lambda x=x, c=c: [self.src(x, c)], c, c, h, w, res_tensor=x)
        x = self.attention(ops, "mid_attn", x, c, h, w, True)
        x = self.resnet_block(ops, "mid_block2", lambda x=x, c=c: [self.src(x, c)], c, c, h, w, res_tensor=x)
        feat = self.cond_feat
        if self.fusion_const is not None:
            x = self.fusion_block_folded(ops, x, c, h, w)
        else:
            x = self.resnet_block(ops, "conv_fusion", lambda x=x, c=c: [self.src(x, c), self.src(feat, c)], 2 * c, c, h, w)
        for j, ((cin, cout), full) in enumerate(zip(reversed(io), reversed(cfg.full_attn))):
            p = f"ups.{j}"
            for k in (0, 1):
                sk, sc = skips.pop()
                x = self.resnet_block(ops, f"{p}.{k}", lambda x=x, c=c, sk=sk, sc=sc: [self.src(x, c), self.src(sk, sc)],
                                      c + sc, cout, h, w)
                c = cout
            x = self.attention(ops, p + ".2", x, c, h, w, full)
            if j < n - 1:
                h, w = h * 2, w * 2
                x = self.conv3(ops, [self.src(x, c, ups=1)], p + ".3.1", cin, h, w)
            else:
                x = self.conv3(ops, [self.src(x, c)], p + ".3", cin, h, w)
            self.named[p + ".3"] = x
            c = cin
        if self.tn.recompute_stem and self._track is not None and self.dt != cabi.LD_F32 and cfg.init_dim == 32:
            r2 = self.buf(H, W, cfg.init_dim)
            wstem2 = self.P["stem"]
            self._raw(ops, lambda st, r2=r2: cabi.check(lib.ld_conv_stem(
                self.x_in.data_ptr(), wstem2.data_ptr(), bi.data_ptr(), r2.data_ptr(), B, cfg.channels, H, W, self.dt, st),
                "init_conv (again)"), "conv_image7x7",
                nbytes=B * H * W * (4 * cfg.channels + self.esize * cfg.init_dim), flops=2 * 49 * cfg.channels * cfg.init_dim * B * H * W, writes=[r2])
            r_cat = r2
        else:
            r_cat = r
        x = self.resnet_block(ops, "final_res_block", lambda x=x, c=c, r_cat=r_cat: [self.src(x, c), self.src(r_cat, cfg.init_dim)],
                              c + cfg.init_dim, cfg.dim, h, w)
        wf = f["final_conv.weight"].reshape(cfg.out_dim, cfg.dim).contiguous()
        bf = f["final_conv.bias"]
        self.keep += [wf, bf, x, r]
        self.final = (x, wf, bf)
        self.live_out.append(x)
        self._raw(ops, lambda st, x=x: cabi.check(lib.ld_final_conv(
            x.data_ptr(), wf.data_ptr(), bf.data_ptr(), self.model_out.data_ptr(), B, H, W, cfg.dim, cfg.out_dim,
            self.dt, st), "final_conv"), "final_conv",
            nbytes=B * H * W * (self.esize * cfg.dim + 4 * cfg.out_dim), flops=2 * cfg.dim * cfg.out_dim * B * H * W, reads=[x])

    def __del__(self):
        try:
            if getattr(self, "_cond_graph", None) is not None:
                self.lib.ld_graph_destroy(self._cond_graph)
        except Exception:
            pass

    def run_time(self, st):
        for op in self.ops_time:
            op(st)

    def run_cond(self, st):
        self.cond_version = getattr(self, "cond_version", 0) + 1
        s = self.stats[:self.cond_slots]
        self.lib.ld_range_push(b"encoder")
        try:
            cabi.check(self.lib.ld_memset_zero(s.data_ptr(), s.numel() * 8, st), "memset")
            for op in self.ops_cond:
                op(st)
        finally:
            self.lib.ld_range_pop()

    def run_cond_replayed(self, stream):
        st = stream.cuda_stream
        g = getattr(self, "_cond_graph", None)
        if g is None:
            self.run_cond(st)
            stream.synchronize()
            s = self.stats[:self.cond_slots]
            cabi.check(self.lib.ld_graph_begin(st), "graph_begin")
            try:
                cabi.check(self.lib.ld_memset_zero(s.data_ptr(), s.numel() * 8, st), "memset")
                for op in self.ops_cond:
                    op(st)
            finally:
                g = C.c_void_p()
                rc = self.lib.ld_graph_end(st, C.byref(g))
            cabi.check(rc, "graph_end")
            self._cond_graph = g
            if self.tn.graph_prewarm:
                cabi.check(self.lib.ld_graph_launch(g, st), "graph_launch")
            return
        self.cond_version = getattr(self, "cond_version", 0) + 1
        self.lib.ld_range_push(b"encoder (graph replay)")
        try:
            cabi.check(self.lib.ld_graph_launch(g, st), "graph_launch")
        finally:
            self.lib.ld_range_pop()

    def run_main(self, st, skip_final=False, step_delta=0, idx_ptr=None, t_table=None):
        self.lib.ld_range_push(b"step")
        try:
            ops = self.ops_main[:-1] if skip_final else self.ops_main
            stem_begin = getattr(self, "_stem_begin", None) if self.tn.fused_step_begin else None
            if stem_begin is not None:
                stem_begin(st, 0 if idx_ptr is not None else int(step_delta), idx_ptr, t_table)
                ops = ops[1:]
            elif idx_ptr is not None:
                cabi.check(self.lib.ld_step_begin_film(*self._begin_args, self._t_dev_ptr, 0, idx_ptr, t_table, *self._film_args, st),
                           "step_begin")
            else:
                cabi.check(self.lib.ld_step_begin_film(*self._begin_args, self._t_dev_ptr, int(step_delta), None, None,
                                                       *self._film_args, st), "step_begin")
            for op in ops:
                op(st)
        finally:
            self.lib.ld_range_pop()

    def run_main_timed(self, st, acc):
        lib = self.lib
        cabi.check(lib.ld_step_begin_film(*self._begin_args, self._t_dev_ptr, 0, None, None, *self._film_args, st), "step_begin")
        cabi.check(lib.ld_timing_begin(8 * len(self.ops_main)), "timing_begin")
        marks = [0]
        try:
            for op in self.ops_main:
                op(st)
                marks.append(lib.ld_timing_count())
        finally:
            n = max(1, lib.ld_timing_count())
            ms, cnt = (C.c_float * n)(), C.c_int()
            rc = lib.ld_timing_end(ms, n, C.byref(cnt))
        cabi.check(rc, "timing_end")
        for i in range(len(self.ops_main)):
            a = acc.setdefault(i, [0.0, 0])
            a[0] += sum(ms[marks[i]:marks[i + 1]])
            a[1] += 1

    def set_step(self, t):
        self.t_dev.fill_(int(t))
```

Measured before the change: 6.559 patches/s.

## Fuse final resblock 1x1 GN-tail conv with final conv and DDPM step

Adds an EPI_FINAL_STEP epilogue to the conv1x1 kernel. The last resnet block's GroupNorm-tail 1x1 conv now stages its output in LDS and, in the same kernel, applies the final 32->C conv and the DDPM/final-step update (noise, x_t, model_out). This drops one launch per step and avoids writing the 32-channel activation to global memory and reading it back. In exchange the kernel uses more LDS and registers and has a more complex code path. It is enabled by default through fuse_final_tail=True.

```diff
diff --git a/include/localdiff_hip.h b/include/localdiff_hip.h
--- a/include/localdiff_hip.h
+++ b/include/localdiff_hip.h
@@ -196,6 +196,11 @@
                      const float* sched, const int32_t* t_ptr, float lo, float hi, int objective, uint64_t seed,
                      int64_t noise_base, int64_t noise_tmul, int64_t noise_first, const float* keep_mask,
                      int B, int H, int W, int Cin, int Cout, int dtype, void* stream);
+
+int ld_final_tail_step_at(const ld_conv1x1_args* tail, const float* w, const float* b, float* model_out, float* x_t,
+                          float* x0_out, const float* sched, const int32_t* t_ptr, float lo, float hi, int objective,
+                          uint64_t seed, int64_t noise_base, int64_t noise_tmul, int64_t noise_first,
+                          const float* keep_mask, int Cout, void* stream);
 
 #define LD_OBJ_X0 0
 #define LD_OBJ_NOISE 1
diff --git a/localdiffusion-hallucination_amd/_cabi.py b/localdiffusion-hallucination_amd/_cabi.py
--- a/localdiffusion-hallucination_amd/_cabi.py
+++ b/localdiffusion-hallucination_amd/_cabi.py
@@ -127,6 +127,8 @@
                                 C.c_int, C.c_int, C.c_int, vp]),
     "ld_final_step_at": (C.c_int, [vp, vp, vp, vp, vp, vp, vp, vp, f32, f32, C.c_int, u64, i64, i64, i64, vp, C.c_int,
                                    C.c_int, C.c_int, C.c_int, C.c_int, C.c_int, vp]),
+    "ld_final_tail_step_at": (C.c_int, [C.POINTER(Conv1x1Args), vp, vp, vp, vp, vp, vp, vp, f32, f32, C.c_int, u64, i64, i64, i64, vp,
+                                        C.c_int, vp]),
     "ld_timing_begin": (C.c_int, [C.c_int]),
     "ld_timing_count": (C.c_int, []),
     "ld_timing_end": (C.c_int, [vp, C.c_int, vp]),
diff --git a/localdiffusion-hallucination_amd/csrc/conv1x1.hip b/localdiffusion-hallucination_amd/csrc/conv1x1.hip
--- a/localdiffusion-hallucination_amd/csrc/conv1x1.hip
+++ b/localdiffusion-hallucination_amd/csrc/conv1x1.hip
@@ -1,9 +1,11 @@
 #include "common.hip.h"
+#include "final_step.hip.h"
 #include <stdlib.h>
 
 namespace {
 
 constexpr int EPI_GN_TAIL_RES = 6;
+constexpr int EPI_FINAL_STEP = 7;
 
 struct Conv1Dev {
   SrcDev s[2];
@@ -22,15 +24,30 @@
   unsigned* kmax;
   SrcDev tail;
 };
+struct FinalTailDev {
+  const float* fw;
+  const float* fb;
+  float* model_out;
+  float* x_t;
+  float* x0o;
+  const float* sched;
+  const int* t_ptr;
+  const float* keep_mask;
+  unsigned long long seed;
+  long stream_base, stream_tmul, first;
+  float lo, hi;
+  int obj, fc_out;
+};
 
 constexpr int KG = 4;
 typedef const Conv1Dev __attribute__((address_space(4)))* Conv1KernargPtr;
 template <typename T, int MT, int NW, int EPI, int G, bool TLEAD, bool KLEAD = false>
-__device__ __forceinline__ void conv1x1_body(const Conv1Dev& head, Conv1KernargPtr rest) {
+__device__ __forceinline__ void conv1x1_body(const Conv1Dev& head, Conv1KernargPtr rest, const FinalTailDev* fin = nullptr) {
   constexpr int E = DT<T>::E, CK = DT<T>::CK;
   constexpr int NPT = 64 * NW, PLANE = NPT * 16;
   constexpr int XCH = 4 * PLANE, WCHB = MT * 1024;
-  static_assert(!TLEAD || EPI == LD_EPI_GN_TAIL || EPI == EPI_GN_TAIL_RES, "tail-lead variant: GroupNorm-tail epilogues only");
+  constexpr bool FINAL = EPI == EPI_FINAL_STEP;
+  static_assert(!TLEAD || EPI == LD_EPI_GN_TAIL || EPI == EPI_GN_TAIL_RES || FINAL, "tail-lead variant: GroupNorm-tail epilogues only");
   Conv1Dev a = head;
   if constexpr (KLEAD) {
     a.out = rest->out; a.bias = rest->bias; a.g2 = rest->g2; a.kmax = rest->kmax; a.hidden = rest->hidden; a.q_scale = rest->q_scale;
@@ -39,7 +56,7 @@
     asm volatile("" ::"s"(a.H), "s"(a.W), "s"(a.Cout), "s"(a.nsrc), "s"(a.unshuffle), "s"(a.rms_in), "s"(a.wsplit), "s"(a.s[0].C),
                  "s"(a.s[0].ld), "s"(a.s[0].data), "s"(a.s[1].C), "s"(a.s[1].ld), "s"(a.s[1].data), "s"(a.w), "s"(a.w_bstride),
                  "s"(a.res), "s"(a.out));
-    if constexpr (EPI == LD_EPI_GN_TAIL || EPI == EPI_GN_TAIL_RES)
+    if constexpr (EPI == LD_EPI_GN_TAIL || EPI == EPI_GN_TAIL_RES || FINAL)
       asm volatile("" ::"s"(a.tail.data), "s"(a.tail.stats), "s"(a.tail.gamma), "s"(a.tail.beta), "s"(a.tail.film), "s"(a.tail.C),
                    "s"(a.tail.groups), "s"(a.tail.act), "s"(a.tail.film_bstride));
   }
@@ -48,6 +65,8 @@
   char* s_x = smem;
   char* s_w = smem + G * XCH;
   float* s_rinv = reinterpret_cast<float*>(s_w + G * WCHB);
+  const int pstride = FINAL ? head.Cout * (int)sizeof(T) + 16 : 0;
+  if constexpr (FINAL) s_rinv = reinterpret_cast<float*>(smem + max(G * (XCH + WCHB), NPT * pstride));
   float* s_tcoef = s_rinv + NPT;
 
   const int tid = threadIdx.x, lane = tid & 63, wv = tid >> 6, px = lane & 15, kq = lane >> 4;
@@ -64,7 +83,7 @@
 #pragma unroll
   for (int i = 0; i < NW; ++i) rs[i] = 0.f;
 
-  constexpr bool TAIL = EPI == LD_EPI_GN_TAIL || EPI == EPI_GN_TAIL_RES;
+  constexpr bool TAIL = EPI == LD_EPI_GN_TAIL || EPI == EPI_GN_TAIL_RES || FINAL;
   constexpr bool HAS_OP2 = EPI == LD_EPI_RMS_RES || EPI == LD_EPI_RES || TAIL;
   typedef typename Raw4<T>::type R4;
   constexpr bool W2 = sizeof(T) == 2;
@@ -97,6 +116,8 @@
     }
   };
   if constexpr (HAS_OP2) load_op(reinterpret_cast<const T*>(TAIL ? a.tail.data : a.res), op2);
+  [[maybe_unused]] int f_t = 0;
+  if constexpr (FINAL) f_t = fin->t_ptr ? *fin->t_ptr : 0;
   if constexpr (TAIL) {
     double* red = reinterpret_cast<double*>(s_tcoef + 2 * a.Cout);
     if constexpr (TLEAD) {
@@ -114,6 +135,33 @@
       build_gn_coef<DT<T>::precise>(a.tail, b, 0, (long)HW, s_tcoef, red, tid, 256);
     }
   }
+  [[maybe_unused]] FinalStepK fk{};
+  [[maybe_unused]] float fwv = 0.f;
+  [[maybe_unused]] f32x4 f_xi = {0.f, 0.f, 0.f, 0.f}, f_nz = {0.f, 0.f, 0.f, 0.f}, f_fb = {0.f, 0.f, 0.f, 0.f};
+  [[maybe_unused]] float f_keep = 1.0f;
+  const int f_qq = wv * NW * 16 + lane;
+  const bool f_own = FINAL && lane < 16 * NW && p0 + f_qq < HW;
+  auto final_head = [&]() {
+    if constexpr (FINAL) {
+      const FinalTailDev& f = *fin;
+      const int fco = f.fc_out;
+      fk = final_step_setup_t(f.sched, f_t, f.lo, f.hi, f.obj, f.seed, f.stream_base, f.stream_tmul, f.first);
+      fwv = f.fw[min(tid, a.Cout * fco - 1)];
+      if (f_own) {
+        const int p = p0 + f_qq;
+        if (f.keep_mask) f_keep = f.keep_mask[(size_t)b * HW + p];
+#pragma unroll
+        for (int o = 0; o < 4; ++o)
+          if (o < fco) { f_xi[o] = f.x_t[((size_t)b * fco + o) * HW + p]; f_fb[o] = f.fb[o]; }
+        if (fk.t > 0) {
+#pragma unroll
+          for (int o = 0; o < 4; ++o)
+            if (o < fco) f_nz[o] = final_step_noise(fk, ((size_t)b * fco + o) * HW + p);
+        }
+      }
+    }
+  };
+  if constexpr (FINAL && G == 1) final_head();
   const int nc0 = a.s[0].C / CK;
   const int ws = a.wsplit;
   const int nch = (a.unshuffle ? 4 * nc0 : nc0 + (a.nsrc > 1 ? a.s[1].C / CK : 0)) << ws;
@@ -178,9 +226,16 @@
 #pragma unroll
           for (int k = 0; k < WPT; ++k) {
             const int u = k * 256 + tid;
-            wr[g][k] = u < MT * 64 ? wg[((size_t)(c0 + g) * mt_total + m0) * 64 + u] : make_uint4(0u, 0u, 0u, 0u);
+            if constexpr (FINAL) {
+              const u32x4 q = load16_act(&wg[((size_t)(c0 + g) * mt_total + m0) * 64 + min(u, MT * 64 - 1)]);
+              wr[g][k] = make_uint4(q.x, q.y, q.z, q.w);
+            }
+            else wr[g][k] = u < MT * 64 ? wg[((size_t)(c0 + g) * mt_total + m0) * 64 + u] : make_uint4(0u, 0u, 0u, 0u);
           }
         }
+      }
+      if constexpr (FINAL) {
+        if (c0 == 0) final_head();
       }
       __syncthreads();
 #pragma unroll
@@ -228,6 +283,11 @@
     __syncthreads();
   }
 
+  if constexpr (FINAL) {
+    float* s_fw = reinterpret_cast<float*>(reinterpret_cast<double*>(s_tcoef + 2 * a.Cout) + 64);
+    if (tid < a.Cout * fin->fc_out) s_fw[tid] = fwv;
+    __syncthreads();
+  }
   float bv[MT][4], g2v[EPI == LD_EPI_RMS_RES ? MT : 1][4];
 #pragma unroll
   for (int m = 0; m < MT; ++m) {
@@ -346,7 +406,16 @@
       }
     }
     T* opix = out + ((size_t)b * HW + (valid ? p : 0)) * a.Cout + m0 * 16;
-    if constexpr (sizeof(T) == 2) {
+    if constexpr (FINAL) {
+      char* prow = smem + qq * pstride;
+      if constexpr (sizeof(T) == 2) {
+#pragma unroll
+        for (int m = 0; m < MT; m += 2) *reinterpret_cast<uint4*>(prow + m * 32 + pair_frag16_off(kq)) = pair_frag16<T>(v[m], v[m + 1]);
+      } else {
+#pragma unroll
+        for (int m = 0; m < MT; ++m) *reinterpret_cast<float4*>(prow + (m * 16 + kq * 4) * 4) = make_float4(v[m][0], v[m][1], v[m][2], v[m][3]);
+      }
+    } else if constexpr (sizeof(T) == 2) {
       static_assert(MT % 2 == 0, "m-tiles are stored in pairs");
 #pragma unroll
       for (int m = 0; m < MT; m += 2) {
@@ -357,6 +426,23 @@
 #pragma unroll
       for (int m = 0; m < MT; ++m) store4<T>(opix + m * 16 + kq * 4, v[m]);
     }
+  }
+  if constexpr (FINAL) {
+    __builtin_amdgcn_fence(__ATOMIC_RELEASE, "wavefront");
+    __builtin_amdgcn_wave_barrier();
+    __builtin_amdgcn_fence(__ATOMIC_ACQUIRE, "wavefront");
+    const float* s_fw = reinterpret_cast<const float*>(reinterpret_cast<double*>(s_tcoef + 2 * a.Cout) + 64);
+    const FinalTailDev& f = *fin;
+    const int fco = f.fc_out;
+    if (f_own) {
+      const int p = p0 + f_qq;
+      float fc[4];
+      final_conv_pixel<T>(reinterpret_cast<const T*>(smem + f_qq * pstride), s_fw, a.Cout, fco, fc);
+#pragma unroll
+      for (int o = 0; o < 4; ++o)
+        if (o < fco) final_step_elem(fk, fc[o], f_fb[o], f_keep >= 1.0f, f_xi[o], f_nz[o], ((size_t)b * fco + o) * HW + p, f.model_out, f.x_t, f.x0o);
+    }
+    return;
   }
   if (k_part) {
     float* s_cm = reinterpret_cast<float*>(s_x);
@@ -393,6 +479,23 @@
   static_assert(REST_OFF == 48, "conv1x1_taillead_kernel: leading arguments changed");
   typedef const char __attribute__((address_space(4)))* KChar;
   conv1x1_body<T, MT, NW, EPI, G, true>(a, (Conv1KernargPtr)((KChar)__builtin_amdgcn_kernarg_segment_ptr() + REST_OFF));
+}
+
+template <typename T, int MT, int NW, int G>
+__global__ __launch_bounds__(256) void conv1x1_final_kernel(Conv1Dev a, FinalTailDev fin) {
+  conv1x1_body<T, MT, NW, EPI_FINAL_STEP, G, false>(a, nullptr, &fin);
+}
+template <typename T, int MT, int NW, int G>
+__global__ __launch_bounds__(256) void conv1x1_final_taillead_kernel(const void* t_data, const double* t_stats, const float* t_gamma, const float* t_beta,
+                                                                     const float* t_film, int cout_groups, int hw, Conv1Dev rest, FinalTailDev fin) {
+  Conv1Dev a{};
+  a.tail.data = t_data; a.tail.stats = t_stats; a.tail.gamma = t_gamma; a.tail.beta = t_beta; a.tail.film = t_film;
+  a.Cout = cout_groups & 0xffff; a.tail.C = a.Cout; a.tail.ld = a.Cout; a.tail.groups = (int)((unsigned)cout_groups >> 16);
+  a.H = hw; a.W = 1;
+  constexpr unsigned REST_OFF = ld_kernarg_offset<const void*, const double*, const float*, const float*, const float*, int, int>(alignof(Conv1Dev));
+  static_assert(REST_OFF == 48, "conv1x1_final_taillead_kernel: leading arguments changed");
+  typedef const char __attribute__((address_space(4)))* KChar;
+  conv1x1_body<T, MT, NW, EPI_FINAL_STEP, G, true>(a, (Conv1KernargPtr)((KChar)__builtin_amdgcn_kernarg_segment_ptr() + REST_OFF), &fin);
 }
 
 template <typename T, int MT, int NW, int EPI, int G>
@@ -518,9 +621,53 @@
   return big ? launch<T, 2, 4>(a, st) : launch<T, 2, 2>(a, st);
 }
 
-}
-
-extern "C" int ld_conv1x1(const ld_conv1x1_args* p, void* stream) {
+template <typename T, int NW>
+int launch_final(const Conv1Dev& a, const FinalTailDev& f, hipStream_t st) {
+  constexpr int MT = 2, NPT = 64 * NW;
+  const size_t tail = NPT * sizeof(float) + 2 * a.Cout * sizeof(float) + 64 * sizeof(double) + 256 * sizeof(float);
+  const size_t chunk = 4 * NPT * 16 + MT * 1024;
+  const size_t pix = (size_t)NPT * (a.Cout * sizeof(T) + 16);
+  const int HW = a.H * a.W;
+  dim3 grid((HW + NPT - 1) / NPT, 1, a.B);
+  const int g = a.group ? a.group : 1;
+  const size_t lds = (g * chunk > pix ? g * chunk : pix) + tail;
+  const bool tlead = ld_tuning().lead_args && a.tail.film_bstride == 0 && a.tail.film_tstride == 0 && a.tail.groups < 32768 &&
+                     a.tail.C == a.Cout && a.tail.ld == a.Cout && (long)HW < (1L << 31) && (g == KG || g == 2);
+#define LD_C1_TLEAD_ARGS a.tail.data, a.tail.stats, a.tail.gamma, a.tail.beta, a.tail.film, a.Cout | (a.tail.groups << 16), HW, a, f
+  if (tlead && g == KG) {
+    LD_HIP(ld_allow_lds((conv1x1_final_taillead_kernel<T, MT, NW, KG>), lds));
+    LD_LAUNCH((conv1x1_final_taillead_kernel<T, MT, NW, KG>), grid, dim3(256), lds, st, LD_C1_TLEAD_ARGS);
+  } else if (tlead) {
+    LD_HIP(ld_allow_lds((conv1x1_final_taillead_kernel<T, MT, NW, 2>), lds));
+    LD_LAUNCH((conv1x1_final_taillead_kernel<T, MT, NW, 2>), grid, dim3(256), lds, st, LD_C1_TLEAD_ARGS);
+  } else if (g == KG) {
+    LD_HIP(ld_allow_lds((conv1x1_final_kernel<T, MT, NW, KG>), lds));
+    LD_LAUNCH((conv1x1_final_kernel<T, MT, NW, KG>), grid, dim3(256), lds, st, a, f);
+  } else if (g == 2) {
+    LD_HIP(ld_allow_lds((conv1x1_final_kernel<T, MT, NW, 2>), lds));
+    LD_LAUNCH((conv1x1_final_kernel<T, MT, NW, 2>), grid, dim3(256), lds, st, a, f);
+  } else {
+    LD_LAUNCH((conv1x1_final_kernel<T, MT, NW, 1>), grid, dim3(256), lds, st, a, f);
+  }
+#undef LD_C1_TLEAD_ARGS
+  LD_LAUNCH_CHECK("conv1x1(GroupNorm tail + final step)");
+  return LD_OK;
+}
+template <typename T>
+int dispatch_final(const Conv1Dev& a0, const FinalTailDev& f, hipStream_t st) {
+  Conv1Dev a = a0;
+  const int HW = a.H * a.W;
+  {
+    const LdTuning& tn = ld_tuning();
+    const int nch = (a.s[0].C / DT<T>::CK + (a.nsrc > 1 ? a.s[1].C / DT<T>::CK : 0)) << a.wsplit;
+    a.group = (tn.c1_group && (long)HW * a.B <= tn.c1_group_max_px && nch >= (int)tn.c1_group_min_ch) ? KG : 0;
+    if (tn.c1_group && !a.group && (long)HW * a.B <= tn.c1_pair_max_px && nch >= 2) a.group = 2;
+  }
+  const bool big = (long)((HW + 255) / 256) * a.B >= 512;
+  return big ? launch_final<T, 4>(a, f, st) : launch_final<T, 2>(a, f, st);
+}
+
+int conv1_prepare(const ld_conv1x1_args* p, Conv1Dev& a) {
   LD_REQUIRE(p != nullptr, "ld_conv1x1: null args");
   LD_REQUIRE(p->nsrc == 1 || p->nsrc == 2, "ld_conv1x1: nsrc must be 1 or 2");
   LD_REQUIRE(ld_dtype_ok(p->dtype), "ld_conv1x1: bad dtype %d", p->dtype);
@@ -535,7 +682,6 @@
   LD_REQUIRE((reinterpret_cast<uintptr_t>(p->bias) & 15) == 0 && (reinterpret_cast<uintptr_t>(p->g2) & 15) == 0,
              "ld_conv1x1: bias / g2 must be 16-byte aligned (read as float4)");
   if (p->epilogue == LD_EPI_RES) LD_REQUIRE(p->residual, "ld_conv1x1: RES needs residual");
-  Conv1Dev a;
   for (int s = 0; s < p->nsrc; ++s) {
     LD_REQUIRE(p->src[s].data && p->src[s].C > 0 && p->src[s].C % 32 == 0,
                "ld_conv1x1: src[%d] null or C %% 32 != 0", s);
@@ -565,6 +711,35 @@
   LD_REQUIRE(p->weight_terms >= 0 && p->weight_terms <= 2 && !(p->weight_terms == 2 && (!ld_dtype_16(p->dtype) || p->rms_in || p->weight_bstride)),
              "ld_conv1x1: weight_terms %d (2 needs 16-bit storage, no rms_in, no per-batch weights)", p->weight_terms);
   a.wsplit = p->weight_terms == 2 ? 1 : 0;
+  return LD_OK;
+}
+
+}
+
+extern "C" int ld_conv1x1(const ld_conv1x1_args* p, void* stream) {
+  Conv1Dev a;
+  if (int rc = conv1_prepare(p, a)) return rc;
   hipStream_t st = reinterpret_cast<hipStream_t>(stream);
   return LD_DISPATCH(p->dtype, dispatch<T>(a, st));
 }
+
+extern "C" int ld_final_tail_step_at(const ld_conv1x1_args* p, const float* w, const float* b, float* model_out, float* x_t,
+                                     float* x0_out, const float* sched, const int32_t* t_ptr, float lo, float hi, int objective,
+                                     uint64_t seed, int64_t noise_base, int64_t noise_tmul, int64_t noise_first,
+                                     const float* keep_mask, int Cout, void* stream) {
+  LD_REQUIRE(p && w && b && model_out && x_t && sched, "ld_final_tail_step: null pointer");
+  LD_REQUIRE(noise_first >= 0 && (noise_tmul == 0 || t_ptr), "ld_final_tail_step: noise_first %ld, noise_tmul without t_ptr",
+             (long)noise_first);
+  LD_REQUIRE(Cout >= 1 && Cout <= 4, "ld_final_tail_step: final_conv Cout %d (1..4)", Cout);
+  LD_REQUIRE(objective >= 0 && objective <= 2, "ld_final_tail_step: objective %d", objective);
+  LD_REQUIRE(p->epilogue == LD_EPI_GN_TAIL && p->nsrc >= 1 && !p->unshuffle && !p->rms_in && p->weight_bstride == 0 && !p->residual,
+             "ld_final_tail_step: the block's tail must be a plain LD_EPI_GN_TAIL launch (no unshuffle, rms_in, per-batch weights, residual)");
+  LD_REQUIRE(p->weight_terms != 2, "ld_final_tail_step: two-term weights are not routed here (run the two launches)");
+  LD_REQUIRE(p->Cout == 32, "ld_final_tail_step: the block's Cout %d does not fit one workgroup (32)", p->Cout);
+  Conv1Dev a;
+  if (int rc = conv1_prepare(p, a)) return rc;
+  const FinalTailDev f{w, b, model_out, x_t, x0_out, sched, t_ptr, keep_mask, (unsigned long long)seed, (long)noise_base,
+                       (long)noise_tmul, (long)noise_first, lo, hi, objective, Cout};
+  hipStream_t st = reinterpret_cast<hipStream_t>(stream);
+  return LD_DISPATCH(p->dtype, dispatch_final<T>(a, f, st));
+}
diff --git a/localdiffusion-hallucination_amd/csrc/final_step.hip.h b/localdiffusion-hallucination_amd/csrc/final_step.hip.h
--- /dev/null
+++ b/localdiffusion-hallucination_amd/csrc/final_step.hip.h
@@ -0,0 +1,83 @@
+#pragma once
+#include "common.hip.h"
+
+__device__ __forceinline__ float clampf(float v, float lo, float hi) { return fminf(fmaxf(v, lo), hi); }
+
+__device__ __forceinline__ float to_x0(float x, float mo, const float* row, int obj) {
+  if (obj == LD_OBJ_X0) return mo;
+  if (obj == LD_OBJ_NOISE) return row[LD_SCHED_SQRT_RECIP] * x - row[LD_SCHED_SQRT_RECIPM1] * mo;
+  return row[LD_SCHED_SQRT_AB] * x - row[LD_SCHED_SQRT_1MAB] * mo;
+}
+
+__device__ __forceinline__ unsigned long long mix64(unsigned long long z) {
+  z = (z ^ (z >> 30)) * 0xBF58476D1CE4E5B9ull;
+  z = (z ^ (z >> 27)) * 0x94D049BB133111EBull;
+  return z ^ (z >> 31);
+}
+
+template <typename T>
+__device__ __forceinline__ void final_conv_pixel(const T* xp, const float* s_w, int Cin, int Cout, float* acc) {
+  constexpr int E = 16 / sizeof(T);
+  acc[0] = acc[1] = acc[2] = acc[3] = 0.f;
+  for (int c0 = 0; c0 < Cin; c0 += 4 * E) {
+    uint4 raw[4];
+#pragma unroll
+    for (int q = 0; q < 4; ++q)
+      raw[q] = (c0 + q * E < Cin) ? *reinterpret_cast<const uint4*>(xp + c0 + q * E) : make_uint4(0u, 0u, 0u, 0u);
+#pragma unroll
+    for (int q = 0; q < 4; ++q) {
+      if (c0 + q * E >= Cin) break;
+      float v[E];
+      unpack16<T>(raw[q], v);
+#pragma unroll
+      for (int g = 0; g < E; g += 4) {
+        const int c = c0 + q * E + g;
+        for (int o = 0; o < Cout; ++o) {
+          const float* wr = s_w + o * Cin + c;
+          acc[o] = fmaf(v[g], wr[0], fmaf(v[g + 1], wr[1], fmaf(v[g + 2], wr[2], fmaf(v[g + 3], wr[3], acc[o]))));
+        }
+      }
+    }
+  }
+}
+
+struct FinalStepK {
+  float c1, c2, sg, sr, srm1, sab, s1mab, lo, hi;
+  int t, obj;
+  unsigned long long base;
+  long first;
+};
+__device__ __forceinline__ FinalStepK final_step_setup_t(const float* sched, int t, float lo, float hi, int obj,
+                                                         unsigned long long seed, long stream_base, long stream_tmul, long first) {
+  FinalStepK k;
+  k.t = t;
+  const long stream = stream_base + stream_tmul * (long)k.t;
+  const float* row = sched + (size_t)k.t * LD_SCHED_COLS;
+  k.c1 = row[LD_SCHED_COEF1]; k.c2 = row[LD_SCHED_COEF2]; k.sg = row[LD_SCHED_SIGMA];
+  k.sr = row[LD_SCHED_SQRT_RECIP]; k.srm1 = row[LD_SCHED_SQRT_RECIPM1]; k.sab = row[LD_SCHED_SQRT_AB]; k.s1mab = row[LD_SCHED_SQRT_1MAB];
+  k.lo = lo; k.hi = hi; k.obj = obj;
+  k.base = mix64(seed ^ ((unsigned long long)stream * 0xD1B54A32D192ED03ull));
+  k.first = first;
+  return k;
+}
+__device__ __forceinline__ FinalStepK final_step_setup(const float* sched, const int* t_ptr, float lo, float hi, int obj,
+                                                       unsigned long long seed, long stream_base, long stream_tmul, long first) {
+  return final_step_setup_t(sched, t_ptr ? *t_ptr : 0, lo, hi, obj, seed, stream_base, stream_tmul, first);
+}
+__device__ __forceinline__ float final_step_noise(const FinalStepK& k, size_t idx) {
+  const unsigned long long h = mix64(k.base + (unsigned long long)(k.first + idx + 1) * 0x9E3779B97F4A7C15ull);
+  const float u1 = ((float)(unsigned)(h >> 40) + 1.0f) * 5.9604644775390625e-8f;
+  const float u2 = (float)(unsigned)((h >> 16) & 0xFFFFFFu) * 5.9604644775390625e-8f;
+  return sqrtf(-2.0f * logf(u1)) * cosf(6.283185307179586f * u2);
+}
+__device__ __forceinline__ void final_step_elem(const FinalStepK& k, float conv, float bias, bool keep, float xi, float nz, size_t idx,
+                                                float* model_out, float* x_t, float* x0o) {
+  const float mo = keep ? conv + bias : k.lo;
+  store_f32_out(&model_out[idx], mo);
+  const float x0r = k.obj == LD_OBJ_X0 ? mo : (k.obj == LD_OBJ_NOISE ? k.sr * xi - k.srm1 * mo : k.sab * xi - k.s1mab * mo);
+  const float x0 = clampf(x0r, k.lo, k.hi);
+  const float mean = k.c1 * x0 + k.c2 * xi;
+  const float r = k.t > 0 ? mean + k.sg * nz : mean;
+  store_f32_out(&x_t[idx], r);
+  if (x0o) store_f32_out(&x0o[idx], x0);
+}
diff --git a/localdiffusion-hallucination_amd/csrc/pointwise.hip b/localdiffusion-hallucination_amd/csrc/pointwise.hip
--- a/localdiffusion-hallucination_amd/csrc/pointwise.hip
+++ b/localdiffusion-hallucination_amd/csrc/pointwise.hip
@@ -1,4 +1,5 @@
 #include "common.hip.h"
+#include "final_step.hip.h"
 
 namespace {
 constexpr int BS = 256;
@@ -10,19 +11,6 @@
 }
 #define GRID_STRIDE(i, n) for (long i = (long)blockIdx.x * BS + threadIdx.x; i < (n); i += (long)gridDim.x * BS)
 
-__device__ __forceinline__ float clampf(float v, float lo, float hi) { return fminf(fmaxf(v, lo), hi); }
-
-__device__ __forceinline__ float to_x0(float x, float mo, const float* row, int obj) {
-  if (obj == LD_OBJ_X0) return mo;
-  if (obj == LD_OBJ_NOISE) return row[LD_SCHED_SQRT_RECIP] * x - row[LD_SCHED_SQRT_RECIPM1] * mo;
-  return row[LD_SCHED_SQRT_AB] * x - row[LD_SCHED_SQRT_1MAB] * mo;
-}
-
-__device__ __forceinline__ unsigned long long mix64(unsigned long long z) {
-  z = (z ^ (z >> 30)) * 0xBF58476D1CE4E5B9ull;
-  z = (z ^ (z >> 27)) * 0x94D049BB133111EBull;
-  return z ^ (z >> 31);
-}
 __global__ void randn_kernel(float* out, long n, long first, unsigned long long seed, long stream_base, long stream_tmul,
                              const int* t_ptr) {
   const long stream = stream_base + (t_ptr ? stream_tmul * (long)(*t_ptr) : 0);
@@ -236,32 +224,6 @@
 }
 
 template <typename T>
-__device__ __forceinline__ void final_conv_pixel(const T* xp, const float* s_w, int Cin, int Cout, float* acc) {
-  constexpr int E = 16 / sizeof(T);
-  acc[0] = acc[1] = acc[2] = acc[3] = 0.f;
-  for (int c0 = 0; c0 < Cin; c0 += 4 * E) {
-    uint4 raw[4];
-#pragma unroll
-    for (int q = 0; q < 4; ++q)
-      raw[q] = (c0 + q * E < Cin) ? *reinterpret_cast<const uint4*>(xp + c0 + q * E) : make_uint4(0u, 0u, 0u, 0u);
-#pragma unroll
-    for (int q = 0; q < 4; ++q) {
-      if (c0 + q * E >= Cin) break;
-      float v[E];
-      unpack16<T>(raw[q], v);
-#pragma unroll
-      for (int g = 0; g < E; g += 4) {
-        const int c = c0 + q * E + g;
-        for (int o = 0; o < Cout; ++o) {
-          const float* wr = s_w + o * Cin + c;
-          acc[o] = fmaf(v[g], wr[0], fmaf(v[g + 1], wr[1], fmaf(v[g + 2], wr[2], fmaf(v[g + 3], wr[3], acc[o]))));
-        }
-      }
-    }
-  }
-}
-
-template <typename T>
 __global__ void final_conv_kernel(const T* __restrict__ x, const float* __restrict__ w, const float* __restrict__ bias,
                                   float* __restrict__ out, int HW, int Cin, int Cout, long npix) {
   extern __shared__ float s_fw[];
@@ -283,11 +245,7 @@
                                   const float* __restrict__ keep_mask, int HW, int Cin, int Cout, long npix) {
   extern __shared__ float s_fw[];
   for (int i = threadIdx.x; i < Cin * Cout; i += BS) s_fw[i] = w[i];
-  const int t = t_ptr ? *t_ptr : 0;
-  const long stream = stream_base + stream_tmul * (long)t;
-  const float* row = sched + (size_t)t * LD_SCHED_COLS;
-  const float c1 = row[LD_SCHED_COEF1], c2 = row[LD_SCHED_COEF2], sg = row[LD_SCHED_SIGMA];
-  const unsigned long long base = mix64(seed ^ ((unsigned long long)stream * 0xD1B54A32D192ED03ull));
+  const FinalStepK k = final_step_setup(sched, t_ptr, lo, hi, obj, seed, stream_base, stream_tmul, first);
   __syncthreads();
   GRID_STRIDE(i, npix) {
     const long b = i / HW, p = i - b * HW;
@@ -296,20 +254,7 @@
     const bool keep = keep_mask ? keep_mask[i] >= 1.0f : true;
     for (int o = 0; o < Cout; ++o) {
       const size_t idx = ((size_t)b * Cout + o) * HW + p;
-      const float mo = keep ? acc[o] + bias[o] : lo;
-      store_f32_out(&model_out[idx], mo);
-      const float xi = x_t[idx];
-      const float x0 = clampf(to_x0(xi, mo, row, obj), lo, hi);
-      const float mean = c1 * x0 + c2 * xi;
-      float r = mean;
-      if (t > 0) {
-        const unsigned long long h = mix64(base + (unsigned long long)(first + idx + 1) * 0x9E3779B97F4A7C15ull);
-        const float u1 = ((float)(unsigned)(h >> 40) + 1.0f) * 5.9604644775390625e-8f;
-        const float u2 = (float)(unsigned)((h >> 16) & 0xFFFFFFu) * 5.9604644775390625e-8f;
-        r = mean + sg * (sqrtf(-2.0f * logf(u1)) * cosf(6.283185307179586f * u2));
-      }
-      store_f32_out(&x_t[idx], r);
-      if (x0o) store_f32_out(&x0o[idx], x0);
+      final_step_elem(k, acc[o], bias[o], keep, x_t[idx], k.t > 0 ? final_step_noise(k, idx) : 0.f, idx, model_out, x_t, x0o);
     }
   }
 }
diff --git a/localdiffusion-hallucination_amd/diffusion.py b/localdiffusion-hallucination_amd/diffusion.py
--- a/localdiffusion-hallucination_amd/diffusion.py
+++ b/localdiffusion-hallucination_amd/diffusion.py
@@ -95,23 +95,34 @@
         for m in self.masks.values():
             m.copy_(mask.reshape(m.shape))
 
+    def _gkey(self, i, lo, hi, base):
+        return (i, float(lo), float(hi), base, self.gd.noise_seed, self.gd.noise_offset, self.gd.fuse_final_tail)
+
     def _step(self, i, st, lo, hi, base):
         gd, sp = self.gd, self.plans[i]
         lib = cabi.lib()
         xa, wf, bf = sp.final
         B_, C_, H_, W_ = sp.model_out.shape
-        sp.run_main(st, skip_final=True, step_delta=-1)
+        tail = sp.final_tail if gd.fuse_final_tail else None
+        sp.run_main(st, skip_final=True, step_delta=-1, skip_tail=tail is not None)
+        first = gd.noise_offset + (0 if self.shared_noise else i * sp.x_in.numel())
+        if tail is not None:
+            import ctypes as C
+            cabi.check(lib.ld_final_tail_step_at(C.byref(tail), wf.data_ptr(), bf.data_ptr(), sp.model_out.data_ptr(),
+                                                 sp.x_in.data_ptr(), None, gd._sched_table().data_ptr(), sp.t_dev.data_ptr(),
+                                                 lo, hi, cabi.OBJ[gd.objective], gd.noise_seed, base, -1, first,
+                                                 cabi.ptr(self.masks.get(i)), C_, st), "final_tail_step")
+            return
         cabi.check(lib.ld_final_step_at(xa.data_ptr(), wf.data_ptr(), bf.data_ptr(), sp.model_out.data_ptr(),
                                         sp.x_in.data_ptr(), None, gd._sched_table().data_ptr(), sp.t_dev.data_ptr(),
-                                        lo, hi, cabi.OBJ[gd.objective], gd.noise_seed, base, -1,
-                                        gd.noise_offset + (0 if self.shared_noise else i * sp.x_in.numel()),
+                                        lo, hi, cabi.OBJ[gd.objective], gd.noise_seed, base, -1, first,
                                         cabi.ptr(self.masks.get(i)),
                                         B_, H_, W_, wf.shape[1], C_, sp.dt, st), "final_step")
 
     def _ensure_graph(self, i, gs, lo, hi, base):
         import ctypes as C
         lib, st = cabi.lib(), gs.cuda_stream
-        key = (i, float(lo), float(hi), base, self.gd.noise_seed, self.gd.noise_offset)
+        key = self._gkey(i, lo, hi, base)
         if key in self.graphs:
             return 0
         ran = 0
@@ -132,7 +143,7 @@
     def _ensure_joint_graph(self, lo, hi, base):
         import ctypes as C
         lib = cabi.lib()
-        key = ("joint", float(lo), float(hi), base, self.gd.noise_seed, self.gd.noise_offset)
+        key = self._gkey("joint", lo, hi, base)
         if key in self.graphs:
             return self.graphs[key]
         s0 = self.streams[0]
@@ -159,7 +170,7 @@
         return g
 
     def _trim(self, lo, hi, base):
-        if (0, float(lo), float(hi), base, self.gd.noise_seed, self.gd.noise_offset) in self.graphs or len(self.graphs) < 8 * self.S:
+        if self._gkey(0, lo, hi, base) in self.graphs or len(self.graphs) < 8 * self.S:
             return
         torch.cuda.synchronize()
         for g in self.graphs.values():
@@ -185,7 +196,7 @@
                     sp.run_cond_replayed(gs)
                 sp.set_step(t_start + 1)
                 todo[i] -= self._ensure_graph(i, gs, lo, hi, base)
-                ex[i] = self.graphs[(i, float(lo), float(hi), base, self.gd.noise_seed, self.gd.noise_offset)]
+                ex[i] = self.graphs[self._gkey(i, lo, hi, base)]
         h0 = time.perf_counter()
         tn = self.gd.tuning
         if tn.sub_joint_graph and self.S > 1 and min(todo) == max(todo):
@@ -234,7 +245,7 @@
         for i in range(1, self.S):
             with torch.cuda.stream(self.streams[i]):
                 self._ensure_graph(i, self.streams[i], lo, hi, base)
-            g = self.graphs[(i, float(lo), float(hi), base, self.gd.noise_seed, self.gd.noise_offset)]
+            g = self.graphs[self._gkey(i, lo, hi, base)]
             for _ in range(n_steps + 2):
                 cabi.check(lib.ld_graph_launch(g, self.streams[i].cuda_stream), "graph_launch")
         sp, gs = self.plans[0], self.streams[0]
@@ -393,6 +404,7 @@
         self.tuning = getattr(model, "tuning", None) or Tuning.from_env()
         self.noise_source = "device"
         self.fuse_final_step = bool(self.tuning.fused_final_step)
+        self.fuse_final_tail = True
         self.noise_seed = 10
         self.noise_offset = 0
         self.use_graph = False
@@ -665,14 +677,22 @@
         if fused:
             xa, wf, bf = jp.final
             B_, C_, H_, W_ = jp.model_out.shape
+            tail = jp.final_tail if self.fuse_final_tail else None
             for _ in range(n_steps):
                 jp.set_step(t)
-                jp.run_main(st, skip_final=True)
+                jp.run_main(st, skip_final=True, skip_tail=tail is not None)
                 k = draw if t > 0 else 0
-                cabi.check(lib.ld_final_step_at(xa.data_ptr(), wf.data_ptr(), bf.data_ptr(), jp.model_out.data_ptr(),
-                                                jp.x_in.data_ptr(), cabi.ptr(x0_buf), sched.data_ptr(), jp.t_dev.data_ptr(),
-                                                lo, hi, obj, self.noise_seed, k, 0, self.noise_offset, None,
-                                                B_, H_, W_, wf.shape[1], C_, jp.dt, st), "final_step")
+                if tail is not None:
+                    import ctypes as C
+                    cabi.check(lib.ld_final_tail_step_at(C.byref(tail), wf.data_ptr(), bf.data_ptr(), jp.model_out.data_ptr(),
+                                                         jp.x_in.data_ptr(), cabi.ptr(x0_buf), sched.data_ptr(), jp.t_dev.data_ptr(),
+                                                         lo, hi, obj, self.noise_seed, k, 0, self.noise_offset, None, C_, st),
+                               "final_tail_step")
+                else:
+                    cabi.check(lib.ld_final_step_at(xa.data_ptr(), wf.data_ptr(), bf.data_ptr(), jp.model_out.data_ptr(),
+                                                    jp.x_in.data_ptr(), cabi.ptr(x0_buf), sched.data_ptr(), jp.t_dev.data_ptr(),
+                                                    lo, hi, obj, self.noise_seed, k, 0, self.noise_offset, None,
+                                                    B_, H_, W_, wf.shape[1], C_, jp.dt, st), "final_step")
                 if t > 0:
                     draw += 1
                 if after is not None:
diff --git a/localdiffusion-hallucination_amd/unet.py b/localdiffusion-hallucination_amd/unet.py
--- a/localdiffusion-hallucination_amd/unet.py
+++ b/localdiffusion-hallucination_amd/unet.py
@@ -606,6 +606,7 @@
         cin = sum(s.C for s in srcs) * (4 if unshuffle else 1)
         npx = self.B * h * w
         el = npx * cin + npx * cout + cin * cout * (self.B if bstride else 1) + (npx * cout if (residual is not None or gn_tail is not None) else 0)
+        self._last_conv1 = a
         self._call(ops, self.lib.ld_conv1x1, a, what,
                    dict(family="conv1x1", bytes=el * self.esize, flops=2 * cin * cout * npx, shape=f"{cin}->{cout}@{h}x{w}"),
                    reads=[s._tensor for s in srcs] + [residual, gn_tail._tensor if gn_tail is not None else None], writes=[out])
@@ -914,6 +915,13 @@
         self.keep += [wf, bf, x, r]
         self.final = (x, wf, bf)
         self.live_out.append(x)
+        self.final_tail = None
+        tail_i, ta = len(ops) - 1, getattr(self, "_last_conv1", None)
+        if (self.meta[tail_i]["what"] == "res_conv+tail final_res_block" and ta is not None and ta.out == x.data_ptr()
+                and ta.epilogue == cabi.EPI_GN_TAIL and ta.Cout == 32 and ta.weight_terms != 2 and not ta.residual
+                and 1 <= cfg.out_dim <= 4):
+            self.final_tail = ta
+            self.live_out += list(self.decl[tail_i][0])
         self._raw(ops, lambda st, x=x: cabi.check(lib.ld_final_conv(
             x.data_ptr(), wf.data_ptr(), bf.data_ptr(), self.model_out.data_ptr(), B, H, W, cfg.dim, cfg.out_dim,
             self.dt, st), "final_conv"), "final_conv",
@@ -968,10 +976,13 @@
         finally:
             self.lib.ld_range_pop()
 
-    def run_main(self, st, skip_final=False, step_delta=0, idx_ptr=None, t_table=None):
+    def run_main(self, st, skip_final=False, step_delta=0, idx_ptr=None, t_table=None, skip_tail=False):
         self.lib.ld_range_push(b"step")
         try:
             ops = self.ops_main[:-1] if skip_final else self.ops_main
+            if skip_tail:
+                assert skip_final and self.final_tail is not None
+                ops = ops[:-1]
             stem_begin = getattr(self, "_stem_begin", None) if self.tn.fused_step_begin else None
             if stem_begin is not None:
                 stem_begin(st, 0 if idx_ptr is not None else int(step_delta), idx_ptr, t_table)
```

After: 6.500 patches/s, median of 2. About the same (-0.9%).
